# WasifurRahman/BERT_multimodal_transformer

Measured on AMD Instinct MI355X. Metric: train samples/sec MAG-BERT MOSI seq_len=50, higher is better.
Workload: dtype bf16; 1 GPU; MAG-BERT bert-base-uncased, MOSI dims (V=47, A=74), batch 48/GPU, seq_len 50, full optimizer step (fwd+MSE+bwd+HF-AdamW+schedule+zero_grad; inputs resident in HBM), dropout on, random-init weights; global_batch=48, seq_len=50, parallelism=dp1, step_call=mb_bert_train_step, hipGraph replay

## Files before the change

### bert_multimodal_transformer_amd/_lib.py

```python
import ctypes as C
import os

_HERE = os.path.dirname(os.path.abspath(__file__))
LIB_PATH = os.path.join(os.environ.get("MB_LIB_DIR") or os.path.join(_HERE, "lib"), "libmagbert_hip.so")

DT_F32, DT_BF16 = 0, 1
GEMM_NT, GEMM_NN, GEMM_TN = 0, 1, 2
EPI_BIAS, EPI_BIAS_GELU, EPI_BIAS_DROP_RES, EPI_ADD_RES, EPI_DGELU, EPI_ACCUM_F32, EPI_BIAS_F32 = range(7)
EPI_BIAS_RELU, EPI_BIAS_SWISH, EPI_BIAS_GELU_NEW, EPI_BIAS_MISH = 7, 8, 9, 10
ACT_GELU, ACT_RELU, ACT_SWISH, ACT_GELU_NEW, ACT_MISH = range(5)
ACTIVATIONS = {"gelu": ACT_GELU, "relu": ACT_RELU, "swish": ACT_SWISH, "silu": ACT_SWISH, "gelu_new": ACT_GELU_NEW, "mish": ACT_MISH}
ACT_EPILOGUE = {ACT_GELU: EPI_BIAS_GELU, ACT_RELU: EPI_BIAS_RELU, ACT_SWISH: EPI_BIAS_SWISH, ACT_GELU_NEW: EPI_BIAS_GELU_NEW,
                ACT_MISH: EPI_BIAS_MISH}


def activation_code(name, field):
    if isinstance(name, str) and name in ACTIVATIONS:
        return ACTIVATIONS[name]
    raise NotImplementedError("%s=%r: the feed-forward activations built are %s (and silu = swish)"
                              % (field, name, ", ".join(n for n in ACTIVATIONS if n != "silu")))


class DropKey(C.Structure):
    _fields_ = [("k0", C.c_uint32), ("k1", C.c_uint32), ("thresh", C.c_uint32), ("scale", C.c_float)]
# ... 49 lines not shown
    "mb_gemm": (_i, [_i, _i, _i, _i, _i, _i, _vp, _i, _vp, _i, _vp, _i, _vp, _vp, _vp, _vp, _i, _f, _dk, _i, _i, _vp]),
    "mb_gemm_grouped_wgrad": (_i, [_i, _i, _vp, _vp, _i, _vp, _vp, _vp, _vp, _vp, _vp, _i, _vp]),
    "mb_narrow": (_i, [_i, _vp, _vp, _sz, _vp]),
    "mb_widen": (_i, [_i, _vp, _vp, _sz, _vp]),
    "mb_layernorm_forward": (_i, [_i, _vp, _vp, _vp, _f, _vp, _vp, _vp, _i, _i, _dk, _vp]),
    "mb_layernorm_backward": (_i, [_i, _vp, _vp, _vp, _vp, _vp, _vp, _vp, _vp, _vp, _vp, _i, _i, _dk, _dk, _vp]),
    "mb_embed_forward": (_i, [_i, _vp, _vp, _vp, _vp, _vp, _vp, _vp, _f, _vp, _vp, _vp, _i, _i, _i, _dk, _vp]),
    "mb_embed_backward": (_i, [_i, _vp, _vp, _vp, _vp, _vp, _vp, _vp, _vp, _vp, _vp, _vp, _vp, _vp, _vp, _vp, _i, _i, _i,
                               _i, _dk, _vp]),
    "mb_attention_forward": (_i, [_i, _vp, _vp, _vp, _i, _i, _i, _dk, _vp]),
    "mb_attention_backward": (_i, [_i, _vp, _vp, _vp, _vp, _i, _i, _i, _dk, _vp]),
    "mb_attention_resident_forward": (_i, [_i, _vp, _vp, _vp, _i, _i, _i, _dk, _vp, _vp, _vp]),
    "mb_attention_resident_backward": (_i, [_i, _vp, _vp, _vp, _vp, _vp, _i, _i, _i, _dk, _vp, _vp]),
    "mb_head_forward": (_i, [_vp, _vp, _vp, _vp, _vp, _vp, _vp, _vp, _i, _i, _i, _dk, _i, _f, _vp, _vp]),
    "mb_head_backward": (_i, [_i, _vp, _vp, _vp, _f, _vp, _vp, _vp, _vp, _vp, _vp, _vp, _sz, _i, _i, _i, _dk, _i, _f, _vp, _vp]),
    "mb_head_forward_ex": (_i, [_vp, _vp, _vp, _vp, _vp, _vp, _vp, _vp, _i, _i, _i, _dk, C.POINTER(HeadLossStruct), _vp]),
    "mb_head_backward_ex": (_i, [_i, _vp, _vp, _vp, _f, _vp, _vp, _vp, _vp, _vp, _vp, _vp, _sz, _i, _i, _i, _dk, C.POINTER(HeadLossStruct), _vp]),
    "mb_bert_set_head_loss_ex": (_i, [_vp, C.POINTER(HeadLossStruct)]),
    "mb_bert_get_head_loss_ex": (_i, [_vp, C.POINTER(HeadLossStruct), _vp, C.POINTER(_i)]),
    "mb_xlnet_set_head_loss_ex": (_i, [_vp, C.POINTER(HeadLossStruct)]),
    "mb_xlnet_get_head_loss_ex": (_i, [_vp, C.POINTER(HeadLossStruct), _vp, C.POINTER(_i)]),
    "mb_bert_set_head_loss": (_i, [_vp, _i, _f, _vp]),
    "mb_bert_get_head_loss": (_i, [_vp, C.POINTER(_i), C.POINTER(_f), _vp, C.POINTER(_i)]),
    "mb_xlnet_set_head_loss": (_i, [_vp, _i, _f, _vp]),
    "mb_xlnet_get_head_loss": (_i, [_vp, C.POINTER(_i), C.POINTER(_f), _vp, C.POINTER(_i)]),
    "mb_attention_tiled_stats_bytes": (_sz, [_i, _i, _i]),
    "mb_attention_tiled_forward": (_i, [_i, _vp, _vp, _vp, _vp, _i, _i, _i, _dk, _vp, _vp, _vp]),
    "mb_attention_tiled_backward": (_i, [_i, _vp, _vp, _vp, _vp, _vp, _vp, _vp, _i, _i, _i, _dk, _vp, _vp]),
    "mb_mag_workspace_bytes": (_sz, [_i, _i, _i, _i, _i]),
    "mb_mag_forward": (_i, [_i] + [_vp] * 13 + [_f, _dk, _vp, _vp, _i, _i, _i, _i, _vp]),
    "mb_mag_backward": (_i, [_i] + [_vp] * 11 + [_f, _dk] + [_vp] * 14 + [_i, _i, _i, _i, _vp]),
    "mb_debug_mag_forward_ex": (_i, [_i] + [_vp] * 13 + [_f, _dk, _vp, _vp, _i, _i, _i, _i, _i, _vp]),
    "mb_debug_mag_slab_bytes": (_sz, [_i, _i]),
    "mb_debug_mag_backward_ex": (_i, [_i] + [_vp] * 7 + [_f, _dk] + [_vp] * 14 + [_i, _i, _i, _i, _i, _i, _i, _vp, _sz, _i,
                                      C.POINTER(_i), _vp]),
    "mb_adamw_step": (_i, [_vp, _vp, _vp, _vp, _vp, _sz, _sz, _sz, _sz, _f, _f, _f, _f, _f, _i, _i, _f, _i, _vp]),
    "mb_bert_create": (_i, [C.POINTER(BertEngineConfig), C.POINTER(_vp)]),
    "mb_bert_destroy": (None, [_vp]),
    "mb_bert_num_tensors": (_i, [_vp]),
    "mb_bert_tensor_info": (_i, [_vp, _i, C.c_char_p, _i, C.POINTER(_sz), C.POINTER(_sz), C.POINTER(_i),
                                 C.POINTER(C.c_int64), C.POINTER(_i)]),
    "mb_bert_param_count": (_sz, [_vp]),
    "mb_bert_decay_count": (_sz, [_vp]),
    "mb_bert_shadow_range": (None, [_vp, C.POINTER(_sz), C.POINTER(_sz)]),
    "mb_bert_workspace_bytes": (_sz, [_vp]),
    "mb_bert_bind": (_i, [_vp, _vp, _vp, _vp, _vp, _sz]),
    "mb_bert_sync_weights": (_i, [_vp, _vp]),
    "mb_bert_forward": (_i, [_vp, _vp, _vp, _vp, _vp, _vp, _vp, _i, _i, _i, _u64, _u64, _vp, _vp, _vp, _vp]),
    "mb_bert_backward": (_i, [_vp, _vp, _vp, _f, _i, _i, _vp]),
    "mb_bert_sequence_output": (_vp, [_vp]),
    "mb_bert_pooled_output": (_vp, [_vp]),
    "mb_bert_hidden_state": (_vp, [_vp, _i]),
    "mb_bert_set_attention_output": (_i, [_vp, _vp]),
    "mb_debug_gemm_ex": (_i, [_i, _i, _i, _i, _i, _i, _vp, _i, _vp, _i, _vp, _i, _vp, _vp, _vp, _vp, _i, _f, _dk, _i, _i,
                              _i, _sz, _i, _i, _vp, _i, _vp, _vp, _vp, _vp, _vp, _sz, _i, _i, _f, _f, _f, _f, _f, _i, _i, _f, _vp,
                              C.POINTER(_i), _vp]),
    "mb_debug_gemm_grouped_ex": (_i, [_i, _i, _vp, _vp, _i, _vp, _vp, _vp, _vp, _vp, _vp, _vp, _vp, _i, _i, _vp, _vp, _vp, _vp, _vp,
                                      _sz, _i, _i, _f, _f, _f, _f, _f, _i, _i, _f, _vp, _vp]),
    "mb_debug_gemm_last_kernel": (_i, [C.c_char_p, _i]),
    "mb_debug_gemm_grouped_rows": (_i, [_i, _i, _vp, _vp, _i, _vp, _vp, _vp, _vp, _vp, _vp, _vp, _i, _vp, _vp, _vp]),
    "mb_debug_live_rows": (_i, [_vp, _i, _i, _i, _vp, _vp, _vp, _vp, _vp]),
    "mb_bert_debug_live_wgrad_launches": (_i, [_vp]),
    "mb_bert_debug_wgrad_dy": (_vp, [_vp, _i, _i, C.POINTER(_i)]),
    "mb_debug_gemm_trace": (_i, [_vp, _i]),
    "mb_debug_attention_trace": (_i, [_vp, _i]),
    "mb_xlnet_attention_probs": (_vp, [_vp, _i, C.POINTER(_i)]),
    "mb_xlnet_attention_probs_into": (_i, [_vp, _i, _vp, _vp]),
    "mb_xlnet_attention_tiled_stats_bytes": (_sz, [_i, _i, _i]),
    "mb_xlnet_attention_tiled_scratch_bytes": (_sz, [_i, _i, _i, _i]),
    "mb_xlnet_attention_tiled_forward": (_i, [_i] + [_vp] * 10 + [_i, _i, _i, _dk, _vp, _vp, _i, _vp, _vp]),
    "mb_xlnet_attention_tiled_backward": (_i, [_i] + [_vp] * 19 + [_i, _i, _i, _dk, _vp, _vp, _vp]),
    "mb_xlnet_attention_forward": (_i, [_i] + [_vp] * 11 + [_i, _i, _i, _dk, _vp, _vp, _i, _vp]),
    "mb_xlnet_attention_backward": (_i, [_i] + [_vp] * 20 + [_i, _i, _i, _dk, _vp, _vp, _vp]),
    "mb_xlnet_set_head_mask": (_i, [_vp, _vp]),
    "mb_xlnet_set_perm_mask": (_i, [_vp, _vp]),
    "mb_xlnet_set_mems": (_i, [_vp, _vp, _i]),
    "mb_xlnet_query_stream_scratch_bytes": (_sz, [_vp, _i, _i, _i]),
    "mb_xlnet_query_stream_state_bytes": (_sz, [_vp, _i, _i]),
    "mb_xlnet_query_stream": (_i, [_vp, _vp, _i, _vp, _sz, _vp, _vp]),
    "mb_bert_mark_grads_zero": (_i, [_vp, _i]),
    "mb_xlnet_mark_grads_zero": (_i, [_vp, _i]),
    "mb_bert_distrust_word_stamps": (_i, [_vp]),
    "mb_bert_word_skip_updates": (_sz, [_vp]),
    "mb_bert_materialize_grads": (_i, [_vp, _vp]),
    "mb_xlnet_materialize_grads": (_i, [_vp, _vp]),
    "mb_bert_grads_stale": (_i, [_vp]),
    "mb_xlnet_grads_stale": (_i, [_vp]),
    "mb_bert_set_head_mask": (_i, [_vp, _vp]),
    "mb_bert_set_inputs_embeds": (_i, [_vp, _vp]),
    "mb_bert_set_position_ids": (_i, [_vp, _vp]),
    "mb_bert_inputs_embeds_grad": (_vp, [_vp]),
    "mb_bert_backward_outputs": (_i, [_vp, _vp, _vp, _vp]),
    "mb_bert_stage_grad_ranges": (_i, [_vp, _i, C.POINTER(_sz), C.POINTER(_sz), _i]),
    "mb_bert_train_step": (_i, [_vp, _vp, _vp, _vp, _vp, _vp, _vp, _i, _i, _u64, _u64, _vp, _vp, _vp, _vp, _vp, _f, _f, _f, _f, _f,
                                _i, _i, _f, _f, _i, _vp]),
    "mb_bert_stage_forward": (_i, [_vp, _vp, _vp, _vp, _vp, _vp, _vp, _i, _i, _u64, _u64, _vp, _vp, _vp, _i, _vp]),
    "mb_bert_stage_backward": (_i, [_vp, _f, _i, _i, _vp]),
    "mb_bert_staged_input_ids": (_vp, [_vp]),
    "mb_bert_load_batch": (_i, [_vp, _vp, _vp, _vp, _vp, _vp, _vp, _i, _i, C.POINTER(_vp), _vp]),
    "mb_bert_graph_stats": (_i, [_vp, C.POINTER(_sz), C.POINTER(_sz)]),
    "mb_bert_set_profiling": (_i, [_vp, _i]),
    "mb_bert_profile_wgrad_us": (_i, [_vp, C.POINTER(_f)]),
    "mb_bert_profile_adamw_us": (_i, [_vp, C.POINTER(_f)]),
    "mb_xlnet_set_inputs_embeds": (_i, [_vp, _vp]),
    "mb_xlnet_inputs_embeds_grad": (_vp, [_vp]),
    "mb_xlnet_model_output": (_vp, [_vp, _vp]),
    "mb_xlnet_backward_outputs": (_i, [_vp, _vp, _vp]),
    "mb_xlnet_set_profiling": (_i, [_vp, _i]),
    "mb_xlnet_profile_wgrad_us": (_i, [_vp, C.POINTER(_f)]),
    "mb_xlnet_profile_adamw_us": (_i, [_vp, C.POINTER(_f)]),
    "mb_xlnet_create": (_i, [C.POINTER(XlnetEngineConfig), C.POINTER(_vp)]),
    "mb_xlnet_destroy": (None, [_vp]),
    "mb_xlnet_num_tensors": (_i, [_vp]),
    "mb_xlnet_tensor_info": (_i, [_vp, _i, C.c_char_p, _i, C.POINTER(_sz), C.POINTER(_sz), C.POINTER(_i),
                                  C.POINTER(C.c_int64), C.POINTER(_i)]),
    "mb_xlnet_param_count": (_sz, [_vp]),
    "mb_xlnet_decay_count": (_sz, [_vp]),
    "mb_xlnet_shadow_range": (None, [_vp, C.POINTER(_sz), C.POINTER(_sz)]),
    "mb_xlnet_workspace_bytes": (_sz, [_vp]),
    "mb_xlnet_bind": (_i, [_vp, _vp, _vp, _vp, _vp, _sz]),
    "mb_xlnet_sync_weights": (_i, [_vp, _vp]),
    "mb_xlnet_forward": (_i, [_vp, _vp, _vp, _vp, _vp, _vp, _vp, _i, _i, _i, _u64, _u64, _vp, _vp, _vp, _vp]),
    "mb_xlnet_backward": (_i, [_vp, _vp, _vp, _f, _i, _i, _vp]),
    "mb_xlnet_sequence_output": (_vp, [_vp]),
    "mb_xlnet_hidden_state": (_vp, [_vp, _i]),
    "mb_xlnet_train_step": (_i, [_vp, _vp, _vp, _vp, _vp, _vp, _vp, _i, _i, _u64, _u64, _vp, _vp, _vp, _vp, _vp, _f, _f, _f, _f, _f,
                                 _i, _i, _f, _f, _i, _vp]),
    "mb_xlnet_load_batch": (_i, [_vp, _vp, _vp, _vp, _vp, _vp, _vp, _i, _i, C.POINTER(_vp), _vp]),
    "mb_xlnet_graph_stats": (_i, [_vp, C.POINTER(_sz), C.POINTER(_sz)]),
    "mb_xlnet_trainable_count": (_sz, [_vp]),
    "mb_bert_set_update_map": (_i, [_vp, _i, _i, _vp, _vp]),
    "mb_bert_set_update_decay": (_i, [_vp, _i, _vp]),
    "mb_bert_set_update_values": (_i, [_vp, _i, _vp, _vp, _vp, _vp, _vp, _vp]),
    "mb_bert_update_stats": (_i, [_vp, C.POINTER(_sz), C.POINTER(_sz), C.POINTER(_i)]),
    "mb_bert_set_update_frozen": (_i, [_vp, _i, _vp]),
    "mb_bert_freeze_stats": (_i, [_vp, C.POINTER(_sz), C.POINTER(_i), C.POINTER(_i)]),
    "mb_xlnet_set_update_frozen": (_i, [_vp, _i, _vp]),
    "mb_xlnet_freeze_stats": (_i, [_vp, C.POINTER(_sz), C.POINTER(_i), C.POINTER(_i)]),
    "mb_xlnet_set_update_map": (_i, [_vp, _i, _i, _vp, _vp]),
    "mb_xlnet_set_update_decay": (_i, [_vp, _i, _vp]),
    "mb_xlnet_set_update_values": (_i, [_vp, _i, _vp, _vp, _vp, _vp, _vp, _vp]),
    "mb_xlnet_update_stats": (_i, [_vp, C.POINTER(_sz), C.POINTER(_sz), C.POINTER(_i)]),
    "mb_grad_clip_scratch_bytes": (_sz, [_sz]),
    "mb_grad_clip_coef": (_i, [_vp, _sz, _f, _f, _vp, _vp, _vp]),
    "mb_bert_set_grad_clip": (_i, [_vp, _f]),
    "mb_bert_grad_clip_stats": (_i, [_vp, C.POINTER(_f), C.POINTER(_f), _vp]),
    "mb_xlnet_set_grad_clip": (_i, [_vp, _f]),
    "mb_xlnet_grad_clip_stats": (_i, [_vp, C.POINTER(_f), C.POINTER(_f), _vp]),
    "mb_xlnet_stage_grad_ranges": (_i, [_vp, _i, C.POINTER(_sz), C.POINTER(_sz), _i]),
    "mb_comm_unique_id": (_i, [_vp]),
    "mb_comm_create_rccl": (_i, [_vp, _i, _i, C.POINTER(_vp)]),
    "mb_comm_create_callbacks": (_i, [_i, _i, _vp, _vp, _vp, C.POINTER(_vp)]),
    "mb_comm_destroy": (None, [_vp]),
    "mb_comm_rank": (_i, [_vp]),
    "mb_comm_world": (_i, [_vp]),
    "mb_comm_stream": (_vp, [_vp]),
    "mb_comm_scratch_bytes": (_sz, [_i, _i, _sz, _i, _i, _i]),
    "mb_comm_bind_scratch": (_i, [_vp, _vp, _sz, _i, _sz, _i, _i, _i]),
    "mb_comm_all_reduce": (_i, [_vp, _vp, _sz, _vp]),
    "mb_comm_exchange_rows": (_i, [_vp, _vp, _vp, _i, _vp]),
    "mb_comm_set_row_exchange": (_i, [_vp, _i]),
    "mb_comm_set_sharding": (_i, [_vp, _i]),
    "mb_comm_sharding": (_i, [_vp]),
    "mb_comm_join": (_i, [_vp, _vp]),
    "mb_comm_gather_shards": (_i, [_vp, _vp, _i, _vp]),
    "mb_comm_shard_slices": (_i, [_vp, C.POINTER(_sz), _i]),
# ... 57 lines not shown
```

### bert_multimodal_transformer_amd/bert.py

```python
import ctypes as C
import os

import torch
import torch.nn as nn

from . import _lib
from . import losses as _losses
from .global_configs import ACOUSTIC_DIM, VISUAL_DIM


SUPPORTED_HIDDEN_SIZES = (256, 512, 768, 1024)


def check_bert_sizes(config, injection_index=None):
    H, nh, I, NL = (int(config.hidden_size), int(config.num_attention_heads), int(config.intermediate_size), int(config.num_hidden_layers))
    if H not in SUPPORTED_HIDDEN_SIZES:
        raise ValueError("hidden_size = %d: the HIP engine runs hidden sizes %s (heads of 64)" % (H, ", ".join(map(str, SUPPORTED_HIDDEN_SIZES))))
    if nh * 64 != H:
        raise ValueError("num_attention_heads = %d with hidden_size = %d: the attention kernels take heads of 64 (%d heads); hidden sizes %s"
                         % (nh, H, H // 64, ", ".join(map(str, SUPPORTED_HIDDEN_SIZES))))
    if I % 128 or I < 128:
        raise ValueError("intermediate_size = %d: must be a multiple of 128" % I)
    if NL < 1:
        raise ValueError("num_hidden_layers = %d: at least one layer" % NL)
# ... 174 lines not shown
        c, mc = self.config, self.mc
        if self.kind == "xlnet":
            return _lib.XlnetEngineConfig(
                c.vocab_size, c.d_model, c.n_layer, c.n_head, c.d_inner, c.num_labels, self.V, self.A, int(self.injection_index),
                c.layer_norm_eps, 1e-5, float(mc.beta_shift), c.dropout, c.summary_last_dropout, float(mc.dropout_prob),
                self.dt, int(B), int(L), _lib.activation_code(c.ff_activation, "ff_activation"))
        return _lib.BertEngineConfig(
            c.vocab_size, c.hidden_size, c.num_hidden_layers, c.num_attention_heads, c.intermediate_size,
            c.max_position_embeddings, c.type_vocab_size, c.num_labels, self.V, self.A, c.pad_token_id,
            c.layer_norm_eps, 1e-5, float(mc.beta_shift), c.hidden_dropout_prob, c.attention_probs_dropout_prob,
            float(mc.dropout_prob), self.dt, int(B), int(L), _lib.activation_code(c.hidden_act, "hidden_act"),
            int(self.injection_index))

    def _make_engine(self, B, L):
        h = C.c_void_p()
        cfg = self._cfg(B, L)
        _lib.check(self._fn("create")(C.byref(cfg), C.byref(h)))
        if self.handle is not None:
            self._fn("destroy")(self.handle)
            self.ws = None
        self.handle = h
        self._optional = (None, None, None, None, None)
        self._update_map = None
        self.max_B, self.max_L = B, L
        self._apply_loss()

    def _apply_loss(self):
        vec = self.loss.vector
        arr = None if vec is None else (C.c_float * len(vec))(*vec)
        hl = _lib.head_loss_struct(self.loss.code, self.loss.beta, None if arr is None else C.addressof(arr), self.loss.label_smoothing,
                                   self.loss.focal_gamma, self.loss.ignore_index)
        _lib.check(self._fn("set_head_loss_ex")(self.handle, C.byref(hl)))

    def set_loss(self, loss):
        old, self.loss = self.loss, loss
        try:
            self._apply_loss()
        except Exception:
            self.loss = old
            raise
        self._lab_ptr = None

    def _comm_join(self):
        comm = getattr(self, "_dp_comm", None)
        if comm is not None and comm.sharding and comm.handle is not None:
            _lib.check(self.lib.mb_comm_join(comm.handle, self.stream()))

    def refresh_sharded_state(self, adam=True):
        old = getattr(self, "_dp_shards", None)
        if old is not None:
            old.gather_masters()
            if adam and hasattr(self, "_adam_m"):
                old._gather([self._adam_m[a:b] for a, b in old.bounds])
                old._gather([self._adam_v[a:b] for a, b in old.bounds])
            return
        comm = getattr(self, "_dp_comm", None)
        if comm is None or not comm.sharding or comm.handle is None:
            return
        self._comm_join()
        st = self.stream()
        _lib.check(self.lib.mb_comm_gather_shards(comm.handle, _lib.ptr(self.params), 4, st))
        if adam and hasattr(self, "_adam_m"):
            _lib.check(self.lib.mb_comm_gather_shards(comm.handle, _lib.ptr(self._adam_m), 4, st))
            _lib.check(self.lib.mb_comm_gather_shards(comm.handle, _lib.ptr(self._adam_v), 4, st))

    def _ensure(self, B, L, join=True):
        if join:
            self._comm_join()
        if L > self.max_seq_length:
            raise _lib.MagbertError("magbert: unsupported shape or alignment: L = %d is above this model's max_seq_length = %d "
                                    "(construct it with max_seq_length=%d, at most %d)"
                                    % (L, self.max_seq_length, L,
                                       self.config.max_position_embeddings if self.kind == "bert" else XLNET_MAX_SEQ))
        if B > self.max_B or L > self.max_L or self.ws is None:
            self.materialize_grads()
            self._make_engine(max(B, self.max_B), max(L, self.max_L))
            nbytes = self._fn("workspace_bytes")(self.handle)
            self.ws = torch.empty(nbytes, dtype=torch.uint8, device=self.device)
            _lib.check(self._fn("bind")(self.handle, _lib.ptr(self.params), _lib.ptr(self.grads),
                                             _lib.ptr(self.shadow) if self.dt == _lib.DT_BF16 else None,
                                             _lib.ptr(self.ws), nbytes))
            self.weights_dirty = True
            _lib.check(self._fn("mark_grads_zero")(self.handle, 1 if self._gz else 0))

    def _tensor_table(self):
        out = []
        name = C.create_string_buffer(160)
        off, numel, ndim, decay = C.c_size_t(), C.c_size_t(), C.c_int(), C.c_int()
        shape = (C.c_int64 * 4)()
        for i in range(self._fn("num_tensors")(self.handle)):
            _lib.check(self._fn("tensor_info")(self.handle, i, name, 160, C.byref(off), C.byref(numel), C.byref(ndim),
                                                    shape, C.byref(decay)))
            out.append((name.value.decode(), off.value, numel.value, tuple(shape[k] for k in range(ndim.value)),
                        int(decay.value)))
        return out

    def stream(self):
        return torch.cuda.current_stream(self.device).cuda_stream

    class _Hop(object):

        def __init__(self, core):
            self.core = core
            self.cur = torch.cuda.current_stream(core.device)
            self.hop = self.cur.cuda_stream == 0
            self.ctx = None

        def __enter__(self):
            if self.hop:
                if self.core._own_stream is None:
                    self.core._own_stream = torch.cuda.Stream(device=self.core.device)
                self.core._own_stream.wait_stream(self.cur)
                self.ctx = torch.cuda.stream(self.core._own_stream)
                self.ctx.__enter__()
            return self

        def __exit__(self, *exc):
            if self.hop:
                self.ctx.__exit__(*exc)
                self.cur.wait_stream(self.core._own_stream)
            return False

    def sync_weights(self):
        if self.dt == _lib.DT_BF16:
            self.refresh_sharded_state(adam=False)
        with _Core._Hop(self):
            _lib.check(self._fn("sync_weights")(self.handle, self.stream()))
        self.weights_dirty = False

    def _pinned_batch(self, tensors, B, L):
        want = (torch.int64, torch.float32, torch.float32, torch.int64, torch.int64, torch.float32)
        shapes = ((B, L), (B, L, self.V), (B, L, self.A), (B, L), (B, L), None)
        for t, dt, shp in zip(tensors, want, shapes):
            if t is None:
                continue
            if t.is_cuda or t.dtype != dt or not t.is_contiguous() or (shp is not None and tuple(t.shape) != shp) or not t.is_pinned():
                return False
        return True

    def _inputs(self, input_ids, visual, acoustic, attention_mask, token_type_ids, labels, gather_in_step=False):
        B, L = input_ids.shape
        dev = self.device
        lab_in = None if labels is None else labels.reshape(-1)
        if lab_in is not None:
            _losses.check_labels(self.loss, lab_in, B, int(self.config.num_labels))
        six = (input_ids, visual, acoustic, attention_mask, token_type_ids, lab_in)
        if self._pinned_batch(six, B, L):
            ptrs = [None if t is None else C.c_void_p(t.data_ptr()) for t in six]
            if gather_in_step:
                return ptrs, six
            staged = (C.c_void_p * 6)()
            with _Core._Hop(self):
                _lib.check(self._fn("load_batch")(self.handle, ptrs[0], ptrs[1], ptrs[2], ptrs[3], ptrs[4], ptrs[5], B, L, staged,
                                                   self.stream()))
            off = staged[0] - self.ws.data_ptr()
            self._ids_dev = self.ws[off: off + B * L * 8].view(torch.int64)
            return [C.c_void_p(staged[i]) if staged[i] else None for i in range(6)], six
        nb = not input_ids.is_cuda and input_ids.is_pinned()
        ids = input_ids.to(dev, torch.int64, non_blocking=nb).contiguous()
        msk = attention_mask.to(dev, torch.int64, non_blocking=nb).contiguous()
        seg = token_type_ids.to(dev, torch.int64, non_blocking=nb).contiguous()
        vis = visual.to(dev, torch.float32, non_blocking=nb).contiguous()
        aco = acoustic.to(dev, torch.float32, non_blocking=nb).contiguous()
        if vis.shape != (B, L, self.V) or aco.shape != (B, L, self.A):
            raise ValueError("visual/acoustic must be [B, L, %d] / [B, L, %d], got %s / %s" %
                             (self.V, self.A, tuple(vis.shape), tuple(aco.shape)))
        lab = None if labels is None else labels.to(dev, torch.float32, non_blocking=nb).contiguous().view(-1)
        keep = (ids, vis, aco, msk, seg, lab)
        self._ids_dev = ids.reshape(-1)
        return [_lib.ptr(t) for t in keep], keep

    def _set_optional(self, head_mask=None, inputs_embeds=None, position_ids=None, perm=None, mems=None):
        want = (head_mask, inputs_embeds, position_ids, perm, mems)
        if all(x is None for x in want) and all(x is None for x in self._optional):
            return
        if self.kind != "bert":
            if position_ids is not None:
                raise NotImplementedError("position_ids is an argument of MAG-BERT only (XLNet has relative positions)")
            _lib.check(self.lib.mb_xlnet_set_head_mask(self.handle, _lib.ptr(head_mask)))
            _lib.check(self.lib.mb_xlnet_set_inputs_embeds(self.handle, _lib.ptr(inputs_embeds)))
            _lib.check(self.lib.mb_xlnet_set_perm_mask(self.handle, _lib.ptr(perm)))
            _lib.check(self.lib.mb_xlnet_set_mems(self.handle, _lib.ptr(mems), 0 if mems is None else int(mems.shape[2])))
        else:
            if perm is not None or mems is not None:
                raise NotImplementedError("perm_mask / mems are arguments of MAG-XLNet only")
            _lib.check(self.lib.mb_bert_set_head_mask(self.handle, _lib.ptr(head_mask)))
            _lib.check(self.lib.mb_bert_set_inputs_embeds(self.handle, _lib.ptr(inputs_embeds)))
            _lib.check(self.lib.mb_bert_set_position_ids(self.handle, _lib.ptr(position_ids)))
        self._optional = want

    def mark_grads_zero(self, known_zero=True):
        if not known_zero:
            self.materialize_grads()
        self._gz = bool(known_zero)
        self._gz_version = self.grads._version
        if self.handle is not None:
            _lib.check(self._fn("mark_grads_zero")(self.handle, 1 if known_zero else 0))

    def torch_wrote_grads(self):
        return (not self._gz) or self.grads._version != getattr(self, "_gz_version", -1)

    def materialize_grads(self):
        if self.handle is not None and self.ws is not None and self._fn("grads_stale")(self.handle):
            with _Core._Hop(self):
                _lib.check(self._fn("materialize_grads")(self.handle, self.stream()))

    def head_mask_table(self, head_mask):
        if head_mask is None:
            return None
        NL, nh = self.n_layers, (self.config.num_attention_heads if self.kind == "bert" else self.config.n_head)
        hm = torch.as_tensor(head_mask).to(self.device, torch.float32)
        if hm.dim() == 1 and hm.numel() == nh:
            hm = hm[None].expand(NL, nh)
        elif hm.numel() == NL * nh and (hm.dim() == 2 or tuple(hm.shape) == (NL, 1, nh, 1, 1)):
            hm = hm.reshape(NL, nh)
        else:
            raise NotImplementedError("head_mask must be [num_heads] or [num_layers, num_heads], got %s" % (tuple(hm.shape),))
        return hm.contiguous()

    def inputs_embeds_grad(self):
        p = self._fn("inputs_embeds_grad")(self.handle)
        B, L, H = self._emb_shape
        off = p - self.ws.data_ptr()
        return self.ws[off: off + B * L * H * 4].view(torch.float32).view(B, L, H).clone()

    def forward(self, input_ids, visual, acoustic, attention_mask, token_type_ids, labels, training, mems=None, head_mask=None,
                inputs_embeds=None, position_ids=None, perm=None):
        dev = self.device
        if inputs_embeds is not None:
            inputs_embeds = inputs_embeds.detach().to(dev, torch.float32).contiguous()
            B, L, H = inputs_embeds.shape
            if H != self.config.hidden_size:
                raise ValueError("inputs_embeds must be [B, L, %d]" % self.config.hidden_size)
            self._emb_shape = (B, L, H)
            input_ids = torch.zeros(B, L, dtype=torch.int64, device=dev)
        B, L = input_ids.shape
        self._ensure(B, L)
        if self.weights_dirty:
            self.sync_weights()
        if position_ids is not None:
            position_ids = position_ids.to(dev, torch.int64).expand(B, L).contiguous()
        if perm is not None:
            perm = perm.to(dev, torch.uint8).contiguous()
            if tuple(perm.shape) != (B, L, L):
                raise ValueError("perm_mask must be [B, L, L] = %s, got %s" % ((B, L, L), tuple(perm.shape)))
        self._set_optional(self.head_mask_table(head_mask), inputs_embeds, position_ids, perm, mems)
        ptr, keep = self._inputs(input_ids, visual, acoustic, attention_mask, token_type_ids, labels)
        logits = torch.empty(B, self.config.num_labels, dtype=torch.float32, device=dev)
        if training:
            self.step += 1
        self._keep = (keep, logits)
        self._lab_ptr = ptr[5]
        self.training_last = bool(training)
        with _Core._Hop(self):
            _lib.check(self._fn("forward")(self.handle, ptr[0], ptr[1], ptr[2], ptr[3], ptr[4], ptr[5], B, L, 1 if training else 0,
                                           self.seed & (2 ** 64 - 1), self.step, _lib.ptr(logits), C.c_void_p(self.loss_buf.data_ptr()),
                                           C.c_void_p(self.loss_buf.data_ptr() + 4) if ptr[5] is not None else None,
                                           self.stream()))
        return logits

    def _backward(self, dlogits=None, loss_scale=1.0):
        nstage = self.n_layers + 2
        lab = self._lab_ptr
        if dlogits is None and lab is None:
            raise ValueError("fused backward needs the labels passed to forward()")
        with _Core._Hop(self):
            self._gz = False
            for s in range(nstage):
                _lib.check(self._fn("backward")(self.handle, _lib.ptr(dlogits), lab if dlogits is None else None,
                                                float(loss_scale), s, s + 1, self.stream()))
                for hook in self.stage_hooks:
                    hook(s)

    def batch_ids(self):
        return self._ids_dev

    def fused_step_blocker(self):
        if self.stage_hooks:
            return "backward stage hooks are installed (data parallel: the gradient exchange is issued between stages)"
        return None
# ... 657 lines not shown
```

### bert_multimodal_transformer_amd/csrc/adamw.hip

```cpp
#include <cstdlib>
#include "kernels.h"
#include "adamw_dev.h"

namespace mb {

template <bool NT>
__global__ void __launch_bounds__(256) adamw_range_kernel(float* __restrict__ p, float* __restrict__ g, float* __restrict__ m,
                                                          float* __restrict__ v, bf16* __restrict__ shadow, size_t n4, size_t n_decay,
                                                          size_t sh_begin, size_t sh_end, size_t keep_begin, size_t keep_end, AdamArgs a,
                                                          const AdamArgs* __restrict__ dyn, int zero_grad) {
    if (dyn) a = *dyn;
    const size_t per = ((n4 + gridDim.x - 1) / gridDim.x + 255) / 256 * 256;
    const size_t begin = (size_t)blockIdx.x * per + threadIdx.x, end = min(n4, (size_t)(blockIdx.x + 1) * per);
    adam_span<NT>(p, g, m, v, shadow, begin, end, a, n_decay, sh_begin, sh_end, keep_begin, keep_end, zero_grad, false, WordSkip{}, 0u);
}

__global__ void adamw_tail_kernel(float* p, float* g, float* m, float* v, size_t begin, size_t n, size_t n_decay, AdamArgs a,
                                  const AdamArgs* dyn, int zero_grad) {
    if (dyn) a = *dyn;
    const size_t i = begin + threadIdx.x;
    if (i >= n) return;
    {
#pragma clang fp contract(off)
    const float gv = g[i] * a.grad_scale;
    const float mv = a.beta1 * m[i] + (1.0f - a.beta1) * gv;
    const float vv = a.beta2 * v[i] + (1.0f - a.beta2) * gv * gv;
    float pv = p[i] - a.step_size * (mv / (sqrtf(vv) + a.eps));
    if (i < n_decay && a.lr * a.weight_decay > 0.f) pv -= a.lr * a.weight_decay * pv;
    p[i] = pv; m[i] = mv; v[i] = vv;
    if (zero_grad) g[i] = 0.f;
    }
}

struct AdamLaunch { bool nt; unsigned grid; };
static int adam_launch(const float* p, const float* g, const float* m, const float* v, size_t n, size_t n4, AdamLaunch* out) {
    static int log = -1, nt = -1, vgrid = 0;
    if (log < 0) {
        const char* e = getenv("MB_GEMM_LOG"); log = e ? atoi(e) : 0;
        e = getenv("MB_ADAMW_NT"); nt = e ? atoi(e) : 1;
        e = getenv("MB_ADAMW_GRID"); vgrid = e ? atoi(e) : 0;
    }
    if (log) fprintf(stderr, "[magbert adamw] n=%zu\n", n);
    if (((uintptr_t)p | (uintptr_t)g | (uintptr_t)m | (uintptr_t)v) & 15) return MB_ERR_SHAPE;
    unsigned grid = (unsigned)((n4 + 255) / 256);
    if (grid > 256 * 16) grid = 256 * 16;
    if (vgrid > 0 && (unsigned)vgrid < grid) grid = (unsigned)vgrid;
    *out = AdamLaunch{nt != 0, grid};
    return MB_OK;
}

int adamw_step(float* p, float* g, float* m, float* v, void* shadow, size_t n, size_t n_decay, size_t sh_begin,
               size_t sh_end, AdamArgs a, int zero_grad, hipStream_t st, const AdamArgs* dyn, size_t keep_begin, size_t keep_end) {
    if (n == 0) return MB_OK;
    const size_t n4 = n / 4;
    AdamLaunch l;
    if (const int rc = adam_launch(p, g, m, v, n, n4, &l)) return rc;
    if ((n_decay % 4 && n_decay < n) || (sh_begin % 4) || (sh_end % 4) || (keep_begin % 4) || (keep_end % 4)) return MB_ERR_SHAPE;
    if (n4) {
        auto k = l.nt ? adamw_range_kernel<true> : adamw_range_kernel<false>;
        hipLaunchKernelGGL(k, dim3(l.grid), dim3(256), 0, st, p, g, m, v, (bf16*)shadow, n4, n_decay, sh_begin, sh_end, keep_begin, keep_end, a,
                           dyn, zero_grad);
    }
    if (n % 4) hipLaunchKernelGGL(adamw_tail_kernel, dim3(1), dim3(64), 0, st, p, g, m, v, n4 * 4, n, n_decay, a, dyn, zero_grad);
    return (int)hipGetLastError();
}

template <bool NT>
__global__ void __launch_bounds__(256) adamw_sweep_kernel(float* __restrict__ p, float* __restrict__ g, float* __restrict__ m,
                                                          float* __restrict__ v, bf16* __restrict__ shadow, const AdamPieces R,
                                                          size_t sh_begin, size_t sh_end, size_t keep_begin, size_t keep_end,
                                                          const AdamArgs* __restrict__ cls, WordSkip ws, unsigned upd_blocks) {
    if (blockIdx.x >= upd_blocks) {
        const size_t c0 = R.start4[R.clear_first], ctotal4 = R.start4[R.count] - c0;
        const unsigned nclr = gridDim.x - upd_blocks;
        const size_t cper = ((ctotal4 + nclr - 1) / nclr + 255) / 256 * 256;
        const size_t cb = c0 + (size_t)(blockIdx.x - upd_blocks) * cper, ce = min(c0 + ctotal4, cb + cper);
#pragma unroll 1
        for (int k = R.clear_first; k < R.count; ++k) {
            const size_t off = R.start4[k], nxt = R.start4[k + 1];
            if (nxt <= cb) continue;
            if (off >= ce) break;
            const size_t lo = max(cb, off), hi = min(ce, nxt);
            const size_t base4 = (size_t)R.begin4[k] - off;
            for (size_t i4 = base4 + lo + threadIdx.x; i4 < base4 + hi; i4 += 256) {
                if constexpr (NT) __builtin_nontemporal_store(f32x4{0.f, 0.f, 0.f, 0.f}, (f32x4*)(g + i4 * 4));
                else *(f32x4*)(g + i4 * 4) = f32x4{0.f, 0.f, 0.f, 0.f};
            }
        }
        return;
    }
    const size_t total4 = R.start4[R.clear_first];
    const size_t per = ((total4 + upd_blocks - 1) / upd_blocks + 255) / 256 * 256;
    const size_t vb = (size_t)blockIdx.x * per, ve = min(total4, vb + per);
    const bool skip_on = ws.stamp != nullptr && ws.state[1] != 0u;
    const uint32_t stamp_no = skip_on ? ws.state[0] : 0u;
#pragma unroll 1
    for (int k = 0; k < R.clear_first; ++k) {
        const size_t off = R.start4[k], nxt = R.start4[k + 1];
        if (nxt <= vb) continue;
        if (off >= ve) break;
        const size_t lo = max(vb, off), hi = min(ve, nxt);
        if (lo >= hi) continue;
        const AdamArgs a = cls[R.slot[k]];
        const size_t base4 = (size_t)R.begin4[k] - off;
        adam_span<NT>(p, g, m, v, shadow, base4 + lo + threadIdx.x, base4 + hi, a, ~(size_t)0, sh_begin, sh_end, keep_begin, keep_end, 1,
                      skip_on, ws, stamp_no);
    }
}

int adamw_sweep(float* p, float* g, float* m, float* v, void* shadow, const AdamPieces& r, size_t sh_begin, size_t sh_end,
                size_t keep_begin, size_t keep_end, const AdamArgs* cls, const WordSkip& skip, hipStream_t st) {
    if (r.count < 0 || r.count > MB_SWEEP_PIECES_MAX || r.clear_first < 0 || r.clear_first > r.count || !cls) return MB_ERR_ARG;
    if (r.count && r.start4[0] != 0u) return MB_ERR_ARG;
    for (int k = 0; k < r.count; ++k)
        if (r.start4[k + 1] < r.start4[k] || (k < r.clear_first ? r.slot[k] >= 2 * MB_CLASSES_MAX : r.slot[k] != MB_PIECE_CLEAR)) return MB_ERR_SHAPE;
    const size_t n4 = r.count ? r.start4[r.clear_first] : 0, c4 = r.count ? r.start4[r.count] - n4 : 0;
    if (n4 + c4 == 0) return MB_OK;
    if ((sh_begin % 4) || (sh_end % 4) || (keep_begin % 4) || (keep_end % 4)) return MB_ERR_SHAPE;
    if (skip.stamp && (!skip.state || skip.row_len == 0 || (skip.begin | skip.end | skip.row_len) % 4 || skip.end < skip.begin ||
                       skip.end - skip.begin > 0xffffffffull)) return MB_ERR_SHAPE;
    AdamLaunch l;
    if (const int rc = adam_launch(p, g, m, v, n4 * 4, n4, &l)) return rc;
    unsigned cgrid = (unsigned)((c4 + 2047) / 2048);
    if (cgrid > 256) cgrid = 256;
    auto k = l.nt ? adamw_sweep_kernel<true> : adamw_sweep_kernel<false>;
    hipLaunchKernelGGL(k, dim3(l.grid + cgrid), dim3(256), 0, st, p, g, m, v, (bf16*)shadow, r, sh_begin, sh_end, keep_begin, keep_end, cls, skip,
                       l.grid);
    return (int)hipGetLastError();
}

}
```

### bert_multimodal_transformer_amd/csrc/adamw_dev.h

```cpp
#pragma once
#include "kernels.h"

namespace mb {

struct AdamQuad { f32x4 p, g, m, v; };
template <bool NT> __device__ __forceinline__ AdamQuad adam_load(const float* p, const float* g, const float* m, const float* v, size_t i) {
    AdamQuad q;
    if constexpr (NT) {
        q.p = __builtin_nontemporal_load((const f32x4*)(p + i)); q.g = __builtin_nontemporal_load((const f32x4*)(g + i));
        q.m = __builtin_nontemporal_load((const f32x4*)(m + i)); q.v = __builtin_nontemporal_load((const f32x4*)(v + i));
    } else {
        q.p = *(const f32x4*)(p + i); q.g = *(const f32x4*)(g + i); q.m = *(const f32x4*)(m + i); q.v = *(const f32x4*)(v + i);
    }
    return q;
}
template <bool NT> __device__ __forceinline__ AdamQuad adam_load(const float* p, const float* g, const float* m, const float* v, size_t i, bool live) {
    AdamQuad q;
    q.g = f32x4{0.f, 0.f, 0.f, 0.f};
    if constexpr (NT) {
        q.p = __builtin_nontemporal_load((const f32x4*)(p + i));
        if (live) q.g = __builtin_nontemporal_load((const f32x4*)(g + i));
        q.m = __builtin_nontemporal_load((const f32x4*)(m + i)); q.v = __builtin_nontemporal_load((const f32x4*)(v + i));
    } else {
        q.p = *(const f32x4*)(p + i);
        if (live) q.g = *(const f32x4*)(g + i);
        q.m = *(const f32x4*)(m + i); q.v = *(const f32x4*)(v + i);
    }
    return q;
}
template <bool NT> __device__ __forceinline__ void adam_update_store(AdamQuad q, float* p, float* g, float* m, float* v, bf16* shadow, size_t i,
                                                                     const AdamArgs& a, float omb1, float omb2, float decay, size_t n_decay,
                                                                     size_t sh_begin, size_t sh_end, size_t keep_begin, size_t keep_end, int zero_grad) {
#pragma clang fp contract(off)
    q.g *= a.grad_scale;
    q.m = a.beta1 * q.m + omb1 * q.g;
    q.v = a.beta2 * q.v + omb2 * q.g * q.g;
#pragma unroll
    for (int r = 0; r < 4; ++r) q.p[r] -= a.step_size * (q.m[r] / (sqrtf(q.v[r]) + a.eps));
    if (i < n_decay && decay > 0.f) q.p -= decay * q.p;
    const bool zg = zero_grad && !(i >= keep_begin && i < keep_end);
    if constexpr (NT) {
        __builtin_nontemporal_store(q.p, (f32x4*)(p + i));
        __builtin_nontemporal_store(q.m, (f32x4*)(m + i));
        __builtin_nontemporal_store(q.v, (f32x4*)(v + i));
        if (zg) __builtin_nontemporal_store(f32x4{0.f, 0.f, 0.f, 0.f}, (f32x4*)(g + i));
    } else {
        *(f32x4*)(p + i) = q.p;
        *(f32x4*)(m + i) = q.m;
        *(f32x4*)(v + i) = q.v;
        if (zg) *(f32x4*)(g + i) = f32x4{0.f, 0.f, 0.f, 0.f};
    }
    if (shadow && i >= sh_begin && i < sh_end) store4(shadow + i, q.p);
}

template <bool NT>
__device__ __forceinline__ void adam_span(float* p, float* g, float* m, float* v, bf16* shadow, size_t begin, size_t end, const AdamArgs& a,
                                          size_t n_decay, size_t sh_begin, size_t sh_end, size_t keep_begin, size_t keep_end, int zero_grad,
                                          bool skip_on, const WordSkip& ws, uint32_t stamp_no) {
    constexpr int UNR = 2; const size_t stride = 256;
    const float omb1 = 1.0f - a.beta1, omb2 = 1.0f - a.beta2;
    const float decay = a.lr * a.weight_decay;
    for (size_t i4 = begin; i4 < end; i4 += stride * UNR) {
        AdamQuad q[UNR];
        bool live[UNR];
#pragma unroll
        for (int u = 0; u < UNR; ++u) {
            live[u] = true;
            if (i4 + u * stride < end) {
                const size_t i = (i4 + u * stride) * 4;
                if (skip_on && i >= ws.begin && i < ws.end) live[u] = ws.stamp[(uint32_t)(i - ws.begin) / ws.row_len] == stamp_no;
                q[u] = adam_load<NT>(p, g, m, v, i, live[u]);
            }
        }
#pragma unroll
        for (int u = 0; u < UNR; ++u)
            if (i4 + u * stride < end)
                adam_update_store<NT>(q[u], p, g, m, v, shadow, (i4 + u * stride) * 4, a, omb1, omb2, decay, n_decay, sh_begin, sh_end, keep_begin,
                                      keep_end, live[u] ? zero_grad : 0);
    }
}

template <int NTHREADS, int UNR>
__device__ __forceinline__ void adam_ride_block(const AdamRide& r, int rb) {
    if (r.n4 == 0) return;
    const AdamArgs a = *r.dyn;
    const float omb1 = 1.0f - a.beta1, omb2 = 1.0f - a.beta2;
    const float decay = a.lr * a.weight_decay;
    const size_t per = ((r.n4 + r.blocks - 1) / r.blocks + NTHREADS - 1) / NTHREADS * NTHREADS;
    const size_t begin = (size_t)rb * per + threadIdx.x;
    const size_t end = r.n4 < (size_t)(rb + 1) * per ? r.n4 : (size_t)(rb + 1) * per;
    const size_t all = ~(size_t)0;
    constexpr size_t half = (size_t)NTHREADS * UNR;
    AdamQuad qa[UNR], qb[UNR];
    auto load = [&](AdamQuad (&q)[UNR], size_t i4) {
#pragma unroll
        for (int u = 0; u < UNR; ++u)
            if (i4 + (size_t)u * NTHREADS < end) q[u] = adam_load<true>(r.p, r.g, r.m, r.v, (i4 + (size_t)u * NTHREADS) * 4);
    };
    auto update = [&](AdamQuad (&q)[UNR], size_t i4) {
#pragma unroll
        for (int u = 0; u < UNR; ++u)
            if (i4 + (size_t)u * NTHREADS < end)
                adam_update_store<true>(q[u], r.p, r.g, r.m, r.v, r.shadow, (i4 + (size_t)u * NTHREADS) * 4, a, omb1, omb2, decay, all, 0, r.shadow ? all : 0,
                                        0, 0, r.zero_grad);
    };
    load(qa, begin);
    for (size_t i4 = begin; i4 < end; i4 += 2 * half) {
        load(qb, i4 + half);
        update(qa, i4);
        load(qa, i4 + 2 * half);
        update(qb, i4 + half);
    }
}

}
```

### bert_multimodal_transformer_amd/csrc/engine.hip

```cpp
#include "dp_step.h"

struct LayerOff { size_t wqkv, wo, w1, w2, bqkv, bo, ln1w, ln1b, b1, b2, ln2w, ln2b; };
#ifndef MB_WGRAD_LIVE_DEFAULT
#define MB_WGRAD_LIVE_DEFAULT 1
#endif
struct LayerWs { size_t qkv, ctx, s1, st1, y1, u, g, s2, st2, stats; };

struct mb_bert_engine : StepMixin {
    mb_bert_config c;
    std::vector<TensorInfo> tensors;
    std::vector<LayerOff> lo;
    size_t word, pos, type, emb_lnw, emb_lnb, wp, bp, wc, bc;
    size_t mag_whv, mag_wha, mag_wv, mag_wa, mag_bhv, mag_bha, mag_bv, mag_ba, mag_lnw, mag_lnb;
    size_t n_params, n_decay, sh_begin, sh_end;
    size_t n_update_end() const { return n_params; }
    int n_layers() const { return c.num_layers; }
    size_t layer_begin(int l) const { return lo[l].wqkv; }
    size_t layers_end() const { return wp; }
    int width() const { return c.hidden_size; }
    size_t layer_end(int l) const { return l + 1 < c.num_layers ? lo[l + 1].wqkv : wp; }
    bool embed_all_frozen() const { return range_frozen(word, mag_whv) && range_frozen(emb_lnw, bp); }
    WordSkip word_skip(char* w) const {
        if (!(stamp_off != 0 && stamp_enable && idcnt_enable)) return {};
        return WordSkip{stamp_table(w), stamp_state(w), word, word + (size_t)c.vocab_size * c.hidden_size, (uint32_t)c.hidden_size};
// ... 61 lines not shown
    for (int l = 0; l < c.num_layers; ++l) {
        LayerOff& o = e->lo[l];
        o.wqkv = e->add(nm(l, "attention.self.query.weight"), {H, H}, 1, cur);
        e->add(nm(l, "attention.self.key.weight"), {H, H}, 1, cur);
        e->add(nm(l, "attention.self.value.weight"), {H, H}, 1, cur);
        o.wo = e->add(nm(l, "attention.output.dense.weight"), {H, H}, 1, cur);
        o.w1 = e->add(nm(l, "intermediate.dense.weight"), {I, H}, 1, cur);
        o.w2 = e->add(nm(l, "output.dense.weight"), {H, I}, 1, cur);
    }
    e->wp = e->add("bert.pooler.dense.weight", {H, H}, 1, cur);
    e->sh_end = cur;
    e->word = e->add("bert.embeddings.word_embeddings.weight", {c.vocab_size, H}, 1, cur);
    e->pos = e->add("bert.embeddings.position_embeddings.weight", {c.max_position, H}, 1, cur);
    e->type = e->add("bert.embeddings.token_type_embeddings.weight", {c.type_vocab, H}, 1, cur);
    e->mag_whv = e->add("bert.MAG.W_hv.weight", {H, V + H}, 1, cur);
    e->mag_wha = e->add("bert.MAG.W_ha.weight", {H, A + H}, 1, cur);
    e->mag_wv = e->add("bert.MAG.W_v.weight", {H, V}, 1, cur);
    e->mag_wa = e->add("bert.MAG.W_a.weight", {H, A}, 1, cur);
    e->wc = e->add("classifier.weight", {c.num_labels, H}, 1, cur);
    e->n_decay = cur;
    for (int l = 0; l < c.num_layers; ++l) {
        LayerOff& o = e->lo[l];
        o.bqkv = e->add(nm(l, "attention.self.query.bias"), {H}, 0, cur);
        e->add(nm(l, "attention.self.key.bias"), {H}, 0, cur);
        e->add(nm(l, "attention.self.value.bias"), {H}, 0, cur);
        o.bo = e->add(nm(l, "attention.output.dense.bias"), {H}, 0, cur);
        o.ln1w = e->add(nm(l, "attention.output.LayerNorm.weight"), {H}, 0, cur);
        o.ln1b = e->add(nm(l, "attention.output.LayerNorm.bias"), {H}, 0, cur);
        o.b1 = e->add(nm(l, "intermediate.dense.bias"), {I}, 0, cur);
        o.b2 = e->add(nm(l, "output.dense.bias"), {H}, 0, cur);
        o.ln2w = e->add(nm(l, "output.LayerNorm.weight"), {H}, 0, cur);
        o.ln2b = e->add(nm(l, "output.LayerNorm.bias"), {H}, 0, cur);
    }
    e->emb_lnw = e->add("bert.embeddings.LayerNorm.weight", {H}, 0, cur);
    e->emb_lnb = e->add("bert.embeddings.LayerNorm.bias", {H}, 0, cur);
    e->bp = e->add("bert.pooler.dense.bias", {H}, 0, cur);
    e->mag_bhv = e->add("bert.MAG.W_hv.bias", {H}, 0, cur);
    e->mag_bha = e->add("bert.MAG.W_ha.bias", {H}, 0, cur);
    e->mag_bv = e->add("bert.MAG.W_v.bias", {H}, 0, cur);
    e->mag_ba = e->add("bert.MAG.W_a.bias", {H}, 0, cur);
    e->mag_lnw = e->add("bert.MAG.LayerNorm.weight", {H}, 0, cur);
    e->mag_lnb = e->add("bert.MAG.LayerNorm.bias", {H}, 0, cur);
    e->bc = e->add("classifier.bias", {c.num_labels}, 0, cur);
    e->n_params = cur;

    const size_t es = esize(c.dtype);
    const size_t T = align_up((size_t)c.max_batch * c.max_seq, 64);
    Carver w;
    e->mw.init(c.dtype, (int)T, (int)H, (int)V, (int)A);
    e->ws_mag = w.take(e->mw.bytes);
    e->pk_vis = e->ws_mag + e->mw.vp; e->pk_aco = e->ws_mag + e->mw.ap; e->pk_Vp = e->mw.Vp; e->pk_Ap = e->mw.Ap; e->pk_dtype = c.dtype;
    e->ws_emb = w.take(T * H * es);
    e->ws_emb_st = w.take(2 * T * 4);
    e->ws_x.resize(c.num_layers + 1);
    for (int l = 0; l <= c.num_layers; ++l) e->ws_x[l] = w.take(T * H * es);
    e->ws_pre = c.injection_index >= 1 ? w.take(T * H * es) : 0;
    e->lw.resize(c.num_layers);
    for (int l = 0; l < c.num_layers; ++l) {
        LayerWs& x = e->lw[l];
        x.qkv = w.take(T * 3 * H * es); x.ctx = w.take(T * H * es); x.s1 = w.take(T * H * es); x.st1 = w.take(2 * T * 4);
        x.y1 = w.take(T * H * es); x.u = w.take(T * I * es); x.g = w.take(T * I * es); x.s2 = w.take(T * H * es);
        x.st2 = w.take(2 * T * 4);
        x.stats = c.max_seq > 128 ? w.take(tiled_stats_floats(c.max_batch, c.max_seq, c.num_heads) * 4) : 0;
    }
    e->ws_head_z = w.take((size_t)c.max_batch * H * 4);
    e->ws_head_pooled = w.take((size_t)c.max_batch * H * 4);
    e->ws_logits = w.take((size_t)c.max_batch * c.num_labels * 4);
    e->ws_dxa = w.take(T * H * es); e->ws_dxb = w.take(T * H * es);
    for (int k = 0; k < 2; ++k) {
        e->ws_ds[k] = w.take(T * H * es); e->ws_dzd[k] = w.take(T * H * es); e->ws_ds2[k] = w.take(T * H * es);
        e->ws_dzd2[k] = w.take(T * H * es); e->ws_du[k] = w.take(T * I * es); e->ws_dqkv[k] = w.take(T * 3 * H * es);
    }
    e->ws_dctx = w.take(T * H * es); e->ws_dsum = w.take(T * H * 4); e->ws_dz = w.take((size_t)c.max_batch * H * es);
    e->lnp_stride = ln_partials_floats((int)T, (int)H);
    {
        const size_t emb = (size_t)c.max_seq * ((c.max_batch + 7) / 8) * 3 * H;
        if (emb > e->lnp_stride) e->lnp_stride = emb;
    }
    e->ws_lnp_a = w.take(e->lnp_stride * 4 * (c.num_layers + 2)); e->ws_lnp_b = w.take(e->lnp_stride * 4 * (c.num_layers + 2));
    e->carve_step(w, T, (int)V, (int)A, c.max_batch, c.num_labels, SITE_LAYER0 + 4 * c.num_layers);
    e->idcnt_off = w.take((size_t)c.vocab_size * 4);
    e->idcnt_enable = env_on("MB_EMBED_UNIQUE", true);
    e->stamp_rows = (size_t)c.vocab_size;
    e->stamp_off = w.take(((size_t)c.vocab_size + 2) * 4);
    e->stamp_enable = env_on("MB_ADAMW_SKIP_ZERO_ROWS", true);
    if (c.dtype == DT_BF16) {
        e->live_cap = std::max((size_t)192, T);
        e->live_off = w.take(2 * (e->live_cap + 8) * 4);
        e->live_mode = env_int("MB_WGRAD_LIVE_ROWS", e->deterministic ? 0 : MB_WGRAD_LIVE_DEFAULT);
        if (e->live_mode < 0 || e->live_mode > 2) e->live_mode = MB_WGRAD_LIVE_DEFAULT;
        e->live_enable = e->live_mode > 0;
    }
    e->one_sweep = env_on("MB_ADAMW_ONE_SWEEP", true);
    if (e->deterministic) {
        e->det_begin = e->wp; e->det_end = e->n_params;
        e->ws_det = w.take((e->det_end - e->det_begin) * sizeof(long long));
    }
    e->ws_bytes = w.off;
}

static int prepare_pass(mb_bert_engine* e, int T, hipStream_t st) {
    const mb_bert_config& c = e->c;
    const int H = c.hidden_size, I = c.intermediate_size, dt = c.dtype;
    char* ws = e->ws;
    const int Tp = (int)align_up((size_t)T, 64);
    if (!e->ws_zeroed) { CK((int)hipMemsetAsync(ws, 0, e->ws_bytes, st)); e->ws_zeroed = true; e->padT = T; }
    if (e->padT != T && Tp > T) {
        const size_t es = esize(dt);
        auto zp = [&](size_t off, size_t cols) {
            return (int)hipMemsetAsync(ws + off + (size_t)T * cols * es, 0, (size_t)(Tp - T) * cols * es, st);
        };
        CK(zp(e->ws_emb, H));
        if (c.injection_index >= 1) CK(zp(e->ws_pre, H));
        CK(mag_clear_pad_rows(dt, ws + e->ws_mag, e->mw, T, H, st));
        for (int k = 0; k < 2; ++k) {
            CK(zp(e->ws_ds[k], H)); CK(zp(e->ws_dzd[k], H)); CK(zp(e->ws_ds2[k], H)); CK(zp(e->ws_dzd2[k], H));
            CK(zp(e->ws_du[k], I)); CK(zp(e->ws_dqkv[k], 3 * H));
        }
        for (int l = 0; l <= c.num_layers; ++l) CK(zp(e->ws_x[l], H));
        for (int l = 0; l < c.num_layers; ++l) { CK(zp(e->lw[l].ctx, H)); CK(zp(e->lw[l].y1, H)); CK(zp(e->lw[l].g, I)); }
    }
    e->padT = T;
    return MB_OK;
}

static AdamArgs adam_scalars(float lr, float beta1, float beta2, float eps, float weight_decay, int step, int correct_bias, float grad_scale) {
    AdamArgs a;
    a.lr = lr; a.beta1 = beta1; a.beta2 = beta2; a.eps = eps; a.weight_decay = weight_decay; a.grad_scale = grad_scale;
    double ss = lr;
    if (correct_bias) ss = (double)lr * sqrt(1.0 - pow((double)beta2, (double)step)) / (1.0 - pow((double)beta1, (double)step));
    a.step_size = (float)ss;
    return a;
}
static int debug_ride(AdamRide& r, float* p, float* g, float* m, float* v, void* shadow, size_t n4, int blocks, int zero_grad, const AdamArgs& a,
                      void* adam_dev, hipStream_t st) {
    r = AdamRide{};
    if (blocks == 0) return MB_OK;
    if (blocks < 0 || !p || !g || !m || !v || !adam_dev) return MB_ERR_ARG;
    if ((((uintptr_t)p | (uintptr_t)g | (uintptr_t)m | (uintptr_t)v) & 15) || ((uintptr_t)shadow & 7) || ((uintptr_t)adam_dev & 3)) return MB_ERR_SHAPE;
    CK((int)hipMemcpyAsync(adam_dev, &a, sizeof(AdamArgs), hipMemcpyHostToDevice, st));
    CK((int)hipStreamSynchronize(st));
    r.p = p; r.g = g; r.m = m; r.v = v; r.shadow = (bf16*)shadow; r.n4 = n4; r.dyn = (const AdamArgs*)adam_dev; r.blocks = blocks;
    r.zero_grad = zero_grad;
    return MB_OK;
}

extern "C" {

const char* mb_error_string(int code) {
    switch (code) {
        case MB_OK: return "ok";
        case MB_ERR_SHAPE: return "magbert: unsupported shape or alignment";
        case MB_ERR_MODE: return "magbert: unsupported layout/epilogue combination";
        case MB_ERR_DTYPE: return "magbert: unsupported dtype";
        case MB_ERR_ARG: return "magbert: invalid argument";
        case MB_ERR_COMM: return "magbert: gradient exchange unavailable (mb_comm_last_error())";
        default:
            if (code >= 2000 && code < 2100) return "magbert: RCCL call failed (mb_comm_last_error())"; return hipGetErrorString((hipError_t)code);
    }
}
int mb_version(void) { return 100; }

void mb_make_dropkey(uint64_t seed, uint64_t step, uint32_t site, float p, mb_dropkey* out) {
    DropKey k = make_key(seed, step, site, p);
    out->k0 = k.k0; out->k1 = k.k1; out->thresh = k.thresh; out->scale = k.scale;
}

static int abi_epilogue(int& epilogue, int layout, GemmArgs& a) {
// ... 209 lines not shown
                                   int L, int nh, const mb_dropkey* drop, const float* head_scale, void* stream) {
    if (int e = resident_check(dtype, B, L, nh, dk(drop))) return e;
    if (!qkv || !mask || !dctx || !dqkv) return MB_ERR_ARG;
    return attention_backward(dtype, qkv, mask, nullptr, dctx, dqkv, dbias, B, L, nh, dk(drop), (hipStream_t)stream, head_scale);
}
size_t mb_attention_tiled_stats_bytes(int B, int L, int nh) {
    return (B < 1 || L < 1 || nh < 1) ? 0 : tiled_stats_floats(B, L, nh) * sizeof(float);
}
int mb_attention_tiled_forward(int dtype, const void* qkv, const int64_t* mask, void* ctx, float* stats, int B, int L, int nh,
                               const mb_dropkey* drop, const float* head_scale, float* probs, void* stream) {
    return attention_tiled_forward(dtype, qkv, mask, ctx, stats, B, L, nh, dk(drop), (hipStream_t)stream, probs, head_scale);
}
int mb_attention_tiled_backward(int dtype, const void* qkv, const int64_t* mask, const void* ctx, const void* dctx, float* stats,
                                void* dqkv, float* dbias, int B, int L, int nh, const mb_dropkey* drop, const float* head_scale,
                                void* stream) {
    return attention_tiled_backward(dtype, qkv, mask, ctx, dctx, stats, dqkv, dbias, B, L, nh, dk(drop), (hipStream_t)stream, head_scale);
}

size_t mb_mag_workspace_bytes(int dtype, int T, int H, int V, int A) {
    MagWs w;
    w.init(dtype, T, H, V, A);
    return w.bytes;
}
int mb_mag_forward(int dtype, const void* text, const float* visual, const float* acoustic, const float* W_hv,
                   const float* b_hv, const float* W_ha, const float* b_ha, const float* W_v, const float* b_v,
                   const float* W_a, const float* b_a, const float* ln_w, const float* ln_b, float beta_shift,
                   const mb_dropkey* drop, void* out, void* ws, int T, int H, int V, int A, void* stream) {
    if (H % 256 || H < 256 || H > 1024 || V < 1 || A < 1) return MB_ERR_SHAPE;
    MagWs w;
    w.init(dtype, T, H, V, A);
    return mag_fwd_impl(dtype, text, visual, acoustic, W_hv, b_hv, W_ha, b_ha, W_v, b_v, W_a, b_a, ln_w, ln_b, 1e-5f,
                        beta_shift, dk(drop), out, (char*)ws, w, T, H, V, A, true, (hipStream_t)stream);
}
int mb_mag_backward(int dtype, const void* d_out, const void* text, const float* W_hv, const float* b_hv,
                    const float* W_ha, const float* b_ha, const float* W_v, const float* b_v, const float* W_a,
                    const float* b_a, const float* ln_w, float beta_shift, const mb_dropkey* drop, void* ws, void* d_text,
                    float* d_visual, float* d_acoustic, float* dW_hv, float* db_hv, float* dW_ha, float* db_ha,
                    float* dW_v, float* db_v, float* dW_a, float* db_a, float* dln_w, float* dln_b, int T, int H, int V,
                    int A, void* stream) {
    (void)W_hv; (void)W_ha; (void)W_v; (void)W_a;
    if (H % 256 || H < 256 || H > 1024 || V < 1 || A < 1) return MB_ERR_SHAPE;
    MagWs w;
    w.init(dtype, T, H, V, A);
    return mag_bwd_impl(dtype, d_out, text, b_hv, b_ha, b_v, b_a, ln_w, beta_shift, dk(drop), (char*)ws, w, d_text,
                        d_visual, d_acoustic, dW_hv, db_hv, dW_ha, db_ha, dW_v, db_v, dW_a, db_a, dln_w, dln_b, T, H, V, A,
                        false, (hipStream_t)stream);
}

int mb_debug_mag_forward_ex(int dtype, const void* text, const float* visual, const float* acoustic, const float* W_hv,
                            const float* b_hv, const float* W_ha, const float* b_ha, const float* W_v, const float* b_v,
                            const float* W_a, const float* b_a, const float* ln_w, const float* ln_b, float beta_shift,
                            const mb_dropkey* drop, void* out, void* ws, int T, int H, int V, int A, int pads_clean, void* stream) {
    if (H % 256 || H < 256 || H > 1024 || V < 1 || A < 1) return MB_ERR_SHAPE;
    MagWs w;
    w.init(dtype, T, H, V, A);
    return mag_fwd_impl(dtype, text, visual, acoustic, W_hv, b_hv, W_ha, b_ha, W_v, b_v, W_a, b_a, ln_w, ln_b, 1e-5f,
                        beta_shift, dk(drop), out, (char*)ws, w, T, H, V, A, true, (hipStream_t)stream, pads_clean != 0);
}
size_t mb_debug_mag_slab_bytes(int T, int H) { return T < 1 ? 0 : (size_t)2 * ((T + 7) / 8) * 3 * H * sizeof(float); }
int mb_debug_mag_backward_ex(int dtype, const void* d_out, const void* text, const float* b_hv, const float* b_ha, const float* b_v,
                             const float* b_a, const float* ln_w, float beta_shift, const mb_dropkey* drop, void* ws, void* d_text,
                             float* d_visual, float* d_acoustic, float* dW_hv, float* db_hv, float* dW_ha, float* db_ha,
                             float* dW_v, float* db_v, float* dW_a, float* db_a, float* dln_w, float* dln_b, int T, int H, int V,
                             int A, int text_padded, int pads_clean, int slabs, float* slab_scratch, size_t slab_bytes, int dw_zero,
                             int* path, void* stream) {
    hipStream_t st = (hipStream_t)stream;
    if (H % 256 || H < 256 || H > 1024 || V < 1 || A < 1) return MB_ERR_SHAPE;
    if (slabs && (!slab_scratch || slab_bytes < mb_debug_mag_slab_bytes(T, H))) return MB_ERR_ARG;
    MagWs w;
    w.init(dtype, T, H, V, A);
    float* pa = slabs ? slab_scratch : nullptr;
    float* pb = slabs ? slab_scratch + mb_debug_mag_slab_bytes(T, H) / (2 * sizeof(float)) : nullptr;
    int nblk = 0;
    CK(mag_bwd_impl(dtype, d_out, text, b_hv, b_ha, b_v, b_a, ln_w, beta_shift, dk(drop), (char*)ws, w, d_text, d_visual,
                    d_acoustic, dW_hv, db_hv, dW_ha, db_ha, dW_v, db_v, dW_a, db_a, dln_w, dln_b, T, H, V, A, text_padded != 0, st,
                    GradAcc{}, pads_clean != 0, pa, pb, &nblk, dw_zero != 0, path));
    if (slabs) {
        float* const m6[6] = {db_hv, db_ha, db_v, db_a, dln_w, dln_b};
        CK(ln_reduce_partials(pa, pb, nblk, H, m6, st, GradAcc{}));
    }
    return MB_OK;
}

int mb_adamw_step(float* p, float* g, float* m, float* v, void* shadow, size_t n, size_t n_decay, size_t sh_begin,
                  size_t sh_end, float lr, float beta1, float beta2, float eps, float weight_decay, int step,
                  int correct_bias, float grad_scale, int zero_grad, void* stream) {
    const AdamArgs a = adam_scalars(lr, beta1, beta2, eps, weight_decay, step, correct_bias, grad_scale);
    return adamw_step(p, g, m, v, shadow, n, n_decay, sh_begin, sh_end, a, zero_grad, (hipStream_t)stream);
}

size_t mb_grad_clip_scratch_bytes(size_t n) { return (size_t)grad_norm_blocks(n) * sizeof(double); }
int mb_grad_clip_coef(const float* g, size_t n, float max_norm, float grad_scale, void* scratch, float* out2, void* stream) {
    if (!scratch || !out2) return MB_ERR_ARG;
    CK(grad_sumsq(g, n, (double*)scratch, (hipStream_t)stream));
    return grad_clip_finalize((const double*)scratch, grad_norm_blocks(n), nullptr, max_norm, grad_scale, out2, ClipTables{}, (hipStream_t)stream);
}

int mb_bert_create(const mb_bert_config* cfg, mb_bert_engine** out) {
    if (!cfg || !out) return MB_ERR_ARG;
    const int Hc = cfg->hidden_size;
    if ((Hc != 256 && Hc != 512 && Hc != 768 && Hc != 1024) || cfg->num_heads * 64 != Hc || cfg->num_layers < 1) return MB_ERR_SHAPE;
    if (cfg->intermediate_size % 128 || cfg->max_seq < 1 || cfg->max_seq > 512 || cfg->max_batch < 1) return MB_ERR_SHAPE;
    if (cfg->max_seq > cfg->max_position || cfg->num_labels < 1) return MB_ERR_SHAPE;
    if (cfg->dtype != DT_F32 && cfg->dtype != DT_BF16) return MB_ERR_DTYPE;
    if (cfg->hidden_act < ACT_GELU || cfg->hidden_act > ACT_MISH) return MB_ERR_ARG;
    if (cfg->injection_index < 0 || cfg->injection_index >= cfg->num_layers) return MB_ERR_ARG;
    mb_bert_engine* e = new mb_bert_engine();
    e->c = *cfg;
    e->read_env();
    e->ride_opts.read_env();
    e->group_wgrad = env_int("MB_GROUP_WGRAD", e->group_wgrad);
    e->ride_blocks = env_int("MB_ADAMW_RIDE_BLOCKS", e->ride_blocks);
    e->ride_params = env_long("MB_ADAMW_RIDE_PARAMS", e->ride_params);
    e->prefetch = env_int("MB_PREFETCH", e->prefetch);
    e->pf_qkv = env_int("MB_PF_QKV", e->pf_qkv);
    if (e->group_wgrad == 256 && (cfg->dtype != DT_BF16 || cfg->hidden_size % 256 != 0 || cfg->intermediate_size % 256 != 0)) e->group_wgrad = 128;
    e->grouped = (e->group_wgrad == 64 || e->group_wgrad == 128 || e->group_wgrad == 256) && cfg->hidden_size % e->group_wgrad == 0 &&
                 cfg->intermediate_size % e->group_wgrad == 0;

    build_layout(e);
    e->ow_covers = e->grouped;
    e->stale_begin = e->lo[0].wqkv; e->stale_end = e->wp;
    *out = e;
    return MB_OK;
}
void mb_bert_destroy(mb_bert_engine* e) {
    if (!e) return;
    e->destroy_prof();
    e->drop_graphs();
    e->free_class_table();
    e->free_clip_buf();
    e->free_head_loss();
    delete e;
}
int mb_bert_num_tensors(const mb_bert_engine* e) { return (int)e->tensors.size(); }
int mb_bert_tensor_info(const mb_bert_engine* e, int i, char* name, int name_cap, size_t* offset, size_t* numel, int* ndim,
                        int64_t* shape4, int* decay) {
    if (i < 0 || i >= (int)e->tensors.size()) return MB_ERR_ARG;
    const TensorInfo& t = e->tensors[i];
    if (name && name_cap > 0) { strncpy(name, t.name.c_str(), name_cap - 1); name[name_cap - 1] = 0; }
    if (offset) *offset = t.off;
    if (numel) *numel = t.numel;
    if (ndim) *ndim = t.ndim;
    if (shape4) for (int k = 0; k < 4; ++k) shape4[k] = t.shape[k];
    if (decay) *decay = t.decay;
    return MB_OK;
}
size_t mb_bert_param_count(const mb_bert_engine* e) { return e->n_params; }
size_t mb_bert_decay_count(const mb_bert_engine* e) { return e->n_decay; }
void mb_bert_shadow_range(const mb_bert_engine* e, size_t* b, size_t* en) { *b = e->sh_begin; *en = e->sh_end; }
size_t mb_bert_workspace_bytes(const mb_bert_engine* e) { return e->ws_bytes; }

int mb_bert_bind(mb_bert_engine* e, float* params, float* grads, void* shadow, void* workspace, size_t ws_bytes) {
    if (!params || !workspace || ws_bytes < e->ws_bytes) return MB_ERR_ARG;
    if (e->c.dtype == DT_BF16 && !shadow) return MB_ERR_ARG;
    e->P = params; e->G = grads; e->SH = (char*)shadow; e->ws = (char*)workspace;
    e->grads_zero = false;
    e->frz_dirty = true;
    e->stamp_live = e->word_zero = false; e->sweep_no = 1;
    e->ws_zeroed = false; e->padT = -1;
    e->drop_graphs();
    char* mws = e->ws + e->ws_mag;
    e->pkw = {e->P + e->mag_whv, e->P + e->mag_wha, e->P + e->mag_wv, e->P + e->mag_wa, mws + e->mw.We, mws + e->mw.Wv, mws + e->mw.Wa,
              MagDims{0, e->c.hidden_size, e->c.visual_dim, e->c.acoustic_dim, e->mw.Vp, e->mw.Ap}, e->c.dtype};
    return MB_OK;
}

int mb_bert_sync_weights(mb_bert_engine* e, void* stream) {
    hipStream_t st = (hipStream_t)stream;
    if (!e->P) return MB_ERR_ARG;
    if (e->c.dtype == DT_BF16)
        CK(convert(DT_BF16, e->P + e->sh_begin, e->SH + e->sh_begin * 2, e->sh_end - e->sh_begin, st));
    const mb_bert_config& c = e->c;
    MagDims d = {0, c.hidden_size, c.visual_dim, c.acoustic_dim, e->mw.Vp, e->mw.Ap};
    char* mws = e->ws + e->ws_mag;
    CK(mag_pack_weights(c.dtype, e->P + e->mag_whv, e->P + e->mag_wha, e->P + e->mag_wv, e->P + e->mag_wa, mws + e->mw.We,
                        mws + e->mw.Wv, mws + e->mw.Wa, d, st));
    return MB_OK;
}

static int bert_forward_range(mb_bert_engine* e, const int64_t* input_ids, const float* visual, const float* acoustic,
                              const int64_t* attention_mask, const int64_t* token_type_ids, const float* labels, int B, int L,
                              int training, uint64_t seed, uint64_t step, float* logits, float* loss, float* loss_run, void* stream,
                              int l0, int l1, bool first, bool last) {
    hipStream_t st = (hipStream_t)stream;
    const mb_bert_config& c = e->c;
    if (!e->P || !e->ws) return MB_ERR_ARG;
    if (B < 1 || B > c.max_batch || L < 1 || L > c.max_seq) return MB_ERR_SHAPE;
    if ((!input_ids && !e->emb_in) || !visual || !acoustic || !attention_mask || !token_type_ids || !logits) return MB_ERR_ARG;
    const int dt = c.dtype, H = c.hidden_size, I = c.intermediate_size, T = B * L, nh = c.num_heads;
    if (e->emb_in) input_ids = nullptr;
    e->ids = input_ids; e->seg = token_type_ids; e->mask = attention_mask; e->ran_forward = true;
    e->B = B; e->L = L; e->training = training; e->seed = seed; e->step = step; e->logits = logits;
    float* P = e->P;
    char* ws = e->ws;
    if (first && !e->capturing) CK(prepare_pass(e, T, st));
    const int inj = c.injection_index;
    if (first) CK(embed_ln_forward(dt, input_ids, token_type_ids, e->emb_in ? e->emb_in : P + e->word, P + e->pos, P + e->type, P + e->emb_lnw, P + e->emb_lnb,
                        c.layer_norm_eps, ws + (inj >= 1 ? e->ws_x[0] : e->ws_emb), (float*)(ws + e->ws_emb_st), (float*)(ws + e->ws_emb_st) + T, B, L,
                        H, e->key(SITE_EMB, c.hidden_dropout), st, e->pos_ids));
    auto mag = [&](const char* text, char* out) -> int {
        return mag_fwd_impl(dt, text, visual, acoustic, P + e->mag_whv, P + e->mag_bhv, P + e->mag_wha, P + e->mag_bha,
                            P + e->mag_wv, P + e->mag_bv, P + e->mag_wa, P + e->mag_ba, P + e->mag_lnw, P + e->mag_lnb,
                            c.mag_layer_norm_eps, c.beta_shift, e->key(SITE_MAG, c.mag_dropout), out, ws + e->ws_mag,
                            e->mw, T, H, c.visual_dim, c.acoustic_dim, !(e->in_step && e->packed_w), st, true, e->in_step && e->packed);
    };
    if (first && inj == 0) CK(mag(ws + e->ws_emb, ws + e->ws_x[0]));
    for (int l = l0; l < l1; ++l) {
        const LayerOff& o = e->lo[l];
        const LayerWs& w = e->lw[l];
        if (l == inj && inj >= 1) CK(mag(ws + e->ws_pre, ws + e->ws_x[l]));
        const char* x = ws + e->ws_x[l];
        CK(gemm(dt, GEMM_NT, EPI_BIAS, T, 3 * H, H, x, H, e->W(o.wqkv), H, ws + w.qkv, 3 * H, nullptr, nullptr, P + o.bqkv,
                nullptr, 0, kNoDrop, 1, 0, st));
        CK(attention_forward(dt, ws + w.qkv, attention_mask, ws + w.ctx, B, L, nh,
                             e->key(SITE_LAYER0 + 4 * l + 0, c.attn_dropout), st,
                             e->attn_out ? e->attn_out + (size_t)l * B * nh * L * L : nullptr,
                             e->head_mask ? e->head_mask + (size_t)l * nh : nullptr, e->attn_stats(w)));
        CK(gemm(dt, GEMM_NT, EPI_BIAS_DROP_RES, T, H, H, ws + w.ctx, H, e->W(o.wo), H, ws + w.s1, H, nullptr, nullptr,
                P + o.bo, x, H, e->key(SITE_LAYER0 + 4 * l + 1, c.hidden_dropout), 1, 0, st));
        const size_t wes = dt == DT_BF16 ? 2 : 4;
        const Prefetch pf1 = {e->prefetch ? e->W(o.w1) : nullptr, (size_t)2 * I * H * wes, nullptr};
        const Prefetch pf2 = {(e->prefetch && l + 1 < c.num_layers && (l + 1 < l1 || last)) ? e->W(e->lo[l + 1].wqkv) : nullptr, (size_t)4 * H * H * wes, nullptr};
        CK(ln_forward(dt, ws + w.s1, P + o.ln1w, P + o.ln1b, c.layer_norm_eps, ws + w.y1, (float*)(ws + w.st1),
                      (float*)(ws + w.st1) + T, T, H, kNoDrop, st, pf1));
        CK(gemm(dt, GEMM_NT, ffn_act_mode(c.hidden_act), T, I, H, ws + w.y1, H, e->W(o.w1), H, ws + w.u, I, ws + w.g, nullptr, P + o.b1,
                nullptr, 0, kNoDrop, 1, 0, st, 0, 0, GradAcc{}, c.hidden_act));
        CK(gemm(dt, GEMM_NT, EPI_BIAS_DROP_RES, T, H, I, ws + w.g, I, e->W(o.w2), I, ws + w.s2, H, nullptr, nullptr,
                P + o.b2, ws + w.y1, H, e->key(SITE_LAYER0 + 4 * l + 2, c.hidden_dropout), 1, 0, st));
        CK(ln_forward(dt, ws + w.s2, P + o.ln2w, P + o.ln2b, c.layer_norm_eps, ws + (l + 1 == inj ? e->ws_pre : e->ws_x[l + 1]), (float*)(ws + w.st2),
                      (float*)(ws + w.st2) + T, T, H, kNoDrop, st, pf2));
    }
    if (!last) return MB_OK;
    float* z = (float*)(ws + e->ws_head_z);
    CK(gemm(dt, GEMM_NT, EPI_BIAS_F32, B, H, H, ws + e->ws_x[c.num_layers], L * H, e->W(e->wp), H, nullptr, H, nullptr, z,
            P + e->bp, nullptr, 0, kNoDrop, 1, 64, st));
    if (loss && !(e->in_step && e->loss_cleared)) CK(zero_fill(loss, 4, st));
    if (labels && !e->in_step) CK(e->sync_head_loss());
    CK(head_forward(z, P + e->wc, P + e->bc, labels, (float*)(ws + e->ws_head_pooled), logits, loss, loss_run, B, H,
                    c.num_labels, e->key(SITE_HEAD, c.hidden_dropout), st, e->head_loss()));
    return MB_OK;
}
// ... 385 lines not shown

const int64_t* mb_bert_staged_input_ids(const mb_bert_engine* e) { return (e && e->ws) ? (const int64_t*)(e->ws + e->ws_in_ids) : nullptr; }

int mb_bert_load_batch(mb_bert_engine* e, const int64_t* input_ids, const float* visual, const float* acoustic,
                       const int64_t* attention_mask, const int64_t* token_type_ids, const float* labels, int B, int L,
                       const void** staged6, void* stream) {
    hipStream_t st = (hipStream_t)stream;
    if (!e || !e->ws || !staged6) return MB_ERR_ARG;
    const mb_bert_config& c = e->c;
    if (B < 1 || B > c.max_batch || L < 1 || L > c.max_seq) return MB_ERR_SHAPE;
    if (!input_ids || !visual || !acoustic || !attention_mask || !token_type_ids) return MB_ERR_ARG;
    const int T = B * L;
    char* ws = e->ws;
    CK(prepare_pass(e, T, st));
    PrologueArgs pa = {};
    e->fill_copies(pa, ws, input_ids, visual, acoustic, attention_mask, token_type_ids, labels, B, L, c.visual_dim, c.acoustic_dim,
                   c.num_labels);
    CK(step_prologue(pa, st));
    e->staged(ws, labels != nullptr, staged6);
    return MB_OK;
}

int mb_bert_graph_stats(const mb_bert_engine* e, size_t* captures, size_t* launches) {
    if (!e) return MB_ERR_ARG;
    if (captures) *captures = e->graph_captures;
    if (launches) *launches = e->graph_launches;
    return MB_OK;
}

int mb_bert_set_profiling(mb_bert_engine* e, int on) {
    if (!e) return MB_ERR_ARG;
    return e->set_profiling(on, e->c.num_layers);
}
int mb_bert_profile_wgrad_us(mb_bert_engine* e, float* avg_us) {
    if (!e || !e->grouped) return MB_ERR_ARG;
    return e->prof_span_us(0, e->c.num_layers, avg_us);
}
int mb_bert_profile_adamw_us(mb_bert_engine* e, float* us) {
    if (!e) return MB_ERR_ARG;
    return e->prof_span_us(2 * e->c.num_layers, 1, us);
}

const void* mb_bert_hidden_state(const mb_bert_engine* e, int i) {
    if (!e || !e->ws || i < 0 || i > e->c.num_layers) return nullptr;
    return e->ws + e->ws_x[i];
}
const void* mb_bert_debug_wgrad_dy(const mb_bert_engine* e, int layer, int which, int* ld) {
    if (!e || !e->ws || layer < 0 || layer >= e->c.num_layers || which < 0 || which > 7) return nullptr;
    const int par = layer & 1, H = e->c.hidden_size, I = e->c.intermediate_size;
    const bool hd = e->training && e->c.hidden_dropout > 0.f;
    if (ld) *ld = (which == 1 || which == 4) ? I : which == 3 ? 3 * H : H;
    const LayerWs& w = e->lw[layer];
    switch (which) {
        case 4: return e->ws + w.g;
        case 5: return e->ws + w.y1;
        case 6: return e->ws + w.ctx;
        case 7: return e->ws + e->ws_x[layer];
        case 0: return e->ws + (hd ? e->ws_dzd[par] : e->ws_ds[par]);
        case 1: return e->ws + e->ws_du[par];
        case 2: return e->ws + (hd ? e->ws_dzd2[par] : e->ws_ds2[par]);
        default: return e->ws + e->ws_dqkv[par];
    }
}
int mb_bert_set_attention_output(mb_bert_engine* e, float* probs) {
    if (!e) return MB_ERR_ARG;
    e->attn_out = probs;
    return MB_OK;
}
int mb_bert_mark_grads_zero(mb_bert_engine* e, int known_zero) {
    if (!e) return MB_ERR_ARG;
    e->grads_zero = known_zero != 0;
    if (!known_zero) e->stamp_live = e->word_zero = false;
    if (!known_zero) e->frz_dirty = true;
    if (known_zero) e->grads_stale = false;
    return MB_OK;
}
int mb_bert_distrust_word_stamps(mb_bert_engine* e) {
    if (!e) return MB_ERR_ARG;
    e->stamp_live = e->word_zero = false;
    e->frz_dirty = true;
    return MB_OK;
}
size_t mb_bert_word_skip_updates(const mb_bert_engine* e) { return e ? e->skip_updates : 0; }
int mb_bert_materialize_grads(mb_bert_engine* e, void* stream) {
    if (!e) return MB_ERR_ARG;
    return e->materialize_grads(e->G, (hipStream_t)stream);
}
int mb_bert_grads_stale(const mb_bert_engine* e) { return e && e->grads_stale ? 1 : 0; }
int mb_bert_set_head_mask(mb_bert_engine* e, const float* head_mask) {
    if (!e) return MB_ERR_ARG;
    e->head_mask = head_mask;
    return MB_OK;
}
int mb_bert_set_head_loss(mb_bert_engine* e, int kind, float param, const float* vec) {
    if (!e) return MB_ERR_ARG;
    return e->set_head_loss(kind, param, vec, e->c.num_labels);
}
int mb_bert_get_head_loss(const mb_bert_engine* e, int* kind, float* param, float* vec, int* has_vec) {
    if (!e) return MB_ERR_ARG;
    return e->get_head_loss(kind, param, vec, has_vec);
}
int mb_bert_set_head_loss_ex(mb_bert_engine* e, const mb_head_loss* hl) {
    if (!e || !hl) return MB_ERR_ARG;
    return e->set_head_loss_ex(*hl, e->c.num_labels);
}
int mb_bert_get_head_loss_ex(const mb_bert_engine* e, mb_head_loss* hl, float* vec, int* has_vec) {
    if (!e) return MB_ERR_ARG;
    return e->get_head_loss_ex(hl, vec, has_vec);
}
int mb_bert_set_inputs_embeds(mb_bert_engine* e, const float* inputs_embeds) {
    if (!e) return MB_ERR_ARG;
    e->emb_in = inputs_embeds;
    return MB_OK;
}
int mb_bert_set_position_ids(mb_bert_engine* e, const int64_t* position_ids) {
    if (!e) return MB_ERR_ARG;
    e->pos_ids = position_ids;
    return MB_OK;
}
const float* mb_bert_inputs_embeds_grad(const mb_bert_engine* e) {
    if (!e || !e->ws || !e->ran_forward) return nullptr;
    return (const float*)(e->ws + e->ws_dsum);
}
int mb_bert_backward_outputs(mb_bert_engine* e, const void* d_sequence_output, const void* d_pooler_preact, void* stream) {
    hipStream_t st = (hipStream_t)stream;
    if (!e || !e->G || !e->ran_forward) return MB_ERR_ARG;
    CK(e->begin_backward_pass(e->G, st));
    const mb_bert_config& c = e->c;
    const int dt = c.dtype, H = c.hidden_size, B = e->B, L = e->L, T = B * L, NL = c.num_layers;
    char* ws = e->ws;
    const size_t bytes = (size_t)T * H * esize(dt);
    if (d_sequence_output) CK((int)hipMemcpyAsync(ws + e->ws_dxa, d_sequence_output, bytes, hipMemcpyDeviceToDevice, st));
    else CK(zero_fill(ws + e->ws_dxa, bytes, st));
    if (d_pooler_preact) {
        const char* xf = ws + e->ws_x[NL];
        CK(gemm(dt, GEMM_TN, EPI_ACCUM_F32, H, H, B, d_pooler_preact, H, xf, L * H, nullptr, H, nullptr, e->G + e->wp, nullptr, nullptr, 0,
                kNoDrop, 1, 64, st));
        CK(colsum(dt, d_pooler_preact, H, e->G + e->bp, B, H, st, e->acc_of(ws, e->G)));
        CK(gemm(dt, GEMM_NN, EPI_ADD_RES, B, H, H, d_pooler_preact, H, e->W(e->wp), H, ws + e->ws_dxa, L * H, nullptr, nullptr, nullptr,
                ws + e->ws_dxa, L * H, kNoDrop, 1, 64, st));
    }
    return MB_OK;
}

const void* mb_bert_sequence_output(const mb_bert_engine* e) { return e->ws ? e->ws + e->ws_x[e->c.num_layers] : nullptr; }
const float* mb_bert_pooled_output(const mb_bert_engine* e) { return e->ws ? (const float*)(e->ws + e->ws_head_pooled) : nullptr; }

int mb_bert_stage_grad_ranges(const mb_bert_engine* e, int stage, size_t* offs, size_t* lens, int cap) {
    const int NL = e->c.num_layers;
    std::vector<std::pair<size_t, size_t>> r;
    auto span = [&](size_t a, size_t b) { r.push_back({a, b - a}); };
    if (stage == 0) {
        span(e->wp, e->sh_end);
        span(e->wc, e->n_decay);
        span(e->bp, e->mag_bhv);
        span(e->bc, e->n_params);
    } else if (stage <= NL) {
        const int l = NL - stage;
        const LayerOff& o = e->lo[l];
        span(o.wqkv, l + 1 < NL ? e->lo[l + 1].wqkv : e->wp);
        span(o.bqkv, l + 1 < NL ? e->lo[l + 1].bqkv : e->emb_lnw);
    } else if (stage == NL + 1) {
        span(e->word, e->wc);
        span(e->emb_lnw, e->bp);
        span(e->mag_bhv, e->bc);
    } else return -1;
// ... 7 lines not shown
```

### bert_multimodal_transformer_amd/csrc/engine_common.h

```cpp
#pragma once
#include <string>
#include <vector>
#include <cstring>
#include <cstdio>
#include <cstdlib>
#include <cmath>
#include <algorithm>
#include "kernels.h"
#include "../../include/magbert_hip.h"

using namespace mb;
static_assert(MB_UPDATE_CLASSES_MAX == MB_CLASSES_MAX && MB_UPDATE_SEGMENTS_MAX == MB_SEGMENTS_MAX, "public limits = the kernels' limits");

namespace {

struct TensorInfo {
    std::string name;
    size_t off, numel;
    int ndim;
    int64_t shape[4];
    int decay;
};

inline size_t align_up(size_t x, size_t a) { return (x + a - 1) / a * a; }
// ... 120 lines not shown
        int per_cu = 0;
        const int tiles = gemm_nn_ride_tiles(dt, mode, a, &per_cu);
        const int slots = per_cu * cus, rounds = tiles > 0 ? (tiles + slots - 1) / slots : 0;
        const int blocks = tiles > 0 ? (ro.dgrad_blocks > 0 ? ro.dgrad_blocks : rounds * slots - tiles) / 8 * 8 : 0;
        if (blocks >= 8) {
            size_t budget = ro.dgrad_params > 0 ? (size_t)ro.dgrad_params : (size_t)(1.25e6 * ((double)Mo * No * Ko) / (2400.0 * 768.0 * 3072.0)) / 1024 * 1024;
            if (mode == EPI_DGELU) budget = ro.dgelu_params > 0 ? (size_t)ro.dgelu_params : (size_t)blocks * 14336;
            else if (per_cu == 1) budget = ride_pn_params() > 0 ? (size_t)ride_pn_params() : (size_t)(blocks * 16384.0 * ((double)Mo * No * Ko) / (2400.0 * 768.0 * 3072.0)) / 1024 * 1024;
            const AdamRide r = take(budget, blocks);
            if (r.blocks) return gemm_nn_ride_launch(dt, mode, a, r, st);
        }
    }
    if (mode == EPI_DGELU)
        return gemm(dt, GEMM_NN, EPI_DGELU, Mo, No, Ko, dY, ldy, Wt, ldw, dX, ldx, nullptr, colsum, nullptr, R, ldr, drop, 1, 0, st, 0, 0, acc);
    return gemm(dt, GEMM_NN, EPI_ADD_RES, Mo, No, Ko, dY, ldy, Wt, ldw, dX, ldx, nullptr, nullptr, nullptr, R, ldr, drop, 1, 0, st);
}

inline GemmArgs wgrad_args(int Mo, int No, int rows, const void* dY, int ldy, const void* X, int ldx, float* dW, int ldw) {
    GemmArgs a = {};
    a.A = dY; a.B = X; a.M = Mo; a.N = No; a.K = rows; a.lda = ldy; a.ldb = ldx;
    a.C = nullptr; a.ldc = ldw; a.C2 = nullptr; a.Cf = dW; a.bias = nullptr; a.colsum = nullptr; a.R = nullptr; a.ldr = 0;
    a.alpha = 1.0f; a.drop = kNoDrop; a.kchunk = rows; a.dbg = 0; a.reg_m = a.reg_n = a.tpr_m = a.tpr_n = 0;
    return a;
}

inline int wgrad(int dtype, int Mo, int No, int rows, const void* dY, int ldy, const void* X, int ldx, float* dW, int ldw,
          hipStream_t st) {
    const long t128 = (long)((Mo + 127) / 128) * ((No + 127) / 128);
    const long t64 = (long)((Mo + 63) / 64) * ((No + 63) / 64);
    int tile, splits;
    if (t128 >= 256) { tile = 128; splits = 1; }
    else if (t64 >= 100) { tile = 64; splits = 1; }
    else { tile = 64; splits = (int)((256 + t64 - 1) / t64); }
    if (splits > 8) splits = 8;
    while (splits > 1 && rows / splits < 128) --splits;
    if (splits < 1) splits = 1;
    (void)t128;
    return gemm(dtype, GEMM_TN, EPI_ACCUM_F32, Mo, No, rows, dY, ldy, X, ldx, nullptr, ldw, nullptr, dW, nullptr, nullptr, 0,
                kNoDrop, splits, tile, st);
}

struct StepGraph {
    int B, L, with_opt, overwrite; const void *logits, *loss, *loss_run, *m, *v; float loss_scale; hipStream_t st;
    int nseg;
    int variant;
    const void* tag;
    std::vector<hipGraph_t> graph; std::vector<hipGraphExec_t> exec;
    size_t ridden = 0, swept = 0; int segments = 0;
    size_t frozen = 0; int wgrad_skipped = 0, embed_skipped = 0;
    int clip = 0;
    void destroy() {
        for (auto x : exec) if (x) hipGraphExecDestroy(x);
        for (auto g : graph) if (g) hipGraphDestroy(g);
        exec.clear(); graph.clear();
    }
};

struct StageGraph { int B, L, stage, overwrite; const void *logits, *loss, *loss_run; float loss_scale; hipStream_t st; hipGraph_t graph; hipGraphExec_t exec; };

struct StepMixin {
    bool dyn = false;
    bool stage_mode = false;
    std::vector<StageGraph> stage_graphs;
    bool pk_enable = false, packed = false;
    bool pkw_enable = false, packed_w = false;
    PrologueArgs::MagPackW pkw = {};
    size_t pk_vis = 0, pk_aco = 0; int pk_Vp = 0, pk_Ap = 0, pk_dtype = 0;
    void read_env() {
        ow_enable = env_int("MB_WGRAD_OVERWRITE", ow_enable);
        keep_enable = env_int("MB_ADAMW_KEEP", keep_enable);
        deterministic = env_int("MB_DETERMINISTIC", deterministic);
        pk_enable = env_on("MB_PROLOGUE_PACK", true);
        pkw_enable = env_on("MB_PROLOGUE_PACKW", true);
    }
    size_t idcnt_off = 0; bool idcnt_enable = false, counted = false;
    size_t live_off = 0, live_cap = 0; bool live_enable = false, live_built = false; int live_mode = 0, live_launches = 0;
    uint32_t* live_rows(char* ws) const { return (uint32_t*)(ws + live_off); }
    uint32_t* live_count(char* ws) const { return live_rows(ws) + live_cap; }
    uint32_t* cls_rows(char* ws) const { return live_rows(ws) + live_cap + 8; }
    uint32_t* cls_count(char* ws) const { return cls_rows(ws) + live_cap; }
    size_t stamp_off = 0, stamp_rows = 0; bool stamp_enable = false, stamp_live = false, word_zero = false;
    uint32_t sweep_no = 1;
    size_t skip_updates = 0;
    uint32_t* stamp_table(char* ws) const { return (uint32_t*)(ws + stamp_off); }
    uint32_t* stamp_state(char* ws) const { return stamp_table(ws) + stamp_rows; }
    bool one_sweep = false;
    bool loss_cleared = false;
    bool capturing = false;
    int nsites = 0;
    size_t ws_state = 0, ws_in_ids = 0, ws_in_seg = 0, ws_in_mask = 0, ws_in_vis = 0, ws_in_aco = 0, ws_in_lab = 0;
    std::vector<StepGraph> graphs;
    size_t graph_launches = 0, graph_captures = 0;
    hipStream_t cap = nullptr;
    int capture_stream(hipStream_t* out) {
        if (!cap) CK((int)hipStreamCreateWithFlags(&cap, hipStreamNonBlocking));
        *out = cap;
        return MB_OK;
    }
    bool grads_zero = false, ow_pass = false, in_step = false;
    int ow_enable = 1;
    int deterministic = 0;
    size_t ws_det = 0, det_begin = 0, det_end = 0;
    GradAcc acc_of(char* ws, const float* G) const {
        GradAcc a = {nullptr, nullptr};
        if (deterministic && ws && G) { a.shadow = (long long*)(ws + ws_det) - det_begin; a.base = G; }
        return a;
    }
    int cus = 0;
    int cu_count() {
        if (cus <= 0) {
            int dev = 0, n = 0;
            if (hipGetDevice(&dev) == hipSuccess && hipDeviceGetAttribute(&n, hipDeviceAttributeMultiprocessorCount, dev) == hipSuccess) cus = n;
            if (cus <= 0) cus = 256;
        }
        return cus;
    }
    bool grads_stale = false, ow_covers = false;
    size_t stale_begin = 0, stale_end = 0;
    int keep_enable = 1;
    bool keep_in_step() const { return keep_enable && ow_enable && ow_covers && stale_end > stale_begin; }
    int materialize_grads(float* G, hipStream_t st) {
        if (grads_stale && G) CK(zero_fill(G + stale_begin, (stale_end - stale_begin) * sizeof(float), st));
        grads_stale = false;
        return MB_OK;
    }
    int begin_backward_pass(float* G, hipStream_t st) {
        if (in_step) return MB_OK;
        stamp_live = word_zero = false;
        frz_dirty = true;
        ow_pass = grads_zero && ow_enable;
        grads_zero = false;
        if (!(ow_pass && ow_covers)) CK(materialize_grads(G, st));
        grads_stale = false;
        return MB_OK;
    }

    bool prof = false;
    std::vector<hipEvent_t> pev;
    int prof_layers = 0;
    int set_profiling(int on, int layers) {
        if (on && pev.empty()) {
            prof_layers = layers;
            pev.assign((size_t)2 * layers + 2, nullptr);
            for (auto& ev : pev) CK((int)hipEventCreate(&ev));
        }
        prof = on != 0;
        return MB_OK;
    }
    int prof_mark(int idx, hipStream_t st) { return (prof && !capturing && idx < (int)pev.size()) ? (int)hipEventRecord(pev[idx], st) : 0; }
    int prof_span_us(int first, int pairs, float* avg_us) {
        if (!prof || !avg_us || pev.empty()) return MB_ERR_ARG;
        double sum = 0.0;
        for (int i = 0; i < pairs; ++i) {
            float ms = 0.f;
            CK((int)hipEventSynchronize(pev[first + 2 * i + 1]));
            CK((int)hipEventElapsedTime(&ms, pev[first + 2 * i], pev[first + 2 * i + 1]));
            sum += ms;
        }
        *avg_us = (float)(sum * 1e3 / pairs);
        return MB_OK;
    }
    void destroy_prof() { for (auto& ev : pev) if (ev) hipEventDestroy(ev); pev.clear(); }

    void carve_step(Carver& w, size_t Tpad, int V, int A, int max_batch, int num_labels, int nsites_) {
        nsites = nsites_;
        ws_state = w.take(2 * sizeof(AdamArgs) + (size_t)nsites * 8);
        ws_in_ids = w.take(Tpad * 8); ws_in_seg = w.take(Tpad * 8); ws_in_mask = w.take(Tpad * 8);
        ws_in_vis = w.take(Tpad * (size_t)V * 4); ws_in_aco = w.take(Tpad * (size_t)A * 4);
        ws_in_lab = w.take((size_t)max_batch * num_labels * 4);
    }
    void drop_graphs() {
        if (cap) { hipStreamDestroy(cap); cap = nullptr; }
        for (auto& g : graphs) g.destroy();
        graphs.clear();
        for (auto& g : stage_graphs) { hipGraphExecDestroy(g.exec); hipGraphDestroy(g.graph); }
        stage_graphs.clear();
    }
    template <class Enq>
    int run_stage_graph(int B, int L, int stage, int overwrite, const void* logits, const void* loss, const void* loss_run, float loss_scale,
                        int mode, hipStream_t st, Enq enqueue) {
        struct Scope { StepMixin* m; ~Scope() { m->dyn = false; m->capturing = false; m->in_step = false; m->stage_mode = false; } } scope{this};
        dyn = true; in_step = true; stage_mode = true;
        stamp_live = word_zero = false;
        frz_dirty = true;
        if (mode == 2) return enqueue(st);
        StageGraph* g = nullptr;
        for (auto& x : stage_graphs)
            if (x.B == B && x.L == L && x.stage == stage && x.overwrite == overwrite && x.logits == logits && x.loss == loss && x.loss_run == loss_run &&
                x.loss_scale == loss_scale && x.st == st) { g = &x; break; }
        if (!g) {
            if (stage_graphs.size() >= 256) {
                hipGraphExecDestroy(stage_graphs.front().exec); hipGraphDestroy(stage_graphs.front().graph);
                stage_graphs.erase(stage_graphs.begin());
            }
            StageGraph ng = {B, L, stage, overwrite, logits, loss, loss_run, loss_scale, st, nullptr, nullptr};
            hipStream_t cs = nullptr;
            CK(capture_stream(&cs));
            CK((int)hipStreamBeginCapture(cs, hipStreamCaptureModeRelaxed));
            capturing = true;
            const int r = enqueue(cs);
            capturing = false;
            const int r2 = (int)hipStreamEndCapture(cs, &ng.graph);
            if (r) { if (ng.graph) hipGraphDestroy(ng.graph); return r; }
            CK(r2);
            CK((int)hipGraphInstantiate(&ng.exec, ng.graph, nullptr, nullptr, 0));
            stage_graphs.push_back(ng);
            g = &stage_graphs.back();
            ++graph_captures;
        }
        CK((int)hipGraphLaunch(g->exec, st));
        ++graph_launches;
        return MB_OK;
    }
    AdamArgs* adam_state(char* ws) const { return (AdamArgs*)(ws + ws_state); }
    struct ClassVals { float lr, beta1, beta2, eps, weight_decay; int correct_bias; };
    int n_classes = 0, map_version = 0;
    std::vector<size_t> seg_bounds;
    std::vector<int> seg_class;
    std::vector<uint8_t> seg_nodecay, seg_frozen;
    bool any_frozen = false, frz_dirty = true;
    std::vector<std::pair<size_t, size_t>> frz_unwritten;
    size_t ride_hopped = 0;
    size_t frz_elems = 0; int frz_wgrad_skipped = 0, frz_embed_skipped = 0;
    std::vector<ClassVals> class_vals;
    AdamArgs* class_table = nullptr;
    size_t upd_ridden = 0, upd_swept = 0; int upd_segments = 0;
    int ensure_class_table() {
        if (!class_table) {
            CK((int)hipMalloc((void**)&class_table, (size_t)2 * MB_CLASSES_MAX * sizeof(AdamArgs)));
            CK((int)hipMemset(class_table, 0, (size_t)2 * MB_CLASSES_MAX * sizeof(AdamArgs)));
        }
        return MB_OK;
    }
    void free_class_table() { if (class_table) { hipFree(class_table); class_table = nullptr; } }
    AdamArgs* class_state(char*) const { return class_table; }
    float clip_max = 0.f;
    bool clip_step = false;
    bool clip_ran = false;
    char* clip_buf = nullptr; size_t clip_cap = 0;
    float* clip_record() const { return (float*)clip_buf; }
    float* clip_params() const { return (float*)clip_buf + 2; }
    double* clip_partials() const { return (double*)(clip_buf + 256); }
    int ensure_clip_buf(size_t n) {
        const size_t need = 256 + (size_t)grad_norm_blocks(n) * sizeof(double);
        if (clip_buf && need > clip_cap) return MB_ERR_ARG;
        if (!clip_buf) { CK((int)hipMalloc((void**)&clip_buf, need)); clip_cap = need; }
        return MB_OK;
    }
    void free_clip_buf() { if (clip_buf) { hipFree(clip_buf); clip_buf = nullptr; clip_cap = 0; } }
    int set_grad_clip(float max_norm) {
        const float v = (std::isfinite(max_norm) && max_norm > 0.f) ? max_norm : 0.f;
        if ((v > 0.f) != (clip_max > 0.f)) clip_ran = false;
        clip_max = v;
        return MB_OK;
    }
    int grad_clip_stats(float* norm, float* coef, hipStream_t st) const {
        if (!(clip_max > 0.f) || !clip_ran || !clip_buf) return MB_ERR_MODE;
        float rec[2] = {0.f, 0.f};
        CK((int)hipStreamSynchronize(st));
        CK((int)hipMemcpy(rec, clip_record(), sizeof rec, hipMemcpyDeviceToHost));
        if (norm) *norm = rec[0];
        if (coef) *coef = rec[1];
        return MB_OK;
    }
    int enqueue_clip(const float* G, size_t n, char* ws, hipStream_t st) {
        unsigned blocks = grad_norm_blocks(n);
        if (any_frozen) {
            AdamPieces tr;
            CK(sweep_pieces(tr, 0, n, n, n, false));
            CK(grad_sumsq_pieces(G, tr, clip_partials(), &blocks, st));
        } else
        CK(grad_sumsq(G, n, clip_partials(), st));
        ClipTables t = {{adam_state(ws), n_classes > 0 ? class_state(ws) : nullptr}, {2, n_classes > 0 ? MB_CLASSES_MAX + n_classes : 0}};
        return grad_clip_finalize(clip_partials(), blocks, clip_params(), 0.f, 1.f, clip_record(), t, st);
    }
    int set_update_map(const std::vector<TensorInfo>& tensors, size_t n_update_end, int nc, int ns, const size_t* bounds, const int* classes) {
        if (nc == 0) {
            n_classes = 0; seg_bounds.clear(); seg_class.clear(); seg_nodecay.clear(); class_vals.clear();
            if (any_frozen) marks_changed();
            seg_frozen.clear(); any_frozen = false;
            return MB_OK;
        }
        if (nc < 0 || nc > MB_CLASSES_MAX || ns < 1 || ns > MB_SEGMENTS_MAX || !bounds || !classes) return MB_ERR_ARG;
        if (bounds[0] != 0 || bounds[ns] != n_update_end) return MB_ERR_SHAPE;
        for (int s = 0; s < ns; ++s) {
            if (bounds[s + 1] <= bounds[s]) return MB_ERR_SHAPE;
            if (classes[s] < 0 || classes[s] >= nc) return MB_ERR_ARG;
            bool at_tensor = false;
            for (const auto& t : tensors) if (t.off == bounds[s]) { at_tensor = true; break; }
            if (!at_tensor) return MB_ERR_SHAPE;
        }
        const bool same = nc == n_classes && (int)seg_class.size() == ns && std::equal(classes, classes + ns, seg_class.begin()) &&
                          std::equal(bounds, bounds + ns + 1, seg_bounds.begin());
        const bool marked = any_frozen || std::any_of(seg_nodecay.begin(), seg_nodecay.end(), [](uint8_t x) { return x != 0; });
        if (same && !marked) return MB_OK;
        if (any_frozen) marks_changed();
        if (!same) class_vals.clear();
        n_classes = nc; seg_bounds.assign(bounds, bounds + ns + 1); seg_class.assign(classes, classes + ns);
        seg_nodecay.assign((size_t)ns, 0);
        seg_frozen.assign((size_t)ns, 0); any_frozen = false;
        if (++map_version <= 0) map_version = 1;
        return MB_OK;
    }
    int set_update_decay(int ns, const uint8_t* no_decay) {
        if (n_classes == 0) return MB_ERR_MODE;
        if (ns != (int)seg_class.size() || !no_decay) return MB_ERR_ARG;
        bool same = true;
        for (int s = 0; s < ns; ++s) same = same && (no_decay[s] != 0) == (seg_nodecay[s] != 0);
        if (same) return MB_OK;
        for (int s = 0; s < ns; ++s) seg_nodecay[s] = no_decay[s] ? 1 : 0;
        if (++map_version <= 0) map_version = 1;
        return MB_OK;
    }
    void marks_changed() { frz_dirty = true; stamp_live = word_zero = false; }
    int set_update_frozen(int ns, const uint8_t* frozen) {
        if (n_classes == 0) return MB_ERR_MODE;
        if (ns != (int)seg_class.size() || !frozen) return MB_ERR_ARG;
        bool same = true;
        for (int s = 0; s < ns; ++s) same = same && (frozen[s] != 0) == (seg_frozen[s] != 0);
        if (same) return MB_OK;
        any_frozen = false;
        for (int s = 0; s < ns; ++s) { seg_frozen[s] = frozen[s] ? 1 : 0; any_frozen = any_frozen || frozen[s]; }
        marks_changed();
        if (++map_version <= 0) map_version = 1;
        return MB_OK;
    }
    int freeze_stats(size_t* frozen_elems, int* wgrad_launches_skipped, int* embed_skipped) const {
        if (frozen_elems) *frozen_elems = frz_elems;
        if (wgrad_launches_skipped) *wgrad_launches_skipped = frz_wgrad_skipped;
        if (embed_skipped) *embed_skipped = frz_embed_skipped;
        return MB_OK;
    }
    size_t frozen_total() const {
        size_t n = 0;
        for (size_t s = 0; s + 1 < seg_bounds.size(); ++s) if (seg_frozen[s]) n += seg_bounds[s + 1] - seg_bounds[s];
        return n;
    }
    bool range_frozen(size_t b, size_t e) const {
        if (!any_frozen || e <= b || seg_bounds.empty() || e > seg_bounds.back()) return false;
        size_t s = (size_t)(std::upper_bound(seg_bounds.begin(), seg_bounds.end(), b) - seg_bounds.begin()) - 1;
        for (; s + 1 < seg_bounds.size() && seg_bounds[s] < e; ++s) if (!seg_frozen[s]) return false;
        return true;
    }
    bool skipping() const { return any_frozen && in_step && !stage_mode; }
    bool unwritten(size_t b, size_t e) const {
        for (const auto& u : frz_unwritten) if (u.first <= b && e <= u.second) return true;
        return false;
    }
    void begin_step_marks() {
        frz_unwritten.clear(); ride_hopped = 0; frz_wgrad_skipped = frz_embed_skipped = 0;
        frz_elems = any_frozen ? frozen_total() : 0;
    }
    void note_unwritten(size_t b, size_t e) {
        if (e <= b) return;
        if (!frz_unwritten.empty() && frz_unwritten.back().second == b) frz_unwritten.back().second = e;
        else frz_unwritten.push_back({b, e});
        std::sort(frz_unwritten.begin(), frz_unwritten.end());
    }
    int clear_frozen(float* G, hipStream_t st) {
        for (size_t s = 0; s + 1 < seg_bounds.size(); ++s)
            if (seg_frozen[s]) CK(zero_fill(G + seg_bounds[s], (seg_bounds[s + 1] - seg_bounds[s]) * sizeof(float), st));
        frz_dirty = false;
        return MB_OK;
    }
    int seg_slot(size_t s) const { return seg_class[s] + (seg_nodecay[s] ? MB_CLASSES_MAX : 0); }
    int set_update_values(int nc, const float* lr, const float* beta1, const float* beta2, const float* eps, const float* weight_decay,
                          const int* correct_bias) {
        if (nc < 1 || nc != n_classes || !lr || !beta1 || !beta2 || !eps || !weight_decay || !correct_bias) return MB_ERR_ARG;
        class_vals.resize((size_t)nc);
        for (int c = 0; c < nc; ++c) class_vals[c] = ClassVals{lr[c], beta1[c], beta2[c], eps[c], weight_decay[c], correct_bias[c]};
        return MB_OK;
    }
    int update_stats(size_t* ridden, size_t* swept, int* segments) const {
        if (ridden) *ridden = upd_ridden;
        if (swept) *swept = upd_swept;
        if (segments) *segments = upd_segments;
        return MB_OK;
    }
    bool ride_segment(size_t& cursor, size_t limit, size_t* floor, int* cls) {
        while (cursor > limit) {
            const size_t s = (size_t)(std::upper_bound(seg_bounds.begin(), seg_bounds.end(), cursor - 1) - seg_bounds.begin()) - 1;
            if (!seg_frozen[s]) { *floor = seg_bounds[s]; *cls = seg_slot(s); return true; }
            const size_t lo = std::max(seg_bounds[s], limit);
            if (!unwritten(lo, cursor)) return false;
            ride_hopped += cursor - lo; cursor = lo;
        }
        return false;
    }
    int sweep_pieces(AdamPieces& out, size_t b0, size_t e0, size_t b1, size_t e1, bool clear = true, size_t keep_b = 0, size_t keep_e = 0) const {
        std::vector<int> slots(seg_class.size());
        for (size_t s = 0; s < slots.size(); ++s) slots[s] = seg_slot(s);
        return cut_pieces(out, seg_bounds, slots.data(), seg_frozen.empty() ? nullptr : seg_frozen.data(), b0, e0, b1, e1, clear, keep_b, keep_e);
    }
    int cut_pieces(AdamPieces& out, const std::vector<size_t>& bounds, const int* slot, const uint8_t* frozen, size_t b0, size_t e0, size_t b1,
                   size_t e1, bool clear = true, size_t keep_b = 0, size_t keep_e = 0) const {
        out = AdamPieces{};
        const size_t rb[2] = {b0, b1}, re[2] = {e0, e1};
// ... 79 lines not shown
        if (!head_loss_legal(HeadLoss{kind, param, nullptr, in.label_smoothing, in.focal_gamma, ignore, has_ignore}, num_labels)) return MB_ERR_ARG;
        if (kind < HL_DEFAULT || kind > HL_CE) return MB_ERR_ARG;
        if (kind == HL_CE && num_labels < 2) return MB_ERR_ARG;
        if (kind == HL_SMOOTH_L1 && !(std::isfinite(param) && param >= 0.f)) return MB_ERR_ARG;
        const bool takes_vec = kind == HL_BCE || kind == HL_CE;
        if (vec && !takes_vec) return MB_ERR_ARG;
        if (vec) {
            bool any = false;
            for (int k = 0; k < num_labels; ++k) {
                if (!(std::isfinite(vec[k]) && vec[k] >= 0.f)) return MB_ERR_ARG;
                any = any || vec[k] > 0.f;
            }
            if (!any) return MB_ERR_ARG;
        }
        if (kind != HL_SMOOTH_L1) param = 0.f;
        std::vector<float> nv;
        if (vec) nv.assign(vec, vec + num_labels);
        if (kind == loss_kind && param == loss_param && nv == loss_vec && in.label_smoothing == loss_smoothing && in.focal_gamma == loss_gamma &&
            has_ignore == loss_has_ignore && ignore == loss_ignore) return MB_OK;
        if (!graphs.empty() || !stage_graphs.empty()) { CK((int)hipDeviceSynchronize()); drop_graphs(); }
        loss_kind = kind; loss_param = param;
        loss_smoothing = in.label_smoothing; loss_gamma = in.focal_gamma; loss_has_ignore = has_ignore; loss_ignore = ignore;
        loss_vec_dirty = loss_vec_dirty || nv != loss_vec;
        loss_vec.swap(nv);
        return MB_OK;
    }
    int get_head_loss(int* kind, float* param, float* vec, int* has_vec) const {
        if (kind) *kind = loss_kind;
        if (param) *param = loss_param;
        if (has_vec) *has_vec = loss_vec.empty() ? 0 : 1;
        if (vec) std::copy(loss_vec.begin(), loss_vec.end(), vec);
        return MB_OK;
    }
    int get_head_loss_ex(mb_head_loss* hl, float* vec, int* has_vec) const {
        if (hl) *hl = mb_head_loss{loss_kind, loss_param, nullptr, loss_smoothing, loss_gamma, loss_has_ignore, loss_ignore};
        return get_head_loss(nullptr, nullptr, vec, has_vec);
    }
    int sync_head_loss() {
        if (!loss_vec_dirty || capturing) return MB_OK;
        if (!loss_vec.empty()) {
            if (loss_vec_cap < loss_vec.size()) {
                if (loss_vec_dev) { CK((int)hipDeviceSynchronize()); hipFree(loss_vec_dev); loss_vec_dev = nullptr; loss_vec_cap = 0; }
                CK((int)hipMalloc((void**)&loss_vec_dev, loss_vec.size() * sizeof(float)));
                loss_vec_cap = loss_vec.size();
            }
            CK((int)hipDeviceSynchronize());
            CK((int)hipMemcpy(loss_vec_dev, loss_vec.data(), loss_vec.size() * sizeof(float), hipMemcpyHostToDevice));
        }
        loss_vec_dirty = false;
        return MB_OK;
    }
    void free_head_loss() { if (loss_vec_dev) { hipFree(loss_vec_dev); loss_vec_dev = nullptr; loss_vec_cap = 0; } }
    void staged(char* ws, bool with_labels, const void** six) const {
        six[0] = ws + ws_in_ids; six[1] = ws + ws_in_vis; six[2] = ws + ws_in_aco; six[3] = ws + ws_in_mask; six[4] = ws + ws_in_seg;
        six[5] = with_labels ? ws + ws_in_lab : nullptr;
    }
};

struct NoBetween { int operator()(int, hipStream_t) const { return MB_OK; } };
template <class E, class Enqueue, class Between = NoBetween>
inline int train_step_impl(E* e, char* ws, int V, int A, int num_labels, const void* ids, const void* vis, const void* aco, const void* mask,
                           const void* seg, const void* labels, int B, int L, uint64_t seed, uint64_t step, float* logits, float* loss,
                           float* loss_run, float* m, float* v, float lr, float beta1, float beta2, float eps, float weight_decay,
                           int opt_step, int correct_bias, float grad_scale, float loss_scale, int mode, bool force_launches,
                           hipStream_t st, Enqueue enqueue_inner, int nseg = 1, Between between = Between(), int variant = 0,
                           const void* tag = nullptr, int (*verify)(const void* tag, int nseg, int sg, hipGraph_t gr) = nullptr) {
    if (m && e->n_classes > 0 && (int)e->class_vals.size() != e->n_classes) return MB_ERR_ARG;
    if (m && e->n_classes > 0 && variant == 0) variant = -e->map_version;
    if (e->any_frozen && variant > 0) return MB_ERR_MODE;
    if (e->any_frozen && variant == 0) variant = -e->map_version;
    e->upd_ridden = e->upd_swept = 0; e->upd_segments = 0;
    e->live_launches = 0;
    e->frz_elems = 0; e->frz_wgrad_skipped = e->frz_embed_skipped = 0;
    if (e->any_frozen && e->frz_dirty) CK(e->clear_frozen(e->G, st));
    if (m && e->n_classes > 0) CK(e->ensure_class_table());
    CK(e->sync_head_loss());
    const bool clip = m && e->clip_max > 0.f;
    if (clip && variant > 0) return MB_ERR_MODE;
    if (clip) CK(e->ensure_clip_buf(e->n_update_end()));
    const int ow = (e->grads_zero && e->ow_enable) ? 1 : 0;
    if (!(ow && e->ow_covers)) CK(e->materialize_grads(e->G, st));
    const bool stale_before = e->grads_stale;
    struct Flags {
        E* e; bool ok, with_opt, stale_before;
        ~Flags() {
            e->in_step = false; e->loss_cleared = false; e->packed = false; e->packed_w = false; e->counted = false; e->live_built = false;
            if (ok && e->clip_step) e->clip_ran = true;
            e->clip_step = false;
            e->grads_zero = ok && with_opt;
            e->grads_stale = ok ? (with_opt && e->keep_in_step()) : stale_before;
            if (ok && with_opt && e->stamp_live) ++e->skip_updates;
            if (!ok || with_opt) e->stamp_live = false;
            e->word_zero = ok && with_opt;
            if (ok && with_opt && ++e->sweep_no == 0u) e->sweep_no = 1u;
        }
    } flags{e, false, m != nullptr, stale_before};
    const bool no_embed = e->any_frozen && e->embed_all_frozen();
    const bool stamping = e->stamp_off != 0 && e->stamp_enable && e->idcnt_enable && ids != nullptr && !no_embed;
    if (!stamping) e->stamp_live = false;
    else if (e->word_zero) e->stamp_live = true;
    e->word_zero = false;
    e->in_step = true; e->ow_pass = ow != 0; e->clip_step = clip;
    auto enqueue = [&](int sg, float* lg, float* ls, float* lr_, float* m_, float* v_, float sc, hipStream_t s) {
        return enqueue_inner(sg, lg, ls, lr_, m_, v_, sc, s);
    };
    PrologueArgs pa = {};
    e->fill_copies(pa, ws, ids, vis, aco, mask, seg, labels, B, L, V, A, num_labels, e->pk_enable);
    e->packed = e->pk_enable;
    if (e->pkw_enable && e->pkw.W_hv) pa.magw = e->pkw;
    e->packed_w = pa.magw.W_hv != nullptr;
    pa.seed = seed; pa.step = step; pa.keys = e->key_state(ws); pa.nsites = e->nsites;
    pa.zero_dw = (uint32_t*)loss; e->loss_cleared = loss != nullptr;
    if (e->idcnt_enable && ids && !no_embed) { pa.ids = (const int64_t*)ids; pa.n_ids = B * L; pa.id_count = (int*)(ws + e->idcnt_off); }
    e->counted = pa.id_count != nullptr;
    if (stamping) { pa.stamp = e->stamp_table(ws); pa.stamp_state = e->stamp_state(ws); pa.stamp_no = e->sweep_no; pa.stamp_on = e->stamp_live ? 1u : 0u; }
    if (e->live_off != 0 && e->live_enable && variant <= 0 && mask != nullptr && (size_t)align_up((size_t)B * L, 64) <= e->live_cap &&
        B <= MB_LIVE_MAX_SAMPLES && B * L <= MB_LIVE_MAX_ROWS) {
        pa.live_rows = e->live_rows(ws); pa.live_count = e->live_count(ws); pa.live_mask = (const int64_t*)mask;
        pa.live_T = B * L; pa.live_Tp = (int)align_up((size_t)B * L, 64); pa.live_L = L;
        if (e->live_mode >= 2) { pa.cls_rows = e->cls_rows(ws); pa.cls_count = e->cls_count(ws); }
        e->live_built = true;
    }
    if (m) {
        double ss = lr;
        if (correct_bias) ss = (double)lr * sqrt(1.0 - pow((double)beta2, (double)opt_step)) / (1.0 - pow((double)beta1, (double)opt_step));
        AdamArgs a;
        a.lr = lr; a.beta1 = beta1; a.beta2 = beta2; a.eps = eps; a.weight_decay = weight_decay; a.step_size = (float)ss;
        a.grad_scale = grad_scale;
        pa.adam[0] = a;
        a.weight_decay = 0.f;
        pa.adam[1] = a;
        pa.adam_dst = e->adam_state(ws);
        for (int c = 0; c < e->n_classes; ++c) {
            const auto& cv = e->class_vals[c];
            double cs = cv.lr;
            if (cv.correct_bias) cs = (double)cv.lr * sqrt(1.0 - pow((double)cv.beta2, (double)opt_step)) / (1.0 - pow((double)cv.beta1, (double)opt_step));
            AdamArgs k;
            k.lr = cv.lr; k.beta1 = cv.beta1; k.beta2 = cv.beta2; k.eps = cv.eps; k.weight_decay = cv.weight_decay; k.step_size = (float)cs;
            k.grad_scale = grad_scale;
            pa.cls[c] = k;
        }
        if (e->n_classes > 0) { pa.ncls = e->n_classes; pa.cls_dst = e->class_state(ws); }
        if (clip) { pa.clip[0] = e->clip_max; pa.clip[1] = grad_scale; pa.clip_dst = e->clip_params(); }
    }
    CK(step_prologue(pa, st));
    if (mode == 2 || force_launches) {
        e->dyn = true;
        int r = MB_OK;
        for (int sg = 0; sg < nseg && r == MB_OK; ++sg) {
            r = enqueue(sg, logits, loss, loss_run, m, v, loss_scale, st);
            if (r == MB_OK) r = between(sg, st);
        }
        e->dyn = false;
        flags.ok = r == MB_OK;
        return r;
    }
    StepGraph* g = nullptr;
    for (auto& x : e->graphs)
        if (x.B == B && x.L == L && x.with_opt == (m != nullptr) && x.overwrite == ow && x.logits == logits && x.loss == loss && x.loss_run == loss_run &&
            x.m == m && x.v == v && x.loss_scale == loss_scale && x.st == st && x.nseg == nseg && x.variant == variant && x.tag == tag &&
            x.clip == (clip ? 1 : 0)) { g = &x; break; }
    if (!g) {
        if (e->graphs.size() >= 32) {
            e->graphs.front().destroy();
            e->graphs.erase(e->graphs.begin());
        }
        StepGraph ng = {B, L, m != nullptr, ow, logits, loss, loss_run, m, v, loss_scale, st, nseg, variant, tag, {}, {}};
        ng.clip = clip ? 1 : 0;
        hipStream_t cs = nullptr;
        CK(e->capture_stream(&cs));
        for (int sg = 0; sg < nseg; ++sg) {
            hipGraph_t gr = nullptr;
            hipGraphExec_t ex = nullptr;
            CK((int)hipStreamBeginCapture(cs, hipStreamCaptureModeRelaxed));
            e->dyn = true; e->capturing = true;
            const int r = enqueue(sg, logits, loss, loss_run, m, v, loss_scale, cs);
            e->dyn = false; e->capturing = false;
            const int r2 = (int)hipStreamEndCapture(cs, &gr);
            if (r || r2) { mb::ck_trace(r ? "enqueue(segment) inside the capture" : "hipStreamEndCapture", __FILE__, __LINE__, r ? r : r2);
                           if (gr) hipGraphDestroy(gr); ng.destroy(); return r ? r : r2; }
            if (verify) { const int rv = verify(tag, nseg, sg, gr); if (rv) { mb::ck_trace("finish(segment graph)", __FILE__, __LINE__, rv); hipGraphDestroy(gr); ng.destroy(); return rv; } }
            const int r3 = (int)hipGraphInstantiate(&ex, gr, nullptr, nullptr, 0);
            if (r3) { mb::ck_trace("hipGraphInstantiate", __FILE__, __LINE__, r3); hipGraphDestroy(gr); ng.destroy(); return r3; }
            ng.graph.push_back(gr); ng.exec.push_back(ex);
        }
        ng.ridden = e->upd_ridden; ng.swept = e->upd_swept; ng.segments = e->upd_segments;
        ng.frozen = e->frz_elems; ng.wgrad_skipped = e->frz_wgrad_skipped; ng.embed_skipped = e->frz_embed_skipped;
        e->graphs.push_back(ng);
        g = &e->graphs.back();
        ++e->graph_captures;
    }
    for (int sg = 0; sg < nseg; ++sg) {
        CK((int)hipGraphLaunch(g->exec[sg], st));
        CK(between(sg, st));
    }
    ++e->graph_launches;
    e->upd_ridden = g->ridden; e->upd_swept = g->swept; e->upd_segments = g->segments;
    e->frz_elems = g->frozen; e->frz_wgrad_skipped = g->wgrad_skipped; e->frz_embed_skipped = g->embed_skipped;
    flags.ok = true;
    return MB_OK;
}

inline int mag_clear_pad_rows(int dtype, char* ws, const MagWs& w, int T, int H, hipStream_t st) {
    const size_t Tp = align_up((size_t)T, 64), es = esize(dtype);
    if (Tp == (size_t)T) return MB_OK;
    auto zp = [&](size_t off, size_t cols) { return (int)hipMemsetAsync(ws + off + (size_t)T * cols * es, 0, (Tp - T) * cols * es, st); };
    CK(zp(w.vp, w.Vp)); CK(zp(w.ap, w.Ap));
    CK(zp(w.dZe, 2 * (size_t)H)); CK(zp(w.dZv, 2 * (size_t)H)); CK(zp(w.dZa, 2 * (size_t)H));
    return MB_OK;
}
inline int mag_fwd_impl(int dtype, const void* text, const float* visual, const float* acoustic, const float* W_hv,
                 const float* b_hv, const float* W_ha, const float* b_ha, const float* W_v, const float* b_v,
                 const float* W_a, const float* b_a, const float* ln_w, const float* ln_b, float ln_eps, float beta_shift,
                 DropKey drop, void* out, char* ws, const MagWs& w, int T, int H, int V, int A, bool repack, hipStream_t st,
                 bool pads_clean = false, bool packed = false) {
    MagDims d = {T, H, V, A, w.Vp, w.Ap};
    if (repack) CK(mag_pack_weights(dtype, W_hv, W_ha, W_v, W_a, ws + w.We, ws + w.Wv, ws + w.Wa, d, st));
    if (!packed) {
        CK(pack_pad(dtype, visual, V, ws + w.vp, w.Vp, T, st));
        CK(pack_pad(dtype, acoustic, A, ws + w.ap, w.Ap, T, st));
    }
    if (!pads_clean) {
        const int Tp = (int)align_up((size_t)T, 64);
        const size_t es = esize(dtype);
        if (Tp > T) {
            ZeroRanges z = {};
            z.add(ws + w.vp + (size_t)T * w.Vp * es, (size_t)(Tp - T) * w.Vp * es);
// ... 96 lines not shown
```

### bert_multimodal_transformer_amd/csrc/kernels.h

```cpp
#pragma once
#include <cstdio>
#include <cstdlib>
#include "common.h"

namespace mb {

enum {
    MB_OK = 0,
    MB_ERR_SHAPE = 1001,
    MB_ERR_MODE = 1002,
    MB_ERR_DTYPE = 1003,
    MB_ERR_ARG = 1004,
    MB_ERR_COMM = 1005,
};

inline void ck_trace(const char* expr, const char* file, int line, int code) {
    static int on = -1;
    if (on < 0) { const char* v = getenv("MB_CK_TRACE"); on = (v && atoi(v)) ? 1 : 0; }
    if (on) fprintf(stderr, "[magbert] %s:%d: %s -> %d\n", file, line, expr, code);
}

enum { GEMM_NT = 0,
       GEMM_NN = 1,
       GEMM_TN = 2 };
// ... 119 lines not shown
                      MagDims d, DropKey drop, hipStream_t st, GradAcc acc = {},
                      float* part_a = nullptr, float* part_b = nullptr, int* nblk = nullptr);

int attention_forward(int dtype, const void* qkv, const int64_t* mask, void* ctx, int B, int L, int nh,
                      DropKey drop, hipStream_t st, float* probs = nullptr, const float* head_scale = nullptr,
                      float* stats = nullptr);
int attention_backward(int dtype, const void* qkv, const int64_t* mask, const void* ctx, const void* dctx,
                       void* dqkv, float* dbias, int B, int L, int nh, DropKey drop, hipStream_t st,
                       const float* head_scale = nullptr, GradAcc acc = {},
                       const struct AdamRide* ride = nullptr,
                       float* stats = nullptr);
size_t tiled_stats_floats(int B, int L, int nh);
int attention_tiled_forward(int dtype, const void* qkv, const int64_t* mask, void* ctx, float* stats, int B, int L, int nh,
                            DropKey drop, hipStream_t st, float* probs = nullptr, const float* head_scale = nullptr);
int attention_tiled_backward(int dtype, const void* qkv, const int64_t* mask, const void* ctx, const void* dctx, float* stats,
                             void* dqkv, float* dbias, int B, int L, int nh, DropKey drop, hipStream_t st,
                             const float* head_scale = nullptr, GradAcc acc = {}, const struct AdamRide* ride = nullptr);
int attention_backward_free_slots(int dtype, int L, int nblk, int cus);
int attention_trace_fetch(unsigned long long* host_out, int max_blocks);

int xlnet_attention_forward(int dtype, const void* qkv, const void* kr, const float* r_w_bias, const float* r_r_bias,
                            const float* r_s_bias, const float* seg_embed, const int64_t* seg, const int64_t* mask, void* vec,
                            void* psave, int B, int L, int nh, DropKey drop, hipStream_t st, const float* head_scale = nullptr,
                            const uint8_t* perm = nullptr,
                            int gstream = 0,
                            float* stats = nullptr);
int xlnet_attention_backward(int dtype, const void* qkv, const void* kr, const float* r_w_bias, const float* r_r_bias,
                             const float* r_s_bias, const float* seg_embed, const int64_t* seg, const int64_t* mask,
                             const void* psave, const void* dvec, void* gsave, void* dqkv, void* dkr, float* d_rwb,
                             float* d_rrb, float* d_rsb, float* d_seg, int B, int L, int nh, DropKey drop, hipStream_t st,
                             const float* head_scale = nullptr,
                             GradAcc acc = {},
                             const struct AdamRide* ride_q = nullptr, const struct AdamRide* ride_kv = nullptr,
                             const void* vec = nullptr, const float* stats = nullptr, void* pdsave = nullptr,
                             const uint8_t* perm = nullptr);
int xlnet_attention_backward_free_slots(int dtype, int L, int nblk, int cus);
size_t xlnet_tiled_stats_floats(int B, int L, int nh);
size_t xlnet_tiled_scratch_elems(int B, int L, int nh);
int xlnet_attention_tiled_forward(int dtype, const void* qkv, const void* kr, const float* r_w_bias, const float* r_r_bias,
                                  const float* r_s_bias, const float* seg_embed, const int64_t* seg, const int64_t* mask, void* vec,
                                  float* stats, int B, int L, int nh, DropKey drop, hipStream_t st, const float* head_scale = nullptr,
                                  const uint8_t* perm = nullptr, int gstream = 0, float* probs = nullptr);
int xlnet_attention_tiled_backward(int dtype, const void* qkv, const void* kr, const float* r_w_bias, const float* r_r_bias,
                                   const float* r_s_bias, const float* seg_embed, const int64_t* seg, const int64_t* mask,
                                   const void* vec, const void* dvec, const float* stats, void* gsave, void* pdsave, void* dqkv, void* dkr,
                                   float* d_rwb, float* d_rrb, float* d_rsb, float* d_seg, int B, int L, int nh, DropKey drop,
                                   hipStream_t st, const float* head_scale = nullptr, const uint8_t* perm = nullptr, GradAcc acc = {});
int gather_drop_forward(int dtype, const int64_t* ids, const float* word, void* out, int rows, int H, DropKey drop, hipStream_t st);
int gather_drop_backward(int dtype, const void* dout, const int64_t* ids, float* dword, int rows, int H, DropKey drop, hipStream_t st, GradAcc acc = {});
int add_f32(float* dst, const float* src, size_t n, hipStream_t st);
int drop_rows(int dtype, const void* x, void* y, int rows, int H, DropKey drop, hipStream_t st);
int xlnet_pos_emb(int dtype, void* out, int B, int L, int H, DropKey drop, hipStream_t st);
int last_token_forward(int dtype, const void* x, void* xs, int B, int L, int H, DropKey drop, hipStream_t st);
int last_token_backward(int dtype, const void* dxs, void* dx, int B, int L, int H, DropKey drop, hipStream_t st);
int xlnet_broadcast_row(int dtype, const float* row, void* out, int rows, int H, hipStream_t st);
int xlnet_map_query(int dtype, const float* tm, const void* qg, const void* qkv_h, void* qkv_g, int B, int M, int L, int H, hipStream_t st);
int xlnet_unmap_vec(int dtype, const float* tm, const void* vec, void* vecg, int B, int M, int L, int H, hipStream_t st);

enum { HL_DEFAULT = 0, HL_MSE = 1, HL_L1 = 2, HL_SMOOTH_L1 = 3, HL_BCE = 4, HL_CE = 5 };
struct HeadLoss { int kind; float param; const float* vec; float smoothing; float gamma; int ignore; int has_ignore; };
inline bool head_loss_modified(const HeadLoss& hl) { return hl.smoothing != 0.f || hl.gamma != 0.f || hl.has_ignore != 0; }
inline bool head_loss_legal(const HeadLoss& hl, int nl) {
    if (hl.kind < HL_DEFAULT || hl.kind > HL_CE || (hl.kind == HL_CE && nl < 2)) return false;
    if (!(hl.smoothing >= 0.f && hl.smoothing < 1.f)) return false;
    if (!(hl.gamma == 0.f || (hl.gamma >= 1.f && hl.gamma <= 3.402823466e38f))) return false;
    if (hl.smoothing > 0.f && hl.gamma > 0.f) return false;
    if ((hl.smoothing > 0.f || hl.has_ignore) && hl.kind != HL_CE) return false;
    if (hl.gamma > 0.f && hl.kind != HL_CE && hl.kind != HL_BCE) return false;
    return true;
}
inline bool head_loss_per_element(int kind) { return kind >= HL_MSE && kind <= HL_BCE; }
int head_forward(const float* z, const float* Wc, const float* bc, const float* labels, float* pooled,
                 float* logits, float* loss, float* loss_run, int B, int H, int nl, DropKey drop, hipStream_t st,
                 HeadLoss hl = HeadLoss{HL_DEFAULT, 0.f, nullptr});
int head_backward(int dtype, const float* dlogits, const float* logits, const float* labels, float loss_scale,
                  const float* pooled, const float* Wc, void* dz, float* dWc, float* dbc,
                  int B, int H, int nl, DropKey drop, hipStream_t st, GradAcc acc = {}, float* dbp = nullptr,
                  void* zero_p = nullptr, size_t zero_bytes = 0,
                  HeadLoss hl = HeadLoss{HL_DEFAULT, 0.f, nullptr});

int adamw_step(float* p, float* g, float* m, float* v, void* shadow, size_t n, size_t n_decay,
               size_t sh_begin, size_t sh_end, AdamArgs a, int zero_grad, hipStream_t st, const AdamArgs* dyn = nullptr,
               size_t keep_begin = 0, size_t keep_end = 0);
struct WordSkip { const uint32_t* stamp; const uint32_t* state; size_t begin, end; uint32_t row_len; };
#define MB_CLASSES_MAX 32
#define MB_SEGMENTS_MAX 128
#define MB_SWEEP_PIECES_MAX (MB_SEGMENTS_MAX + 2)
#define MB_PIECE_CLEAR 0xff
struct AdamPieces { uint32_t begin4[MB_SWEEP_PIECES_MAX], start4[MB_SWEEP_PIECES_MAX + 1]; uint8_t slot[MB_SWEEP_PIECES_MAX]; int count, clear_first; };
int adamw_sweep(float* p, float* g, float* m, float* v, void* shadow, const AdamPieces& r, size_t sh_begin, size_t sh_end,
                size_t keep_begin, size_t keep_end, const AdamArgs* cls, const WordSkip& skip, hipStream_t st);

unsigned grad_norm_blocks(size_t n);
int grad_sumsq(const float* g, size_t n, double* partial, hipStream_t st);
int grad_sumsq_pieces(const float* g, const AdamPieces& r, double* partial, unsigned* blocks, hipStream_t st);
struct ClipTables { AdamArgs* tab[2]; int count[2]; };
int grad_clip_finalize(const double* partial, unsigned blocks, const float* dyn, float max_norm, float grad_scale, float* out2,
                       const ClipTables& t, hipStream_t st);

#define MB_PROLOGUE_MAX_COPIES 8
#define MB_LIVE_MAX_SAMPLES 8192
#define MB_LIVE_MAX_ROWS 65536
struct PrologueArgs {
    const uint32_t* src[MB_PROLOGUE_MAX_COPIES]; uint32_t* dst[MB_PROLOGUE_MAX_COPIES]; uint32_t dwords[MB_PROLOGUE_MAX_COPIES];
    int ncopies;
    uint64_t seed, step;
    uint32_t* keys; int nsites;
    AdamArgs adam[2]; AdamArgs* adam_dst;
    AdamArgs cls[MB_CLASSES_MAX]; AdamArgs* cls_dst; int ncls;
    float clip[2]; float* clip_dst;
    uint32_t* zero_dw;
    struct PackJob { const float* src; void* dst; int rows, cols, pitch, dtype; } pack[2];
    int npack;
    const int64_t* ids; int n_ids; int* id_count;
    uint32_t* stamp; uint32_t* stamp_state; uint32_t stamp_no, stamp_on;
    uint32_t* live_rows; uint32_t* live_count; const int64_t* live_mask; int live_T, live_Tp, live_L;
    uint32_t* cls_rows; uint32_t* cls_count;
    struct MagPackW { const float* W_hv; const float* W_ha; const float* W_v; const float* W_a; void* We; void* Wv; void* Wa; MagDims d; int dtype; } magw;
    int copy_blocks;
};
static_assert(sizeof(PrologueArgs) <= 2048, "PrologueArgs travels as kernel arguments (4 KB limit)");
int step_prologue(const PrologueArgs& a, hipStream_t st);
#define MB_ZERO_MAX 8
struct ZeroRanges {
    uint32_t* p[MB_ZERO_MAX]; size_t ndw[MB_ZERO_MAX]; int n;
    void add(void* ptr, size_t bytes) { if (bytes && n < MB_ZERO_MAX) { p[n] = (uint32_t*)ptr; ndw[n] = bytes / 4; ++n; } }
    bool full() const { return n >= MB_ZERO_MAX; }
};
int zero_fill(void* p, size_t bytes, hipStream_t st);
int zero_fill_ranges(const ZeroRanges& z, hipStream_t st);

}
```

### bert_multimodal_transformer_amd/csrc/rowops.hip

```cpp
#include <algorithm>
#include "kernels.h"
#include "mag_pack.h"

namespace mb {

template <int CH>
struct RowStat {
    static __device__ __forceinline__ void compute(const f32x4 (&v)[CH], float eps, float& mu, float& rs) {
        constexpr float invH = 1.0f / (CH * 256);
        float s = 0.f;
#pragma unroll
        for (int c = 0; c < CH; ++c) s += (v[c][0] + v[c][1]) + (v[c][2] + v[c][3]);
        mu = wave_sum(s) * invH;
        float q = 0.f;
#pragma unroll
        for (int c = 0; c < CH; ++c) {
#pragma unroll
            for (int r = 0; r < 4; ++r) { const float d = v[c][r] - mu; q += d * d; }
        }
        rs = 1.0f / sqrtf(wave_sum(q) * invH + eps);
    }
};

template <class T, int CH>
// ... 703 lines not shown
        int64_t w[16];
#pragma unroll
        for (int k = 0; k < 16; ++k) w[k] = base + k < r1 ? __builtin_nontemporal_load(a.live_mask + base + k) : 0;
#pragma unroll
        for (int k = 0; k < 16; ++k)
            if (w[k] != 0) {
                const int r = base + k, b = r / L;
                atomicOr(&real[b >> 5], 1u << (b & 31));
                atomicOr(&mbit[r >> 5], 1u << (r & 31));
            }
    }
    __syncthreads();
    auto is_live = [&](int r) {
        const int b = r / L;
        return ((mbit[r >> 5] >> (r & 31)) & 1u) || r == b * L || !((real[b >> 5] >> (b & 31)) & 1u);
    };
    uint32_t n = 0, dead = 0xffffffffu;
    for (int r = r0; r < r1; ++r) {
        if (is_live(r)) ++n;
        else if (dead == 0xffffffffu) dead = (uint32_t)r;
    }
    cnt[t] = n;
    __syncthreads();
    if (dead != 0xffffffffu) atomicMin(&first_dead, dead);
    for (int d = 1; d < 256; d <<= 1) {
        const uint32_t v = t >= d ? cnt[t - d] : 0u;
        __syncthreads();
        cnt[t] += v;
        __syncthreads();
    }
    const uint32_t total = cnt[255];
    uint32_t o = cnt[t] - n;
    for (int r = r0; r < r1; ++r)
        if (is_live(r)) a.live_rows[o++] = (uint32_t)r;
    uint32_t pad = first_dead;
    const bool have_pad = pad != 0xffffffffu || T < a.live_Tp;
    if (pad == 0xffffffffu) pad = T < a.live_Tp ? (uint32_t)T : 0u;
    const uint32_t count = max(192u, (total + 63u) / 64u * 64u);
    for (uint32_t i = total + t; i < count; i += 256) a.live_rows[i] = pad;
    if (t == 0) *a.live_count = count;
    if (a.cls_rows != nullptr) {
        const uint32_t nb = (uint32_t)(T / L);
        if (have_pad) {
            const uint32_t cc = max(192u, (nb + 63u) / 64u * 64u);
            for (uint32_t i = t; i < cc; i += 256) a.cls_rows[i] = i < nb ? i * (uint32_t)L : pad;
            if (t == 0) *a.cls_count = cc;
        } else {
            for (uint32_t i = t; i < count; i += 256) a.cls_rows[i] = i < total ? i : pad;
            if (t == 0) *a.cls_count = count;
        }
    }
}

__global__ void __launch_bounds__(256) step_prologue_kernel(const PrologueArgs a) {
    if (a.live_rows != nullptr && blockIdx.x == gridDim.x - 1) { live_rows_block(a); return; }
    if ((int)blockIdx.x >= a.copy_blocks) {
        const size_t first = (size_t)(blockIdx.x - a.copy_blocks) * 256 + threadIdx.x,
                     stride = (size_t)(gridDim.x - a.copy_blocks - (a.live_rows != nullptr ? 1 : 0)) * 256;
        const PrologueArgs::MagPackW& w = a.magw;
        if (w.dtype == DT_BF16) mag_pack_w_range<bf16>(w.W_hv, w.W_ha, w.W_v, w.W_a, (bf16*)w.We, (bf16*)w.Wv, (bf16*)w.Wa, w.d, first, stride);
        else mag_pack_w_range<float>(w.W_hv, w.W_ha, w.W_v, w.W_a, (float*)w.We, (float*)w.Wv, (float*)w.Wa, w.d, first, stride);
        return;
    }
    const size_t tid = (size_t)blockIdx.x * 256 + threadIdx.x, nth = (size_t)a.copy_blocks * 256;
    if (blockIdx.x == 0) {
        for (int s = threadIdx.x; s < a.nsites; s += 256) {
            const uint64_t h = splitmix64_dev(splitmix64_dev(a.seed) ^ splitmix64_dev(a.step * 0x100000001B3ull + (uint64_t)s));
            a.keys[2 * s] = (uint32_t)h;
            a.keys[2 * s + 1] = (uint32_t)(h >> 32);
        }
        if (a.adam_dst && threadIdx.x < 2) a.adam_dst[threadIdx.x] = a.adam[threadIdx.x];
        if (a.cls_dst && (int)threadIdx.x < a.ncls) {
            AdamArgs k = a.cls[threadIdx.x];
            a.cls_dst[threadIdx.x] = k;
            k.weight_decay = 0.f;
            a.cls_dst[MB_CLASSES_MAX + threadIdx.x] = k;
        }
        if (a.clip_dst && threadIdx.x < 2) a.clip_dst[threadIdx.x] = a.clip[threadIdx.x];
    }
    if (tid == 0 && a.zero_dw) *a.zero_dw = 0u;
    if (a.id_count != nullptr)
        for (size_t i = tid; i < (size_t)a.n_ids; i += nth) atomicAdd(a.id_count + a.ids[i], 1);
    if (a.stamp != nullptr) {
        for (size_t i = tid; i < (size_t)a.n_ids; i += nth) a.stamp[a.ids[i]] = a.stamp_no;
        if (tid < 2) a.stamp_state[tid] = tid == 0 ? a.stamp_no : a.stamp_on;
    }
    for (int k = 0; k < a.npack; ++k) {
        const PrologueArgs::PackJob& j = a.pack[k];
        const size_t n = (size_t)j.rows * j.cols;
        if ((((uintptr_t)j.src) & 15) == 0) {
            for (size_t i = tid; i < (n + 3) / 4; i += nth) {
                const size_t e0 = i * 4;
                f32x4 v = {0.f, 0.f, 0.f, 0.f};
                if (e0 + 4 <= n) v = __builtin_nontemporal_load((const f32x4*)j.src + i);
                else for (int r = 0; r < 4; ++r) if (e0 + r < n) v[r] = j.src[e0 + r];
                size_t row = e0 / j.cols;
                int c = (int)(e0 - row * j.cols);
#pragma unroll
                for (int r = 0; r < 4; ++r) {
                    if (e0 + r < n) {
                        const size_t d = row * j.pitch + c;
                        if (j.dtype == DT_BF16) ((bf16*)j.dst)[d] = from_f<bf16>(v[r]); else ((float*)j.dst)[d] = v[r];
                    }
                    if (++c == j.cols) { c = 0; ++row; }
                }
            }
        } else {
            for (size_t e = tid; e < n; e += nth) {
                const size_t row = e / j.cols, d = row * j.pitch + (e - row * j.cols);
                if (j.dtype == DT_BF16) ((bf16*)j.dst)[d] = from_f<bf16>(j.src[e]); else ((float*)j.dst)[d] = j.src[e];
            }
        }
    }
    size_t most4 = 0;
    bool fast = true;
    for (int c = 0; c < MB_PROLOGUE_MAX_COPIES; ++c)
        if (c < a.ncopies) {
            fast = fast && ((((uintptr_t)a.src[c] | (uintptr_t)a.dst[c]) & 15) == 0);
            if (a.dwords[c] / 4 > most4) most4 = a.dwords[c] / 4;
        }
    if (fast) {
        for (size_t i = tid; i < most4; i += nth) {
            u32x4 v[MB_PROLOGUE_MAX_COPIES];
#pragma unroll
            for (int c = 0; c < MB_PROLOGUE_MAX_COPIES; ++c)
                if (c < a.ncopies && i < a.dwords[c] / 4) v[c] = __builtin_nontemporal_load((const u32x4*)a.src[c] + i);
#pragma unroll
            for (int c = 0; c < MB_PROLOGUE_MAX_COPIES; ++c)
                if (c < a.ncopies && i < a.dwords[c] / 4) ((u32x4*)a.dst[c])[i] = v[c];
        }
#pragma unroll 1
        for (int c = 0; c < a.ncopies; ++c) {
            const size_t n = a.dwords[c];
            for (size_t i = (n / 4) * 4 + tid; i < n; i += nth) a.dst[c][i] = a.src[c][i];
        }
        return;
    }
#pragma unroll 1
    for (int c = 0; c < a.ncopies; ++c) {
        const uint32_t* __restrict__ src = a.src[c];
        uint32_t* __restrict__ dst = a.dst[c];
        const size_t n = a.dwords[c];
        for (size_t i = tid; i < n; i += nth) dst[i] = src[i];
    }
}

int step_prologue(const PrologueArgs& a, hipStream_t st) {
    if (a.ncopies < 0 || a.ncopies > MB_PROLOGUE_MAX_COPIES || a.nsites < 0 || (a.nsites > 0 && !a.keys)) return MB_ERR_ARG;
    if (a.npack < 0 || a.npack > 2 || a.ncls < 0 || a.ncls > MB_CLASSES_MAX) return MB_ERR_ARG;
    if (a.stamp && (!a.stamp_state || !a.ids)) return MB_ERR_ARG;
    size_t most = 0;
    for (int k = 0; k < a.npack; ++k) {
        if (!a.pack[k].src || !a.pack[k].dst || a.pack[k].cols < 1 || a.pack[k].pitch < a.pack[k].cols) return MB_ERR_ARG;
        most = std::max(most, (size_t)a.pack[k].rows * a.pack[k].cols);
    }
    for (int c = 0; c < a.ncopies; ++c) {
        if (a.dwords[c] && (!a.src[c] || !a.dst[c])) return MB_ERR_ARG;
        if (a.dwords[c] > most) most = a.dwords[c];
    }
    unsigned grid = (unsigned)((most / 4 + 255) / 256);
    if (grid < 1) grid = 1;
    if (grid > 512) grid = 512;
    PrologueArgs b = a;
    b.copy_blocks = (int)grid;
    if (a.magw.W_hv != nullptr) {
        if (!a.magw.W_ha || !a.magw.W_v || !a.magw.W_a || !a.magw.We || !a.magw.Wv || !a.magw.Wa) return MB_ERR_ARG;
        if (a.magw.dtype != DT_BF16 && a.magw.dtype != DT_F32) return MB_ERR_DTYPE;
        grid += 256;
    }
    if (a.live_rows != nullptr) {
        if (!a.live_count || !a.live_mask || a.live_T < 1 || a.live_Tp < a.live_T || a.live_L < 1 || a.live_T % a.live_L ||
            a.live_T / a.live_L > MB_LIVE_MAX_SAMPLES || a.live_T > MB_LIVE_MAX_ROWS || (a.cls_rows && !a.cls_count))
            return MB_ERR_ARG;
        grid += 1;
    }
    hipLaunchKernelGGL(step_prologue_kernel, dim3(grid), dim3(256), 0, st, b);
    return (int)hipGetLastError();
}


__global__ void __launch_bounds__(256) grad_fold_kernel(long long* __restrict__ shadow, float* __restrict__ g, size_t begin, size_t end) {
    for (size_t i = begin + (size_t)blockIdx.x * 256 + threadIdx.x; i < end; i += (size_t)gridDim.x * 256) {
        const long long v = shadow[i];
        if (v != 0) {
            g[i] += (float)((double)v * (1.0 / (double)kGradFix));
            shadow[i] = 0;
        }
    }
}
int grad_fold(GradAcc acc, float* g, size_t begin, size_t end, hipStream_t st) {
    if (!acc.shadow || end <= begin) return MB_OK;
    if (g != acc.base) return MB_ERR_ARG;
    const size_t n = end - begin;
    hipLaunchKernelGGL(grad_fold_kernel, dim3((unsigned)std::min<size_t>((n + 255) / 256, 4096)), dim3(256), 0, st, acc.shadow, g, begin, end);
    return (int)hipGetLastError();
}

}
```

### bert_multimodal_transformer_amd/optimization.py

```python
import math
import os

import numpy as np
import torch

from . import _lib

UPDATE_CLASSES_MAX = 32
UPDATE_SEGMENTS_MAX = 128


FROZEN = -1


def plan_update_segments(tensors, group_of_tensor, n_update_end, frozen=False):
    if len(tensors) != len(group_of_tensor):
        return None
    rows = sorted((int(t[1]), int(t[2]), g) for t, g in zip(tensors, group_of_tensor) if int(t[1]) < n_update_end)
    boundaries, classes = [], []
    cursor = 0
    for off, numel, g in rows:
        if isinstance(g, (list, tuple, set, frozenset)):
            if len(g) > 1 or (len(g) == 0 and not frozen):
                return None
            g = next(iter(g)) if g else None
        if g is None and frozen:
            g = FROZEN
        elif g is not None and frozen and int(g) < 0:
            return None
        if g is None or off != cursor or numel < 1:
            return None
        cursor = (off + numel + 63) // 64 * 64
        if not classes or classes[-1] != g:
            boundaries.append(off)
            classes.append(int(g))
    if cursor != n_update_end or not classes:
        return None
    boundaries.append(int(n_update_end))
    real = set(classes) - ({FROZEN} if frozen else set())
    if not real or len(real) > UPDATE_CLASSES_MAX or len(classes) > UPDATE_SEGMENTS_MAX:
        return None
    if frozen:
        return boundaries, classes, [1 if c == FROZEN else 0 for c in classes]
    return boundaries, classes


def pair_update_groups(hyper, hints=None):
    decaying, zero = {}, {}
    for g, (lr, betas, eps, correct_bias, wd) in enumerate(hyper):
        key = (float(lr), tuple(float(b) for b in betas), float(eps), bool(correct_bias))
        (zero if float(wd) == 0.0 else decaying).setdefault(key, []).append(g)
    partner = {}
    for key, gs in decaying.items():
        free = list(zero.get(key, []))
        if hints is not None:
            for g in gs:
                z = next((z for z in free if hints[g] is not None and hints[z] == hints[g]), None)
                if z is not None:
                    partner[g], partner[z] = z, g
                    free.remove(z)
        for g, z in zip([g for g in gs if g not in partner], free):
            partner[g], partner[z] = z, g
    class_of, no_decay, members = [None] * len(hyper), [False] * len(hyper), []
    for g in range(len(hyper)):
        if class_of[g] is not None:
            continue
        class_of[g] = len(members)
        other = partner.get(g)
        if other is None:
            members.append((g, None))
            continue
        class_of[other] = len(members)
        carrier, z = (other, g) if float(hyper[g][4]) == 0.0 else (g, other)
        no_decay[z] = True
        members.append((carrier, z))
    return class_of, no_decay, members


def plan_paired_segments(tensors, group_of_tensor, n_update_end, class_of_group, no_decay_of_group, frozen=False):
    if len(tensors) != len(group_of_tensor):
        return None
    rows = sorted((int(t[1]), int(t[2]), g) for t, g in zip(tensors, group_of_tensor) if int(t[1]) < n_update_end)
    boundaries, classes, flags = [], [], []
    cursor = 0
    for off, numel, g in rows:
        if isinstance(g, (list, tuple, set, frozenset)):
            if len(g) > 1 or (len(g) == 0 and not frozen):
                return None
            g = next(iter(g)) if g else None
        if off != cursor or numel < 1:
            return None
        if g is None and frozen:
# ... 204 lines not shown
        if id(core) not in self._class_maps:
            owner = {}
            for gi, group in enumerate(self.param_groups):
                for p in group["params"]:
                    info = getattr(p, "_mb_flat", None)
                    if info is not None and info[0] is core:
                        owner.setdefault(info[1], set()).add(gi)
            n_end = getattr(core, "n_update_end", core.n_params)
            owners = [owner.get(t[1]) for t in core.tensors]
            planned = plan_update_segments(core.tensors, owners, n_end, frozen=True)
            if planned is not None:
                groups = sorted(set(planned[1]) - {FROZEN})
                self._class_frozen[id(core)] = planned[2] if any(planned[2]) else None
                planned = (planned[0], [0 if g == FROZEN else groups.index(g) for g in planned[1]], groups, None, [(g, None) for g in groups])
            else:
                class_of, no_decay, members = pair_update_groups([self._hyper(g) for g in self.param_groups],
                                                                 hints=[g.get("initial_lr") for g in self.param_groups])
                paired = plan_paired_segments(core.tensors, owners, n_end, class_of, no_decay, frozen=True)
                if paired is not None:
                    used = sorted(set(paired[1]) - {FROZEN})
                    planned = (paired[0], [0 if c == FROZEN else used.index(c) for c in paired[1]], [members[c][0] for c in used], paired[2],
                               [members[c] for c in used])
                    self._class_frozen[id(core)] = paired[3] if any(paired[3]) else None
            self._class_maps[id(core)] = planned
        return self._class_maps[id(core)]

    def flat_step_args(self, core, allow_dp=False):
        if (self._dp is not None and not allow_dp) or not self.fused_zero_grad:
            return None
        if allow_dp and self._clip_value() > 0.0:
            return None
        if self._plan is None:
            self._build_plan()
        flats = [it for it in self._plan if it[0] == "flat"]
        loose = [it for it in self._plan if it[0] != "flat"]
        if any(it[2].grad is not None for it in loose):
            return None
        two = self._two_group_args(core, flats)
        if two is not None or self._dp is not None or not flats or any(it[2] is not core for it in flats):
            if two is not None:
                two["max_grad_norm"] = self._clip_value()
            return two
        planned = self._class_map(core)
        if planned is not None and not self._pairs_hold(planned[4]):
            del self._class_maps[id(core)]
            planned = self._class_map(core)
        if planned is None:
            return None
        boundaries, classes, groups, no_decay, _ = planned
        frozen = self._class_frozen.get(id(core))
        gs = [self.param_groups[g] for g in groups]
        marks = {} if no_decay is None else {"no_decay": list(no_decay)}
        if frozen is not None:
            marks["frozen"] = list(frozen)
        return dict(m=core._adam_m, v=core._adam_v, grad_scale=float(self.grad_scale), map=(boundaries, classes),
                    max_grad_norm=self._clip_value(), **marks,
                    classes=dict(lr=[float(g["lr"]) for g in gs], beta1=[float(g["betas"][0]) for g in gs],
                                 beta2=[float(g["betas"][1]) for g in gs], eps=[float(g["eps"]) for g in gs],
                                 weight_decay=[float(g["weight_decay"]) for g in gs],
                                 correct_bias=[1 if g["correct_bias"] else 0 for g in gs]))

    def _two_group_args(self, core, flats):
        if len(flats) != 2 or any(it[2] is not core for it in flats):
            return None
        (_, g0, _, a0, b0), (_, g1, _, a1, b1) = sorted(flats, key=lambda it: it[3])
        if (a0, b0, a1, b1) != (0, core.n_decay, core.n_decay, getattr(core, "n_update_end", core.n_params)):
            return None
        ga, gb = self.param_groups[g0], self.param_groups[g1]
        if any(ga[k] != gb[k] for k in ("lr", "betas", "eps", "correct_bias")) or gb["weight_decay"] != 0.0:
            return None
        return dict(m=core._adam_m, v=core._adam_v, lr=float(ga["lr"]), beta1=float(ga["betas"][0]), beta2=float(ga["betas"][1]),
                    eps=float(ga["eps"]), weight_decay=float(ga["weight_decay"]), correct_bias=bool(ga["correct_bias"]),
                    grad_scale=float(self.grad_scale))

    @torch.no_grad()
    def step(self, closure=None):
        loss = closure() if closure is not None else None
        if self._plan is None:
            self._build_plan()
        L = _lib.lib()
        self._t += 1
        for core, _ in self._covers.values():
            core.materialize_grads()
        dp = self._dp
        late = []
        if dp is not None and getattr(dp, "late_ranges", None):
            late = sorted(dp.late_ranges)

        shards = getattr(dp, "shards", None) if dp is not None else None
        grad_scale = self.grad_scale
        if self._clip_value() > 0.0:
            if shards is not None or getattr(dp, "shard_in_engine", False) or (dp is not None and os.environ.get("MB_DP_SHARD_OPT", "0") == "1"):
                raise _lib.MagbertError("max_grad_norm with MB_DP_SHARD_OPT=1: a rank holds only its shard of the reduced gradient, "
                                        "the norm would need a cross-rank sum -- not supported")
            if dp is not None:
                dp.finish()
                late = []
            norm, coef = self._clip_coef(L)
            grad_scale = float(np.float32(self.grad_scale) * np.float32(coef))
            self._clip_last = (norm, coef)

        def launch(core, group, x, y):
            if shards is not None and core is shards.core and x < shards.hi and y > shards.lo:
                pieces = [(x, min(y, shards.lo)), (max(x, shards.a), min(y, shards.b)), (max(x, shards.hi), y)]
                for px, py in pieces:
                    if py > px:
                        launch_range(core, group, px, py)
                return
            launch_range(core, group, x, y)

        def launch_range(core, group, x, y):
            if y <= x:
                return
            b1, b2 = group["betas"]
            sh = core.shadow if core.dt == _lib.DT_BF16 else None
            sb = min(max(core.sh_begin, x), y) - x
            se = min(max(core.sh_end, x), y) - x
            _lib.check(L.mb_adamw_step(
                core.params.data_ptr() + 4 * x, core.grads.data_ptr() + 4 * x, core._adam_m.data_ptr() + 4 * x,
                core._adam_v.data_ptr() + 4 * x, (sh.data_ptr() + 2 * x) if sh is not None else None, y - x,
                (y - x) if group["weight_decay"] > 0.0 else 0, sb, se, group["lr"], b1, b2, group["eps"],
                group["weight_decay"], self._t, 1 if group["correct_bias"] else 0, grad_scale,
                1 if self.fused_zero_grad else 0, core.stream()))

        deferred = []
        for item in self._plan:
            group = self.param_groups[item[1]]
            b1, b2 = group["betas"]
            if item[0] == "flat":
                _, _, core, a, b = item
                cur = a
                for lo, n in late:
                    hi = lo + n
                    if hi <= cur or lo >= b or core is not dp.core:
                        continue
                    launch(core, group, cur, max(cur, lo))
                    deferred.append((core, group, max(cur, lo), min(b, hi)))
                    cur = min(b, hi)
                launch(core, group, cur, b)
            else:
                p = item[2]
                if p.grad is None:
                    continue
                if not p.is_cuda or p.dtype != torch.float32 or not p.is_contiguous():
                    raise _lib.MagbertError("AdamW runs on the HIP kernel only: fp32 contiguous ROCm tensors required")
                state = self.state[p]
                if len(state) == 0:
                    state["exp_avg"] = torch.zeros_like(p)
                    state["exp_avg_sq"] = torch.zeros_like(p)
                g = p.grad.contiguous()
                n = p.numel()
                _lib.check(L.mb_adamw_step(p.data_ptr(), g.data_ptr(), state["exp_avg"].data_ptr(),
                                           state["exp_avg_sq"].data_ptr(), None, n, n if group["weight_decay"] > 0.0 else 0,
                                           0, 0, group["lr"], b1, b2, group["eps"], group["weight_decay"], self._t,
                                           1 if group["correct_bias"] else 0, grad_scale, 0,
                                           torch.cuda.current_stream(p.device).cuda_stream))
        if late:
            dp.finish()
            for core, group, x, y in deferred:
                launch(core, group, x, y)
        if shards is not None:
            shards.clear_dead_gradients()
            shards.gather_updated()
        if self.fused_zero_grad:
            self._mark_zero()
        return loss

    def state_dict(self):
        if self._plan is None:
            self._build_plan()
        sd = super().state_dict()
        cores = []
        for item in self._plan:
            if item[0] == "flat" and all(item[2] is not c for c in cores):
                cores.append(item[2])
        for c in cores:
            c.refresh_sharded_state(adam=True)
        sd["magbert"] = {"t": self._t,
                         "flat": [{"exp_avg": c._adam_m.detach().cpu(), "exp_avg_sq": c._adam_v.detach().cpu()} for c in cores]}
        return sd

    def load_state_dict(self, state_dict):
        state_dict = dict(state_dict)
        extra = state_dict.pop("magbert", None)
        super().load_state_dict(state_dict)
        self._plan = None
        self._build_plan()
        if extra is not None:
            self._t = int(extra["t"])
            cores = []
            for item in self._plan:
                if item[0] == "flat" and all(item[2] is not c for c in cores):
                    cores.append(item[2])
            if len(cores) != len(extra["flat"]):
                raise ValueError("optimizer checkpoint holds %d flat buffers, this optimizer has %d" % (len(extra["flat"]), len(cores)))
            for c, st in zip(cores, extra["flat"]):
                c._adam_m.copy_(st["exp_avg"])
                c._adam_v.copy_(st["exp_avg_sq"])

    def zero_grad(self, set_to_none=False):
        if self._plan is None:
            self._build_plan()
        done = set()
        for item in self._plan:
            if item[0] == "flat":
                core = item[2]
                if not self.fused_zero_grad and id(core) not in done:
                    core.grads.zero_()
                    core.mark_grads_zero(True)
                    done.add(id(core))
            else:
                p = item[2]
                if p.grad is not None:
                    p.grad.zero_()


def linear_schedule_lambda(current_step, num_warmup_steps, num_training_steps):
    if current_step < num_warmup_steps:
        return float(current_step) / float(max(1, num_warmup_steps))
    return max(0.0, float(num_training_steps - current_step) / float(max(1, num_training_steps - num_warmup_steps)))


def get_linear_schedule_with_warmup(optimizer, num_warmup_steps, num_training_steps, last_epoch=-1):
    return torch.optim.lr_scheduler.LambdaLR(
        optimizer, lambda s: linear_schedule_lambda(s, num_warmup_steps, num_training_steps), last_epoch)
```

### include/magbert_hip.h

```cpp
#ifndef MAGBERT_HIP_H
#define MAGBERT_HIP_H
#include <stddef.h>
#include <stdint.h>

#ifdef __cplusplus
extern "C" {
#endif

#define MB_DT_F32 0
#define MB_DT_BF16 1

typedef struct { uint32_t k0, k1, thresh; float scale; } mb_dropkey;

const char* mb_error_string(int code);
int mb_version(void);
void mb_make_dropkey(uint64_t seed, uint64_t step, uint32_t site, float p, mb_dropkey* out);


enum { MB_EPI_RELU = 7, MB_EPI_SWISH = 8, MB_EPI_GELU_NEW = 9, MB_EPI_MISH = 10 };
enum { MB_ACT_GELU = 0, MB_ACT_RELU = 1, MB_ACT_SWISH = 2, MB_ACT_GELU_NEW = 3, MB_ACT_MISH = 4 };
int mb_gemm(int dtype, int layout, int epilogue, int M, int N, int K, const void* A, int lda, const void* B, int ldb,
            void* C, int ldc, void* C2, float* Cf, const float* bias, const void* R, int ldr, float alpha,
            const mb_dropkey* drop, int splits, int tile, void* stream);

int mb_debug_gemm_trace(unsigned long long* host_out, int max_blocks);
int mb_debug_attention_trace(unsigned long long* host_out, int max_blocks);

int mb_debug_gemm_ex(int dtype, int layout, int epilogue, int M, int N, int K, const void* A, int lda, const void* B, int ldb,
                     void* C, int ldc, void* C2, float* Cf, const float* bias, const void* R, int ldr, float alpha,
                     const mb_dropkey* drop, int splits, int tile, int bseg, size_t bseg_stride, int cvalid, int overwrite,
                     long long* colsum_shadow, int fold, float* rp, float* rg, float* rm, float* rv, void* rshadow, size_t n4, int blocks,
                     int zero_grad, float lr, float beta1, float beta2, float eps, float weight_decay, int step, int correct_bias,
                     float grad_scale, void* adam_dev, int* ride_tiles, void* stream);
int mb_debug_gemm_grouped_ex(int dtype, int count, const int* M, const int* N, int K, const void* const* dY, const int* ldy,
                             const void* const* X, const int* ldx, float* const* dW, const int* ldw, const int* cvalid,
                             const int* overwrite, int tile, int stages, float* rp, float* rg, float* rm, float* rv, void* rshadow,
                             size_t n4, int blocks, int zero_grad, float lr, float beta1, float beta2, float eps, float weight_decay,
                             int step, int correct_bias, float grad_scale, void* adam_dev, void* stream);
int mb_debug_gemm_last_kernel(char* out, int cap);
int mb_debug_gemm_grouped_rows(int dtype, int count, const int* M, const int* N, int K, const void* const* dY, const int* ldy,
                               const void* const* X, const int* ldx, float* const* dW, const int* ldw, const int* overwrite, int tile,
                               const void* const* rows, const void* const* nrows, void* stream);
int mb_debug_live_rows(const int64_t* mask, int B, int L, int Tp, void* live_rows, void* live_count, void* cls_rows, void* cls_count,
                       void* stream);

int mb_gemm_grouped_wgrad(int dtype, int count, const int* M, const int* N, int K, const void* const* dY, const int* ldy,
                          const void* const* X, const int* ldx, float* const* dW, const int* ldw, int tile, void* stream);

int mb_narrow(int dtype, const float* src, void* dst, size_t n, void* stream);
int mb_widen(int dtype, const void* src, float* dst, size_t n, void* stream);

int mb_layernorm_forward(int dtype, const void* x, const float* gamma, const float* beta, float eps, void* y,
                         float* mean, float* rstd, int rows, int H, const mb_dropkey* drop, void* stream);
int mb_layernorm_backward(int dtype, const void* dy, const void* x, const float* gamma, const float* mean,
                          const float* rstd, void* dx, void* dx_drop, float* dgamma, float* dbeta, float* dbias,
                          int rows, int H, const mb_dropkey* drop_out, const mb_dropkey* drop_in, void* stream);

int mb_embed_forward(int dtype, const int64_t* ids, const int64_t* seg, const float* word, const float* pos,
                     const float* type, const float* gamma, const float* beta, float eps, void* out, float* mean,
                     float* rstd, int B, int L, int H, const mb_dropkey* drop, void* stream);
int mb_embed_backward(int dtype, const void* dout, const int64_t* ids, const int64_t* seg, const float* word,
                      const float* pos, const float* type, const float* gamma, const float* mean, const float* rstd,
                      float* dsum_ws, float* dword, float* dpos, float* dtype_, float* dgamma, float* dbeta, int B, int L,
                      int H, int pad_id, const mb_dropkey* drop, void* stream);

int mb_attention_forward(int dtype, const void* qkv, const int64_t* mask, void* ctx, int B, int L, int nh,
                         const mb_dropkey* drop, void* stream);
int mb_attention_backward(int dtype, const void* qkv, const int64_t* mask, const void* dctx, void* dqkv, int B, int L,
                          int nh, const mb_dropkey* drop, void* stream);
int mb_attention_resident_forward(int dtype, const void* qkv, const int64_t* mask, void* ctx, int B, int L, int nh,
                                  const mb_dropkey* drop, const float* head_scale, float* probs, void* stream);
int mb_attention_resident_backward(int dtype, const void* qkv, const int64_t* mask, const void* dctx, void* dqkv, float* dbias, int B,
                                   int L, int nh, const mb_dropkey* drop, const float* head_scale, void* stream);
size_t mb_attention_tiled_stats_bytes(int B, int L, int nh);
int mb_attention_tiled_forward(int dtype, const void* qkv, const int64_t* mask, void* ctx, float* stats, int B, int L, int nh,
                               const mb_dropkey* drop, const float* head_scale, float* probs, void* stream);
int mb_attention_tiled_backward(int dtype, const void* qkv, const int64_t* mask, const void* ctx, const void* dctx, float* stats,
                                void* dqkv, float* dbias, int B, int L, int nh, const mb_dropkey* drop, const float* head_scale,
                                void* stream);

enum { MB_LOSS_DEFAULT = 0, MB_LOSS_MSE = 1, MB_LOSS_L1 = 2, MB_LOSS_SMOOTH_L1 = 3, MB_LOSS_BCE = 4, MB_LOSS_CROSS_ENTROPY = 5 };
int mb_head_forward(const float* z, const float* Wc, const float* bc, const float* labels, float* pooled, float* logits, float* loss,
                    float* loss_run, int B, int H, int num_labels, const mb_dropkey* drop, int loss_kind, float loss_param,
                    const float* loss_vec, void* stream);
int mb_head_backward(int dtype, const float* dlogits, const float* logits, const float* labels, float loss_scale, const float* pooled,
                     const float* Wc, void* dz, float* dWc, float* dbc, float* dbp, void* zero_p, size_t zero_bytes, int B, int H,
                     int num_labels, const mb_dropkey* drop, int loss_kind, float loss_param, const float* loss_vec, void* stream);
typedef struct { int kind; float param; const float* vec; float label_smoothing; float focal_gamma; int has_ignore_index; int ignore_index; } mb_head_loss;
int mb_head_forward_ex(const float* z, const float* Wc, const float* bc, const float* labels, float* pooled, float* logits, float* loss,
                       float* loss_run, int B, int H, int num_labels, const mb_dropkey* drop, const mb_head_loss* hl, void* stream);
int mb_head_backward_ex(int dtype, const float* dlogits, const float* logits, const float* labels, float loss_scale, const float* pooled,
                        const float* Wc, void* dz, float* dWc, float* dbc, float* dbp, void* zero_p, size_t zero_bytes, int B, int H,
                        int num_labels, const mb_dropkey* drop, const mb_head_loss* hl, void* stream);

size_t mb_mag_workspace_bytes(int dtype, int T, int H, int V, int A);
int mb_mag_forward(int dtype, const void* text, const float* visual, const float* acoustic, const float* W_hv,
                   const float* b_hv, const float* W_ha, const float* b_ha, const float* W_v, const float* b_v,
                   const float* W_a, const float* b_a, const float* ln_w, const float* ln_b, float beta_shift,
                   const mb_dropkey* drop, void* out, void* ws, int T, int H, int V, int A, void* stream);
int mb_mag_backward(int dtype, const void* d_out, const void* text, const float* W_hv, const float* b_hv,
                    const float* W_ha, const float* b_ha, const float* W_v, const float* b_v, const float* W_a,
                    const float* b_a, const float* ln_w, float beta_shift, const mb_dropkey* drop, void* ws,
                    void* d_text, float* d_visual, float* d_acoustic, float* dW_hv, float* db_hv, float* dW_ha,
                    float* db_ha, float* dW_v, float* db_v, float* dW_a, float* db_a, float* dln_w, float* dln_b,
                    int T, int H, int V, int A, void* stream);
int mb_debug_mag_forward_ex(int dtype, const void* text, const float* visual, const float* acoustic, const float* W_hv,
                            const float* b_hv, const float* W_ha, const float* b_ha, const float* W_v, const float* b_v,
                            const float* W_a, const float* b_a, const float* ln_w, const float* ln_b, float beta_shift,
                            const mb_dropkey* drop, void* out, void* ws, int T, int H, int V, int A, int pads_clean, void* stream);
size_t mb_debug_mag_slab_bytes(int T, int H);
int mb_debug_mag_backward_ex(int dtype, const void* d_out, const void* text, const float* b_hv, const float* b_ha, const float* b_v,
                             const float* b_a, const float* ln_w, float beta_shift, const mb_dropkey* drop, void* ws, void* d_text,
                             float* d_visual, float* d_acoustic, float* dW_hv, float* db_hv, float* dW_ha, float* db_ha,
                             float* dW_v, float* db_v, float* dW_a, float* db_a, float* dln_w, float* dln_b, int T, int H, int V,
                             int A, int text_padded, int pads_clean, int slabs, float* slab_scratch, size_t slab_bytes, int dw_zero,
                             int* path, void* stream);

int mb_adamw_step(float* p, float* g, float* m, float* v, void* shadow, size_t n, size_t n_decay, size_t sh_begin,
                  size_t sh_end, float lr, float beta1, float beta2, float eps, float weight_decay, int step,
                  int correct_bias, float grad_scale, int zero_grad, void* stream);

size_t mb_grad_clip_scratch_bytes(size_t n);
int mb_grad_clip_coef(const float* g, size_t n, float max_norm, float grad_scale, void* scratch, float* out2, void* stream);

typedef struct {
    int vocab_size, hidden_size, num_layers, num_heads, intermediate_size, max_position, type_vocab, num_labels;
    int visual_dim, acoustic_dim, pad_token_id;
    float layer_norm_eps, mag_layer_norm_eps, beta_shift;
    float hidden_dropout, attn_dropout, mag_dropout;
    int dtype;
    int max_batch, max_seq;
    int injection_index;
    int hidden_act;
} mb_bert_config;

typedef struct mb_bert_engine mb_bert_engine;

int mb_bert_create(const mb_bert_config* cfg, mb_bert_engine** out);
void mb_bert_destroy(mb_bert_engine* e);
int mb_bert_num_tensors(const mb_bert_engine* e);
int mb_bert_tensor_info(const mb_bert_engine* e, int i, char* name, int name_cap, size_t* offset, size_t* numel,
                        int* ndim, int64_t* shape4, int* decay);
size_t mb_bert_param_count(const mb_bert_engine* e);
size_t mb_bert_decay_count(const mb_bert_engine* e);
void mb_bert_shadow_range(const mb_bert_engine* e, size_t* begin, size_t* end);
size_t mb_bert_workspace_bytes(const mb_bert_engine* e);
int mb_bert_bind(mb_bert_engine* e, float* params, float* grads, void* shadow, void* workspace, size_t ws_bytes);
int mb_bert_sync_weights(mb_bert_engine* e, void* stream);

int mb_bert_forward(mb_bert_engine* e, const int64_t* input_ids, const float* visual, const float* acoustic,
                    const int64_t* attention_mask, const int64_t* token_type_ids, const float* labels, int B, int L,
                    int training, uint64_t seed, uint64_t step, float* logits, float* loss, float* loss_run,
                    void* stream);
int mb_bert_backward(mb_bert_engine* e, const float* dlogits, const float* labels, float loss_scale, int stage_begin,
                     int stage_end, void* stream);
const void* mb_bert_sequence_output(const mb_bert_engine* e);
const float* mb_bert_pooled_output(const mb_bert_engine* e);
const void* mb_bert_hidden_state(const mb_bert_engine* e, int i);
const void* mb_bert_debug_wgrad_dy(const mb_bert_engine* e, int layer, int which, int* ld);
int mb_bert_debug_live_wgrad_launches(const mb_bert_engine* e);
int mb_bert_set_attention_output(mb_bert_engine* e, float* probs);
int mb_bert_set_head_mask(mb_bert_engine* e, const float* head_mask);
int mb_bert_set_head_loss(mb_bert_engine* e, int kind, float param, const float* vec);
int mb_bert_get_head_loss(const mb_bert_engine* e, int* kind, float* param, float* vec, int* has_vec);
int mb_bert_set_head_loss_ex(mb_bert_engine* e, const mb_head_loss* hl);
int mb_bert_get_head_loss_ex(const mb_bert_engine* e, mb_head_loss* hl, float* vec, int* has_vec);
int mb_bert_set_inputs_embeds(mb_bert_engine* e, const float* inputs_embeds);
int mb_bert_set_position_ids(mb_bert_engine* e, const int64_t* position_ids);
const float* mb_bert_inputs_embeds_grad(const mb_bert_engine* e);
int mb_bert_backward_outputs(mb_bert_engine* e, const void* d_sequence_output, const void* d_pooler_preact, void* stream);
int mb_bert_stage_grad_ranges(const mb_bert_engine* e, int stage, size_t* offs, size_t* lens, int cap);

int mb_bert_mark_grads_zero(mb_bert_engine* e, int known_zero);
int mb_bert_distrust_word_stamps(mb_bert_engine* e);
size_t mb_bert_word_skip_updates(const mb_bert_engine* e);
int mb_bert_materialize_grads(mb_bert_engine* e, void* stream);
int mb_bert_grads_stale(const mb_bert_engine* e);

int mb_bert_train_step(mb_bert_engine* e, const int64_t* input_ids, const float* visual, const float* acoustic,
                       const int64_t* attention_mask, const int64_t* token_type_ids, const float* labels, int B, int L,
                       uint64_t seed, uint64_t step, float* logits, float* loss, float* loss_run, float* m, float* v, float lr,
                       float beta1, float beta2, float eps, float weight_decay, int opt_step, int correct_bias, float grad_scale,
                       float loss_scale, int mode, void* stream);
int mb_bert_stage_forward(mb_bert_engine* e, const int64_t* input_ids, const float* visual, const float* acoustic,
                          const int64_t* attention_mask, const int64_t* token_type_ids, const float* labels, int B, int L,
                          uint64_t seed, uint64_t step, float* logits, float* loss, float* loss_run, int mode, void* stream);
int mb_bert_stage_backward(mb_bert_engine* e, float loss_scale, int stage, int mode, void* stream);
const int64_t* mb_bert_staged_input_ids(const mb_bert_engine* e);
int mb_bert_load_batch(mb_bert_engine* e, const int64_t* input_ids, const float* visual, const float* acoustic,
                       const int64_t* attention_mask, const int64_t* token_type_ids, const float* labels, int B, int L,
                       const void** staged6, void* stream);
int mb_bert_graph_stats(const mb_bert_engine* e, size_t* captures, size_t* launches);

#define MB_UPDATE_CLASSES_MAX 32
#define MB_UPDATE_SEGMENTS_MAX 128
int mb_bert_set_update_map(mb_bert_engine* e, int n_classes, int n_segments, const size_t* boundaries, const int* classes);
int mb_bert_set_update_decay(mb_bert_engine* e, int n_segments, const uint8_t* no_decay);
int mb_bert_set_update_values(mb_bert_engine* e, int n_classes, const float* lr, const float* beta1, const float* beta2, const float* eps,
                              const float* weight_decay, const int* correct_bias);
int mb_bert_update_stats(const mb_bert_engine* e, size_t* ridden, size_t* swept, int* segments);
int mb_bert_set_update_frozen(mb_bert_engine* e, int n_segments, const uint8_t* frozen);
int mb_bert_freeze_stats(const mb_bert_engine* e, size_t* frozen_elems, int* wgrad_launches_skipped, int* embed_skipped);

int mb_bert_set_grad_clip(mb_bert_engine* e, float max_norm);
int mb_bert_grad_clip_stats(mb_bert_engine* e, float* norm, float* coef, void* stream);

int mb_bert_set_profiling(mb_bert_engine* e, int on);
int mb_bert_profile_wgrad_us(mb_bert_engine* e, float* avg_us);
int mb_bert_profile_adamw_us(mb_bert_engine* e, float* us);

typedef struct {
    int vocab_size, d_model, n_layer, n_head, d_inner, num_labels;
    int visual_dim, acoustic_dim, injection_index;
    float layer_norm_eps, mag_layer_norm_eps, beta_shift;
    float dropout, summary_last_dropout, mag_dropout;
    int dtype;
    int max_batch, max_seq;
    int ff_activation;
} mb_xlnet_config;

typedef struct mb_xlnet_engine mb_xlnet_engine;

size_t mb_xlnet_attention_tiled_stats_bytes(int B, int L, int nh);
size_t mb_xlnet_attention_tiled_scratch_bytes(int dtype, int B, int L, int nh);
int mb_xlnet_attention_tiled_forward(int dtype, const void* qkv, const void* kr, const float* r_w_bias, const float* r_r_bias,
                                     const float* r_s_bias, const float* seg_embed, const int64_t* seg, const int64_t* mask, void* vec,
                                     float* stats, int B, int L, int nh, const mb_dropkey* drop, const float* head_scale,
                                     const uint8_t* perm, int gstream, float* probs, void* stream);
int mb_xlnet_attention_tiled_backward(int dtype, const void* qkv, const void* kr, const float* r_w_bias, const float* r_r_bias,
                                      const float* r_s_bias, const float* seg_embed, const int64_t* seg, const int64_t* mask,
                                      const void* vec, const void* dvec, const float* stats, void* gsave, void* pdsave, void* dqkv,
                                      void* dkr, float* d_rwb, float* d_rrb, float* d_rsb, float* d_seg, int B, int L, int nh,
                                      const mb_dropkey* drop, const float* head_scale, const uint8_t* perm, void* stream);
int mb_xlnet_attention_forward(int dtype, const void* qkv, const void* kr, const float* r_w_bias, const float* r_r_bias,
                               const float* r_s_bias, const float* seg_embed, const int64_t* seg, const int64_t* mask, void* vec,
                               void* psave, float* stats, int B, int L, int nh, const mb_dropkey* drop, const float* head_scale,
                               const uint8_t* perm, int gstream, void* stream);
int mb_xlnet_attention_backward(int dtype, const void* qkv, const void* kr, const float* r_w_bias, const float* r_r_bias,
                                const float* r_s_bias, const float* seg_embed, const int64_t* seg, const int64_t* mask,
                                const void* psave, const void* vec, const void* dvec, const float* stats, void* gsave, void* pdsave,
                                void* dqkv, void* dkr, float* d_rwb, float* d_rrb, float* d_rsb, float* d_seg, int B, int L, int nh,
                                const mb_dropkey* drop, const float* head_scale, const uint8_t* perm, void* stream);

int mb_xlnet_create(const mb_xlnet_config* cfg, mb_xlnet_engine** out);
void mb_xlnet_destroy(mb_xlnet_engine* e);
int mb_xlnet_num_tensors(const mb_xlnet_engine* e);
int mb_xlnet_tensor_info(const mb_xlnet_engine* e, int i, char* name, int name_cap, size_t* offset, size_t* numel,
                         int* ndim, int64_t* shape4, int* decay);
size_t mb_xlnet_param_count(const mb_xlnet_engine* e);
size_t mb_xlnet_decay_count(const mb_xlnet_engine* e);
void mb_xlnet_shadow_range(const mb_xlnet_engine* e, size_t* begin, size_t* end);
size_t mb_xlnet_workspace_bytes(const mb_xlnet_engine* e);
int mb_xlnet_bind(mb_xlnet_engine* e, float* params, float* grads, void* shadow, void* workspace, size_t ws_bytes);
int mb_xlnet_sync_weights(mb_xlnet_engine* e, void* stream);
int mb_xlnet_forward(mb_xlnet_engine* e, const int64_t* input_ids, const float* visual, const float* acoustic,
                     const int64_t* attention_mask, const int64_t* token_type_ids, const float* labels, int B, int L,
                     int training, uint64_t seed, uint64_t step, float* logits, float* loss, float* loss_run,
                     void* stream);
// ... 88 lines not shown
```

Measured before the change: 15650 samples/s.

## Skip moment reads for word-embedding rows with all-zero Adam moments

Adds a lazy path to the AdamW sweep. Word-embedding rows that were not touched this step and whose m and v are known to be all zero now only load the parameter and apply weight decay, instead of reading g, m and v. A new scan kernel marks rows with nonzero moments using a SEEN bit in the stamp table. The engine tracks when that knowledge is stale, for example after external writes, state loads or multi-sweep steps. This cuts HBM traffic over the large vocab-sized embedding, at the cost of extra bookkeeping, an occasional full scan of m and v, and correctness risk if the tracking goes wrong.

```diff
diff --git a/bert_multimodal_transformer_amd/_lib.py b/bert_multimodal_transformer_amd/_lib.py
--- a/bert_multimodal_transformer_amd/_lib.py
+++ b/bert_multimodal_transformer_amd/_lib.py
@@ -155,6 +155,11 @@
     "mb_xlnet_mark_grads_zero": (_i, [_vp, _i]),
     "mb_bert_distrust_word_stamps": (_i, [_vp]),
     "mb_bert_word_skip_updates": (_sz, [_vp]),
+    "mb_bert_distrust_word_moments": (_i, [_vp]),
+    "mb_bert_word_moment_skip_updates": (_sz, [_vp]),
+    "mb_bert_word_moment_scans": (_sz, [_vp]),
+    "mb_debug_adamw_sweep": (_i, [_vp, _vp, _vp, _vp, _vp, _i, _vp, _vp, _vp, _sz, _sz, _sz, _sz, _vp, _vp, _vp, _sz, _sz, C.c_uint32, _vp]),
+    "mb_debug_word_moments_scan": (_i, [_vp, _vp, _vp, _sz, _sz, C.c_uint32, C.c_uint32, _vp]),
     "mb_bert_materialize_grads": (_i, [_vp, _vp]),
     "mb_xlnet_materialize_grads": (_i, [_vp, _vp]),
     "mb_bert_grads_stale": (_i, [_vp]),
diff --git a/bert_multimodal_transformer_amd/bert.py b/bert_multimodal_transformer_amd/bert.py
--- a/bert_multimodal_transformer_amd/bert.py
+++ b/bert_multimodal_transformer_amd/bert.py
@@ -280,6 +280,7 @@
                                              _lib.ptr(self.ws), nbytes))
             self.weights_dirty = True
             _lib.check(self._fn("mark_grads_zero")(self.handle, 1 if self._gz else 0))
+            self.distrust_word_moments()
 
     def _tensor_table(self):
         out = []
@@ -394,6 +395,10 @@
         self._gz_version = self.grads._version
         if self.handle is not None:
             _lib.check(self._fn("mark_grads_zero")(self.handle, 1 if known_zero else 0))
+
+    def distrust_word_moments(self):
+        if self.kind == "bert" and self.handle is not None:
+            _lib.check(self.lib.mb_bert_distrust_word_moments(self.handle))
 
     def torch_wrote_grads(self):
         return (not self._gz) or self.grads._version != getattr(self, "_gz_version", -1)
diff --git a/bert_multimodal_transformer_amd/csrc/adamw.hip b/bert_multimodal_transformer_amd/csrc/adamw.hip
--- a/bert_multimodal_transformer_amd/csrc/adamw.hip
+++ b/bert_multimodal_transformer_amd/csrc/adamw.hip
@@ -12,7 +12,7 @@
     if (dyn) a = *dyn;
     const size_t per = ((n4 + gridDim.x - 1) / gridDim.x + 255) / 256 * 256;
     const size_t begin = (size_t)blockIdx.x * per + threadIdx.x, end = min(n4, (size_t)(blockIdx.x + 1) * per);
-    adam_span<NT>(p, g, m, v, shadow, begin, end, a, n_decay, sh_begin, sh_end, keep_begin, keep_end, zero_grad, false, WordSkip{}, 0u);
+    adam_span<NT>(p, g, m, v, shadow, begin, end, a, n_decay, sh_begin, sh_end, keep_begin, keep_end, zero_grad, false, false, WordSkip{}, 0u);
 }
 
 __global__ void adamw_tail_kernel(float* p, float* g, float* m, float* v, size_t begin, size_t n, size_t n_decay, AdamArgs a,
@@ -94,6 +94,7 @@
     const size_t vb = (size_t)blockIdx.x * per, ve = min(total4, vb + per);
     const bool skip_on = ws.stamp != nullptr && ws.state[1] != 0u;
     const uint32_t stamp_no = skip_on ? ws.state[0] : 0u;
+    const bool lazy_on = skip_on && ws.state[2] != 0u;
 #pragma unroll 1
     for (int k = 0; k < R.clear_first; ++k) {
         const size_t off = R.start4[k], nxt = R.start4[k + 1];
@@ -104,7 +105,7 @@
         const AdamArgs a = cls[R.slot[k]];
         const size_t base4 = (size_t)R.begin4[k] - off;
         adam_span<NT>(p, g, m, v, shadow, base4 + lo + threadIdx.x, base4 + hi, a, ~(size_t)0, sh_begin, sh_end, keep_begin, keep_end, 1,
-                      skip_on, ws, stamp_no);
+                      skip_on, lazy_on, ws, stamp_no);
     }
 }
 
diff --git a/bert_multimodal_transformer_amd/csrc/adamw_dev.h b/bert_multimodal_transformer_amd/csrc/adamw_dev.h
--- a/bert_multimodal_transformer_amd/csrc/adamw_dev.h
+++ b/bert_multimodal_transformer_amd/csrc/adamw_dev.h
@@ -28,6 +28,18 @@
     }
     return q;
 }
+template <bool NT> __device__ __forceinline__ f32x4 adam_load_p(const float* p, size_t i) {
+    if constexpr (NT) return __builtin_nontemporal_load((const f32x4*)(p + i));
+    else return *(const f32x4*)(p + i);
+}
+template <bool NT> __device__ __forceinline__ void adam_decay_store(f32x4 qp, float* p, bf16* shadow, size_t i, float decay, size_t n_decay,
+                                                                    size_t sh_begin, size_t sh_end) {
+#pragma clang fp contract(off)
+    if (i < n_decay && decay > 0.f) qp -= decay * qp;
+    if constexpr (NT) __builtin_nontemporal_store(qp, (f32x4*)(p + i));
+    else *(f32x4*)(p + i) = qp;
+    if (shadow && i >= sh_begin && i < sh_end) store4(shadow + i, qp);
+}
 template <bool NT> __device__ __forceinline__ void adam_update_store(AdamQuad q, float* p, float* g, float* m, float* v, bf16* shadow, size_t i,
                                                                      const AdamArgs& a, float omb1, float omb2, float decay, size_t n_decay,
                                                                      size_t sh_begin, size_t sh_end, size_t keep_begin, size_t keep_end, int zero_grad) {
@@ -56,27 +68,34 @@
 template <bool NT>
 __device__ __forceinline__ void adam_span(float* p, float* g, float* m, float* v, bf16* shadow, size_t begin, size_t end, const AdamArgs& a,
                                           size_t n_decay, size_t sh_begin, size_t sh_end, size_t keep_begin, size_t keep_end, int zero_grad,
-                                          bool skip_on, const WordSkip& ws, uint32_t stamp_no) {
+                                          bool skip_on, bool lazy_on, const WordSkip& ws, uint32_t stamp_no) {
     constexpr int UNR = 2; const size_t stride = 256;
     const float omb1 = 1.0f - a.beta1, omb2 = 1.0f - a.beta2;
     const float decay = a.lr * a.weight_decay;
     for (size_t i4 = begin; i4 < end; i4 += stride * UNR) {
         AdamQuad q[UNR];
-        bool live[UNR];
+        bool live[UNR], lazy[UNR];
 #pragma unroll
         for (int u = 0; u < UNR; ++u) {
-            live[u] = true;
+            live[u] = true; lazy[u] = false;
             if (i4 + u * stride < end) {
                 const size_t i = (i4 + u * stride) * 4;
-                if (skip_on && i >= ws.begin && i < ws.end) live[u] = ws.stamp[(uint32_t)(i - ws.begin) / ws.row_len] == stamp_no;
-                q[u] = adam_load<NT>(p, g, m, v, i, live[u]);
+                if (skip_on && i >= ws.begin && i < ws.end) {
+                    const uint32_t w = ws.stamp[(uint32_t)(i - ws.begin) / ws.row_len];
+                    live[u] = (w & ~MB_STAMP_SEEN) == stamp_no;
+                    lazy[u] = lazy_on && !live[u] && !(w & MB_STAMP_SEEN);
+                }
+                if (lazy[u]) q[u].p = adam_load_p<NT>(p, i);
+                else q[u] = adam_load<NT>(p, g, m, v, i, live[u]);
             }
         }
 #pragma unroll
         for (int u = 0; u < UNR; ++u)
-            if (i4 + u * stride < end)
-                adam_update_store<NT>(q[u], p, g, m, v, shadow, (i4 + u * stride) * 4, a, omb1, omb2, decay, n_decay, sh_begin, sh_end, keep_begin,
-                                      keep_end, live[u] ? zero_grad : 0);
+            if (i4 + u * stride < end) {
+                if (lazy[u]) adam_decay_store<NT>(q[u].p, p, shadow, (i4 + u * stride) * 4, decay, n_decay, sh_begin, sh_end);
+                else adam_update_store<NT>(q[u], p, g, m, v, shadow, (i4 + u * stride) * 4, a, omb1, omb2, decay, n_decay, sh_begin, sh_end,
+                                           keep_begin, keep_end, live[u] ? zero_grad : 0);
+            }
     }
 }
 
diff --git a/bert_multimodal_transformer_amd/csrc/engine.hip b/bert_multimodal_transformer_amd/csrc/engine.hip
--- a/bert_multimodal_transformer_amd/csrc/engine.hip
+++ b/bert_multimodal_transformer_amd/csrc/engine.hip
@@ -167,8 +167,9 @@
     e->idcnt_off = w.take((size_t)c.vocab_size * 4);
     e->idcnt_enable = env_on("MB_EMBED_UNIQUE", true);
     e->stamp_rows = (size_t)c.vocab_size;
-    e->stamp_off = w.take(((size_t)c.vocab_size + 2) * 4);
+    e->stamp_off = w.take(((size_t)c.vocab_size + 4) * 4);
     e->stamp_enable = env_on("MB_ADAMW_SKIP_ZERO_ROWS", true);
+    e->mv_enable = e->stamp_enable && env_on("MB_ADAMW_SKIP_ZERO_MOMENTS", true);
     if (c.dtype == DT_BF16) {
         e->live_cap = std::max((size_t)192, T);
         e->live_off = w.take(2 * (e->live_cap + 8) * 4);
@@ -544,6 +545,24 @@
     return MB_OK;
 }
 
+int mb_debug_adamw_sweep(float* p, float* g, float* m, float* v, void* shadow, int npieces, const uint32_t* begin4, const uint32_t* len4,
+                         const uint8_t* slot, size_t sh_begin, size_t sh_end, size_t keep_begin, size_t keep_end, const void* cls,
+                         const void* stamp, const void* state, size_t word_begin, size_t word_end, uint32_t row_len, void* stream) {
+    if (npieces < 0 || npieces > MB_SWEEP_PIECES_MAX || (npieces && (!begin4 || !len4 || !slot))) return MB_ERR_ARG;
+    AdamPieces r = {};
+    for (int k = 0; k < npieces; ++k) {
+        if ((uint64_t)r.start4[k] + len4[k] > 0xffffffffull) return MB_ERR_SHAPE;
+        r.begin4[k] = begin4[k]; r.slot[k] = slot[k]; r.start4[k + 1] = r.start4[k] + len4[k];
+    }
+    r.count = r.clear_first = npieces;
+    const WordSkip skip = {(const uint32_t*)stamp, (const uint32_t*)state, word_begin, word_end, row_len};
+    return adamw_sweep(p, g, m, v, shadow, r, sh_begin, sh_end, keep_begin, keep_end, (const AdamArgs*)cls, skip, (hipStream_t)stream);
+}
+int mb_debug_word_moments_scan(const float* m, const float* v, void* stamp, size_t begin, size_t rows, uint32_t row_len, uint32_t keep_no,
+                               void* stream) {
+    return word_moments_scan(m, v, (uint32_t*)stamp, begin, rows, row_len, keep_no, (hipStream_t)stream);
+}
+
 int mb_adamw_step(float* p, float* g, float* m, float* v, void* shadow, size_t n, size_t n_decay, size_t sh_begin,
                   size_t sh_end, float lr, float beta1, float beta2, float eps, float weight_decay, int step,
                   int correct_bias, float grad_scale, int zero_grad, void* stream) {
@@ -620,6 +639,7 @@
     e->grads_zero = false;
     e->frz_dirty = true;
     e->stamp_live = e->word_zero = false; e->sweep_no = 1;
+    e->mv_clean = e->mv_prev_single = false;
     e->ws_zeroed = false; e->padT = -1;
     e->drop_graphs();
     char* mws = e->ws + e->ws_mag;
@@ -1171,6 +1191,13 @@
     return MB_OK;
 }
 size_t mb_bert_word_skip_updates(const mb_bert_engine* e) { return e ? e->skip_updates : 0; }
+int mb_bert_distrust_word_moments(mb_bert_engine* e) {
+    if (!e) return MB_ERR_ARG;
+    e->distrust_word_moments();
+    return MB_OK;
+}
+size_t mb_bert_word_moment_skip_updates(const mb_bert_engine* e) { return e ? e->mv_updates : 0; }
+size_t mb_bert_word_moment_scans(const mb_bert_engine* e) { return e ? e->mv_scans : 0; }
 int mb_bert_materialize_grads(mb_bert_engine* e, void* stream) {
     if (!e) return MB_ERR_ARG;
     return e->materialize_grads(e->G, (hipStream_t)stream);
diff --git a/bert_multimodal_transformer_amd/csrc/engine_common.h b/bert_multimodal_transformer_amd/csrc/engine_common.h
--- a/bert_multimodal_transformer_amd/csrc/engine_common.h
+++ b/bert_multimodal_transformer_amd/csrc/engine_common.h
@@ -226,6 +226,21 @@
     size_t stamp_off = 0, stamp_rows = 0; bool stamp_enable = false, stamp_live = false, word_zero = false;
     uint32_t sweep_no = 1;
     size_t skip_updates = 0;
+    bool mv_enable = false, mv_clean = false, mv_prev_single = false;
+    const float* mv_m = nullptr; const float* mv_v = nullptr;
+    size_t mv_updates = 0, mv_scans = 0;
+    void distrust_word_moments() { mv_clean = false; }
+    static bool lazy_scalars_ok(const AdamArgs& a) {
+        const float d = a.lr * a.weight_decay;
+        return a.eps > 0.f && std::isfinite(a.step_size) && a.step_size >= 0.f && std::isfinite(d) && std::isfinite(a.beta1) && a.beta1 >= 0.f &&
+               std::isfinite(a.beta2) && a.beta2 >= 0.f && std::isfinite(a.grad_scale) && a.grad_scale >= 0.f;
+    }
+    bool lazy_slots_ok(const PrologueArgs& pa, size_t b, size_t e, size_t n_decay) const {
+        if (n_classes == 0) return (b >= n_decay || lazy_scalars_ok(pa.adam[0])) && (e <= n_decay || lazy_scalars_ok(pa.adam[1]));
+        for (size_t s = 0; s + 1 < seg_bounds.size(); ++s)
+            if (seg_bounds[s] < e && seg_bounds[s + 1] > b && !lazy_scalars_ok(pa.cls[seg_class[s]])) return false;
+        return true;
+    }
     uint32_t* stamp_table(char* ws) const { return (uint32_t*)(ws + stamp_off); }
     uint32_t* stamp_state(char* ws) const { return stamp_table(ws) + stamp_rows; }
     bool one_sweep = false;
@@ -326,6 +341,7 @@
         struct Scope { StepMixin* m; ~Scope() { m->dyn = false; m->capturing = false; m->in_step = false; m->stage_mode = false; } } scope{this};
         dyn = true; in_step = true; stage_mode = true;
         stamp_live = word_zero = false;
+        mv_clean = mv_prev_single = false;
         frz_dirty = true;
         if (mode == 2) return enqueue(st);
         StageGraph* g = nullptr;
@@ -456,7 +472,7 @@
         if (++map_version <= 0) map_version = 1;
         return MB_OK;
     }
-    void marks_changed() { frz_dirty = true; stamp_live = word_zero = false; }
+    void marks_changed() { frz_dirty = true; stamp_live = word_zero = false; mv_clean = false; }
     int set_update_frozen(int ns, const uint8_t* frozen) {
         if (n_classes == 0) return MB_ERR_MODE;
         if (ns != (int)seg_class.size() || !frozen) return MB_ERR_ARG;
@@ -702,7 +718,7 @@
     if (!(ow && e->ow_covers)) CK(e->materialize_grads(e->G, st));
     const bool stale_before = e->grads_stale;
     struct Flags {
-        E* e; bool ok, with_opt, stale_before;
+        E* e; bool ok, with_opt, stale_before, single, lazy;
         ~Flags() {
             e->in_step = false; e->loss_cleared = false; e->packed = false; e->packed_w = false; e->counted = false; e->live_built = false;
             if (ok && e->clip_step) e->clip_ran = true;
@@ -710,11 +726,14 @@
             e->grads_zero = ok && with_opt;
             e->grads_stale = ok ? (with_opt && e->keep_in_step()) : stale_before;
             if (ok && with_opt && e->stamp_live) ++e->skip_updates;
+            if (!ok || (with_opt && !(e->stamp_live && single))) e->mv_clean = false;
+            if (ok && with_opt && lazy) ++e->mv_updates;
+            if (with_opt) e->mv_prev_single = ok && single;
             if (!ok || with_opt) e->stamp_live = false;
             e->word_zero = ok && with_opt;
-            if (ok && with_opt && ++e->sweep_no == 0u) e->sweep_no = 1u;
-        }
-    } flags{e, false, m != nullptr, stale_before};
+            if (ok && with_opt && ++e->sweep_no >= MB_STAMP_SEEN) e->sweep_no = 1u;
+        }
+    } flags{e, false, m != nullptr, stale_before, variant <= 0, false};
     const bool no_embed = e->any_frozen && e->embed_all_frozen();
     const bool stamping = e->stamp_off != 0 && e->stamp_enable && e->idcnt_enable && ids != nullptr && !no_embed;
     if (!stamping) e->stamp_live = false;
@@ -734,6 +753,7 @@
     if (e->idcnt_enable && ids && !no_embed) { pa.ids = (const int64_t*)ids; pa.n_ids = B * L; pa.id_count = (int*)(ws + e->idcnt_off); }
     e->counted = pa.id_count != nullptr;
     if (stamping) { pa.stamp = e->stamp_table(ws); pa.stamp_state = e->stamp_state(ws); pa.stamp_no = e->sweep_no; pa.stamp_on = e->stamp_live ? 1u : 0u; }
+    if (stamping && e->mv_enable) pa.stamp_seen = MB_STAMP_SEEN;
     if (e->live_off != 0 && e->live_enable && variant <= 0 && mask != nullptr && (size_t)align_up((size_t)B * L, 64) <= e->live_cap &&
         B <= MB_LIVE_MAX_SAMPLES && B * L <= MB_LIVE_MAX_ROWS) {
         pa.live_rows = e->live_rows(ws); pa.live_count = e->live_count(ws); pa.live_mask = (const int64_t*)mask;
@@ -763,6 +783,18 @@
         if (e->n_classes > 0) { pa.ncls = e->n_classes; pa.cls_dst = e->class_state(ws); }
         if (clip) { pa.clip[0] = e->clip_max; pa.clip[1] = grad_scale; pa.clip_dst = e->clip_params(); }
     }
+    if (m && v && (m != e->mv_m || v != e->mv_v)) { e->mv_clean = false; e->mv_m = m; e->mv_v = v; }
+    if (m && v && e->mv_enable && stamping && e->stamp_live && variant <= 0 && !clip) {
+        const WordSkip wsk = e->word_skip(ws);
+        if (wsk.stamp && wsk.end > wsk.begin && !e->range_frozen(wsk.begin, wsk.end) && e->lazy_slots_ok(pa, wsk.begin, wsk.end, e->n_decay)) {
+            if (!e->mv_clean && e->mv_prev_single) {
+                CK(word_moments_scan(m, v, e->stamp_table(ws), wsk.begin, (wsk.end - wsk.begin) / wsk.row_len, wsk.row_len, e->sweep_no, st));
+                e->mv_clean = true; ++e->mv_scans;
+            }
+            flags.lazy = e->mv_clean;
+        }
+    }
+    pa.stamp_lazy = flags.lazy ? 1u : 0u;
     CK(step_prologue(pa, st));
     if (mode == 2 || force_launches) {
         e->dyn = true;
diff --git a/bert_multimodal_transformer_amd/csrc/kernels.h b/bert_multimodal_transformer_amd/csrc/kernels.h
--- a/bert_multimodal_transformer_amd/csrc/kernels.h
+++ b/bert_multimodal_transformer_amd/csrc/kernels.h
@@ -225,6 +225,7 @@
 int adamw_step(float* p, float* g, float* m, float* v, void* shadow, size_t n, size_t n_decay,
                size_t sh_begin, size_t sh_end, AdamArgs a, int zero_grad, hipStream_t st, const AdamArgs* dyn = nullptr,
                size_t keep_begin = 0, size_t keep_end = 0);
+#define MB_STAMP_SEEN 0x80000000u
 struct WordSkip { const uint32_t* stamp; const uint32_t* state; size_t begin, end; uint32_t row_len; };
 #define MB_CLASSES_MAX 32
 #define MB_SEGMENTS_MAX 128
@@ -256,7 +257,7 @@
     struct PackJob { const float* src; void* dst; int rows, cols, pitch, dtype; } pack[2];
     int npack;
     const int64_t* ids; int n_ids; int* id_count;
-    uint32_t* stamp; uint32_t* stamp_state; uint32_t stamp_no, stamp_on;
+    uint32_t* stamp; uint32_t* stamp_state; uint32_t stamp_no, stamp_on, stamp_seen, stamp_lazy;
     uint32_t* live_rows; uint32_t* live_count; const int64_t* live_mask; int live_T, live_Tp, live_L;
     uint32_t* cls_rows; uint32_t* cls_count;
     struct MagPackW { const float* W_hv; const float* W_ha; const float* W_v; const float* W_a; void* We; void* Wv; void* Wa; MagDims d; int dtype; } magw;
@@ -264,6 +265,8 @@
 };
 static_assert(sizeof(PrologueArgs) <= 2048, "PrologueArgs travels as kernel arguments (4 KB limit)");
 int step_prologue(const PrologueArgs& a, hipStream_t st);
+int word_moments_scan(const float* m, const float* v, uint32_t* stamp, size_t begin, size_t rows, uint32_t row_len, uint32_t keep_no,
+                      hipStream_t st);
 #define MB_ZERO_MAX 8
 struct ZeroRanges {
     uint32_t* p[MB_ZERO_MAX]; size_t ndw[MB_ZERO_MAX]; int n;
diff --git a/bert_multimodal_transformer_amd/csrc/rowops.hip b/bert_multimodal_transformer_amd/csrc/rowops.hip
--- a/bert_multimodal_transformer_amd/csrc/rowops.hip
+++ b/bert_multimodal_transformer_amd/csrc/rowops.hip
@@ -809,8 +809,8 @@
     if (a.id_count != nullptr)
         for (size_t i = tid; i < (size_t)a.n_ids; i += nth) atomicAdd(a.id_count + a.ids[i], 1);
     if (a.stamp != nullptr) {
-        for (size_t i = tid; i < (size_t)a.n_ids; i += nth) a.stamp[a.ids[i]] = a.stamp_no;
-        if (tid < 2) a.stamp_state[tid] = tid == 0 ? a.stamp_no : a.stamp_on;
+        for (size_t i = tid; i < (size_t)a.n_ids; i += nth) a.stamp[a.ids[i]] = a.stamp_no | a.stamp_seen;
+        if (tid < 3) a.stamp_state[tid] = tid == 0 ? a.stamp_no : tid == 1 ? a.stamp_on : a.stamp_lazy;
     }
     for (int k = 0; k < a.npack; ++k) {
         const PrologueArgs::PackJob& j = a.pack[k];
@@ -905,6 +905,32 @@
     return (int)hipGetLastError();
 }
 
+__global__ void __launch_bounds__(256) word_moments_scan_kernel(const float* __restrict__ m, const float* __restrict__ v,
+                                                                uint32_t* __restrict__ stamp, size_t rows, uint32_t row_len, uint32_t keep_no) {
+    const size_t row = (size_t)blockIdx.x * 4 + threadIdx.x / 64;
+    if (row >= rows) return;
+    const int lane = threadIdx.x & 63;
+    const u32x4* mr = (const u32x4*)(m + row * row_len);
+    const u32x4* vr = (const u32x4*)(v + row * row_len);
+    uint32_t any = 0u;
+    for (uint32_t i = lane; i < row_len / 4; i += 64) {
+        const u32x4 a = __builtin_nontemporal_load(mr + i), b = __builtin_nontemporal_load(vr + i);
+        any |= a[0] | a[1] | a[2] | a[3] | b[0] | b[1] | b[2] | b[3];
+    }
+    const bool nz = __ballot(any != 0u) != 0ull;
+    if (lane == 0) {
+        const uint32_t w = stamp[row];
+        if ((w & ~MB_STAMP_SEEN) != keep_no) stamp[row] = (w & ~MB_STAMP_SEEN) | (nz ? MB_STAMP_SEEN : 0u);
+    }
+}
+int word_moments_scan(const float* m, const float* v, uint32_t* stamp, size_t begin, size_t rows, uint32_t row_len, uint32_t keep_no, hipStream_t st) {
+    if (!m || !v || !stamp || row_len == 0 || (row_len | begin) % 4 || (((uintptr_t)m | (uintptr_t)v) & 15)) return MB_ERR_ARG;
+    if (rows == 0) return MB_OK;
+    if ((rows + 3) / 4 > 0x7fffffffull) return MB_ERR_SHAPE;
+    hipLaunchKernelGGL(word_moments_scan_kernel, dim3((unsigned)((rows + 3) / 4)), dim3(256), 0, st, m + begin, v + begin, stamp, rows, row_len, keep_no);
+    return (int)hipGetLastError();
+}
+
 
 __global__ void __launch_bounds__(256) grad_fold_kernel(long long* __restrict__ shadow, float* __restrict__ g, size_t begin, size_t end) {
     for (size_t i = begin + (size_t)blockIdx.x * 256 + threadIdx.x; i < end; i += (size_t)gridDim.x * 256) {
diff --git a/bert_multimodal_transformer_amd/optimization.py b/bert_multimodal_transformer_amd/optimization.py
--- a/bert_multimodal_transformer_amd/optimization.py
+++ b/bert_multimodal_transformer_amd/optimization.py
@@ -8,6 +8,12 @@
 
 UPDATE_CLASSES_MAX = 32
 UPDATE_SEGMENTS_MAX = 128
+
+
+def _distrust_word_moments(core):
+    fn = getattr(core, "distrust_word_moments", None)
+    if fn is not None:
+        fn()
 
 
 FROZEN = -1
@@ -378,6 +384,7 @@
         self._t += 1
         for core, _ in self._covers.values():
             core.materialize_grads()
+            _distrust_word_moments(core)
         dp = self._dp
         late = []
         if dp is not None and getattr(dp, "late_ranges", None):
@@ -493,6 +500,7 @@
             for c, st in zip(cores, extra["flat"]):
                 c._adam_m.copy_(st["exp_avg"])
                 c._adam_v.copy_(st["exp_avg_sq"])
+                _distrust_word_moments(c)
 
     def zero_grad(self, set_to_none=False):
         if self._plan is None:
diff --git a/include/magbert_hip.h b/include/magbert_hip.h
--- a/include/magbert_hip.h
+++ b/include/magbert_hip.h
@@ -43,6 +43,11 @@
                                const void* const* rows, const void* const* nrows, void* stream);
 int mb_debug_live_rows(const int64_t* mask, int B, int L, int Tp, void* live_rows, void* live_count, void* cls_rows, void* cls_count,
                        void* stream);
+int mb_debug_adamw_sweep(float* p, float* g, float* m, float* v, void* shadow, int npieces, const uint32_t* begin4, const uint32_t* len4,
+                         const uint8_t* slot, size_t sh_begin, size_t sh_end, size_t keep_begin, size_t keep_end, const void* cls,
+                         const void* stamp, const void* state, size_t word_begin, size_t word_end, uint32_t row_len, void* stream);
+int mb_debug_word_moments_scan(const float* m, const float* v, void* stamp, size_t begin, size_t rows, uint32_t row_len, uint32_t keep_no,
+                               void* stream);
 
 int mb_gemm_grouped_wgrad(int dtype, int count, const int* M, const int* N, int K, const void* const* dY, const int* ldy,
                           const void* const* X, const int* ldx, float* const* dW, const int* ldw, int tile, void* stream);
@@ -174,6 +179,9 @@
 int mb_bert_mark_grads_zero(mb_bert_engine* e, int known_zero);
 int mb_bert_distrust_word_stamps(mb_bert_engine* e);
 size_t mb_bert_word_skip_updates(const mb_bert_engine* e);
+int mb_bert_distrust_word_moments(mb_bert_engine* e);
+size_t mb_bert_word_moment_skip_updates(const mb_bert_engine* e);
+size_t mb_bert_word_moment_scans(const mb_bert_engine* e);
 int mb_bert_materialize_grads(mb_bert_engine* e, void* stream);
 int mb_bert_grads_stale(const mb_bert_engine* e);
 
```

New measurement: 15870 samples/s (median of 6 runs). +1.4%, better.
